# CRIPAC-DIG/GET

Hardware: AMD Instinct MI355X
Metric: claim-evidence pairs/sec fwd+bwd (B=32, h=300) (higher is better)
Workload: dtype f32

## Files before the change

### get_amd/csrc/common.h

```cpp
#pragma once
#include <hip/hip_runtime.h>
#include <stdint.h>
#include <stdio.h>
#include <stdlib.h>
#include <string.h>

namespace gh {

void set_error(const char* fmt, ...);

#define GH_CHECK_HIP(expr)                                                                  \
  do {                                                                                      \
    hipError_t _e = (expr);                                                                 \
    if (_e != hipSuccess) {                                                                 \
      gh::set_error("%s:%d: %s -> %s", __FILE__, __LINE__, #expr, hipGetErrorString(_e));   \
      return 1;                                                                             \
    }                                                                                       \
  } while (0)

#define GH_REQUIRE(cond, ...)                     \
  do {                                            \
    if (!(cond)) {                                \
      gh::set_error(__VA_ARGS__);                 \
      return 2;                                   \
    }                                             \
  } while (0)

#define GH_LAUNCH_CHECK() GH_CHECK_HIP(hipGetLastError())

inline int words_for(int r) { return (r + 63) / 64; }

inline int measure_env(const char* name, int dflt) {
#ifdef GH_MEASURE
  const char* e = getenv(name);
  return e ? atoi(e) : dflt;
#else
  (void)name;
  return dflt;
#endif
}
#ifdef GH_MEASURE
#define GH_DBG_BITS(L) ((L).dbg)
#else
#define GH_DBG_BITS(L) 0
#endif

enum ProfTag : int {
  PROF_GEMM_BIG = 0, PROF_GEMM_BIG_TN, PROF_GEMM_SMALL, PROF_GEMM_SMALL_TN,
  PROF_SPMM, PROF_SCORER_GSL, PROF_GRAPH_BUILD, PROF_ATT_SOFTMAX_FWD, PROF_ATT_SOFTMAX_BWD, PROF_ATT_DPRE,
  PROF_GATE_BWD_PRE, PROF_COLSUM, PROF_ADAM,
  PROF_FEW_ROWS,
  PROF_NTAGS
};
constexpr int PROF_FEW_GROUPS = 256;
unsigned int* clamp_counter();
bool prof_enabled();
void prof_begin(hipStream_t s, int tag);
void prof_end(int tag, double work, hipStream_t s);

int scorer_gsl_impl(const uint64_t* bits, const float* dinv, const float* vals, const int32_t* goff, int pads_collapsed, const float* feat,
                    const float* score_x, int score_parts, long long score_stride, const float* w_p, const float* gate, int n, int r, int h,
                    int k, float* score, uint64_t* keep, float drop_p, uint32_t drop_seed, hipStream_t stream);
int launch_ragged_plan(const int32_t* n_nodes, const int32_t* node_ids, int n, int r, int32_t* goff, int32_t* rowg, int32_t* src,
                       int32_t* cids, float* maskf, const int64_t* slot, int32_t* document, hipStream_t s, bool* scattered);
int launch_graph_build2(const int32_t* ta, const int32_t* la, int na, int ra, int32_t* ida, int32_t* nna, uint64_t* ba, float* da,
                        const int32_t* tb, const int32_t* lb, int nb, int rb, int32_t* idb, int32_t* nnb, uint64_t* bb, float* db,
                        int window, hipStream_t s);
struct ZeroFill { float* p0; long long n0; float* p1; long long n1; };
int launch_spmm(const uint64_t* bits, const float* dinv, const float* vals, const uint64_t* keep, const int32_t* goff,
                int m_real, const float* x, float* y, int n, int r, int h, int transpose, int accumulate, hipStream_t s,
                int bf16 = 0,
                const ZeroFill* zf = nullptr, bool* zf_done = nullptr);
int launch_gate_bwd_pre(const float* g, const float* z, const float* hh, const float* xp, float* dhp, float* dzp,
                        float* dxp, size_t count, hipStream_t s, int bf16 = 0);
int launch_colsum3(const float* a, const float* b, const float* c, float* oa, float* ob, float* oc, int m, int h,
                   hipStream_t s, float* oa2 = nullptr, float* ob2 = nullptr, float* oc2 = nullptr);
int launch_colsum(const float* a, float* oa, int m, int h, hipStream_t s);
struct Workspace { float* p; size_t bytes; float* cs; size_t cs_bytes; };
Workspace workspace_for(hipStream_t s);
int launch_gather_rows(const float* table, const int32_t* ids, float* dst, int m, int d, hipStream_t s,
                       float drop_p = 0.f, unsigned drop_seed = 0, int bf16 = 0);
int launch_tiny_linear_fwd(const float* x, const float* w, const float* bias, float* y, int m, int k, int n, hipStream_t s);
int launch_head_bwd(const float* g_phi, const float* y0, const float* w1, const float* w0, int B, int H, int C, int Xl, int E,
                    float* d_y0, float* dw1, float* db1, float* dx0, int dx0_accumulate, float* dx1, hipStream_t s);
size_t head_bwd_lds(int B, int H, int C, int E, const float* w0);
int launch_tiny_linear_bwd(const float* x, const float* w, const float* g, float* dx, float* dw, float* db, int m, int k, int n,
                           hipStream_t s);
int launch_att_softmax_fwd(float* e, const float* mask, const float* right, const int32_t* goff, int m_real,
                           int b, int l, int dr, int heads, float* weights, float* attended, hipStream_t s,
                           const float* e_parts = nullptr, int n_parts = 0, long long part_stride = 0, const void* right16 = nullptr);
int launch_att_softmax_bwd(const float* right, const float* weights, const float* g_att, const float* g_w,
                           const int32_t* goff, int m_real, int b, int l, int dr, int heads, float* de, float* dright,
                           hipStream_t s, const int32_t* rowg = nullptr, float* dw_tmp = nullptr, int* dw_written = nullptr,
                           const void* right16 = nullptr);
int gemm_mode();
int launch_att_dpre(const float* de, const float* w2, const float* t, const int32_t* goff, int m_real, int b, int l,
                    int ha, int heads, float* dpre, float* du, float* dw2_part, hipStream_t s, const float* dw_in = nullptr,
                    const float* weights = nullptr, float* de_out = nullptr, void* dpre16 = nullptr,
                    long long dw_range_stride = 0, int dw_ranges = 1);

struct GateFuse { const float* z; const float* hh; const float* xp; float* dhp; float* dzp; float* dxp; int bf16; };

int cell_fwd_impl(int bf, float* out32, const uint64_t* bits, const float* dinv, const float* vals, const uint64_t* keep,
                  const int32_t* goff, int m_real, int m_rows, const float* x, const int32_t* ids, int n, int r, int din, int h,
                  const float* w_p, const float* w_z0, const float* w_z1, const float* w_r0, const float* w_r1, const float* w_h0,
                  const float* w_h1, const float* b_z0, const float* b_z1, const float* b_r0, const float* b_r1, const float* b_h0,
                  const float* b_h1, float* xp, float* a, float* z, float* rr, float* rx, float* hh, float* out, float drop_p,
                  uint32_t drop_seed, const float* score_w, float* score_x, float score_drop_p, uint32_t score_drop_seed,
                  void* stream, int pad_out_dead = 0,
                  int* score_parts = nullptr,
                  float* xdrop = nullptr);
int cell_bwd_impl(int bf, const uint64_t* bits, const float* dinv, const float* vals, const uint64_t* keep, const int32_t* goff,
                  int m_real, const float* x, const int32_t* ids, int n, int r, int din, int h, const float* wt_p,
                  const float* wt_z0, const float* wt_z1, const float* wt_r0, const float* wt_r1, const float* wt_h0,
                  const float* wt_h1, const float* xp, const float* a, const float* z, const float* rr, const float* rx,
                  const float* hh, const float* g, float* dhp, float* dzp, float* drp, float* dxp, float* da, float* dx,
                  float* dw_p, float* dw_z0, float* dw_z1, float* dw_r0, float* dw_r1, float* dw_h0, float* dw_h1, float* db_z,
                  float* db_r, float* db_h, float* db_z1, float* db_r1, float* db_h1, float drop_p, uint32_t drop_seed, void* stream,
                  void* wstream, hipEvent_t ev_l1, hipEvent_t ev_agg,
                  int pre_done, const GateFuse* next,
                  const float* xdrop = nullptr);
int att_fwd_impl(const float* left, int nl, const int32_t* rowu, const float* right, const float* mask, const int32_t* goff,
                 const int32_t* rowg, int m_real, int b, int l, int xl, int dr, int ha, int heads, const float* w1, const float* w2,
                 float* u, float* t, float* e, float* weights, float* attended, hipStream_t s, int u_mode = 0,
                 const void* right16 = nullptr, const void* w1_16 = nullptr);
int att_bwd_impl(const float* left, const float* right, const int32_t* goff, int m_real, int b, int l, int xl, int dr, int ha,
                 int heads, const float* w1t, const float* w2, const float* t, const float* weights, const float* g_att,
                 const float* g_w, float* de, float* dpre, float* du, float* dleft, float* dright, float* dw1, float* dw2,
                 const int32_t* claim_offsets, int nl, float* du_c, int dleft_accumulate, hipStream_t s,
                 const int32_t* rowg = nullptr, float* dw_tmp = nullptr, const GateFuse* next = nullptr, int dleft_late = 0,
                 float* dw2_buf = nullptr, const void* right16 = nullptr, const void* w1t_16 = nullptr);
int linear2_fwd(const float* x0, int k0, const float* x1, int k1, const float* w, const float* bias, float* y, int m, int n, hipStream_t s,
                const float* w_out = nullptr, const float* b_out = nullptr, float* y_out = nullptr, int n_out = 0);
int linear2_bwd(const float* x0, int k0, const float* x1, int k1, const float* wt, const float* g, int m, int n, float* dx0,
                int dx0_accumulate, float* dx1, float* dw, float* db, hipStream_t s);

}
```

### get_amd/csrc/gemm.hip.h

```cpp
#pragma once
#include <hip/hip_runtime.h>
#include <stdint.h>
#include <type_traits>

namespace gh {

typedef float f32x4 __attribute__((ext_vector_type(4)));

enum EpiKind : int {
  EPI_STORE = 0,
  EPI_SIGMOID_Z,
  EPI_SIGMOID_R,
  EPI_TANH_H,
  EPI_ATT,
  EPI_BWD_DRX,
  EPI_ATOMIC,
  EPI_GATE_PRE,
};

struct Seg {
  const float* A; const int32_t* gatherA; int lda; int vecA;
  const float* B; const int32_t* gatherB; int ldb; int vecB;
  int K;
};

struct Problem {
  Seg seg[2];
  int nseg;
  int M, N;
  int epi;
  int accumulate;
  float* C; int ldc;
  const float* bias;
  const float* bias2;
  float* out1;
  const float* in0; const float* in1;
  const float* u; const float* w2; float* e; int ldu; int R; int heads;
  int seg0_rows;
  const int32_t* rowg;
  long long split_stride;
  float* colsum; long long colsum_stride;
  int drop_mode; int drop_ld; int drop_col0; unsigned drop_seed; unsigned drop_thresh; float drop_scale;
  int elt; int io; float* c32;
  int e_atomic;
  const float* gin; const float* in2; float* out2;
};

#define GH_MAX_PROBLEMS 12
struct Launch {
  Problem p[GH_MAX_PROBLEMS];
  int nprob;
  int m_tiles;
  int ksplit;
  int kchunk;
  int dbg;
  int n_tiles;
  int per;
};
static_assert(sizeof(Launch) <= 4096, "Launch travels by value in the kernarg segment (4 KB)");
constexpr int DBG_NO_EPILOGUE = 1;
constexpr int DBG_NO_KLOOP = 2;
constexpr int DBG_EPI_TICKS = 1024;

__host__ __device__ __forceinline__ unsigned drop_hash(unsigned seed, unsigned idx) {
  unsigned x = idx * 0x9E3779B1u + seed;
  x ^= x >> 16; x *= 0x85EBCA6Bu; x ^= x >> 13; x *= 0xC2B2AE35u; x ^= x >> 16;
  return x;
}
__device__ __forceinline__ float4 drop4(float4 v, unsigned seed, unsigned idx, unsigned thresh, float scale) {
  v.x = drop_hash(seed, idx + 0) >= thresh ? v.x * scale : 0.f;
  v.y = drop_hash(seed, idx + 1) >= thresh ? v.y * scale : 0.f;
  v.z = drop_hash(seed, idx + 2) >= thresh ? v.z * scale : 0.f;
  v.w = drop_hash(seed, idx + 3) >= thresh ? v.w * scale : 0.f;
  return v;
}

__device__ __forceinline__ float sigmoidf_(float x) { return 1.0f / (1.0f + __expf(-x)); }
__device__ __forceinline__ float tanhf_(float x) {
  float e = __expf(2.0f * x);
  return 1.0f - 2.0f / (e + 1.0f);
}

#define GH_KARG __attribute__((address_space(4)))

template <int WM, int WN, int NI, bool TN>
__global__ void __launch_bounds__(WM * WN * 64, 2)
gemm_kernel(const Launch L_byval) {
  (void)L_byval;
  const GH_KARG Launch& L = *(const GH_KARG Launch*)__builtin_amdgcn_kernarg_segment_ptr();
  constexpr int NTHR = WM * WN * 64;
  constexpr int BM = 32 * WM, BN = 16 * NI * WN, BK = 16;
  constexpr int LDA = BM + 2, LDB = BN + 2;
  constexpr int A4 = BM * 4;
  constexpr int B4 = BK * (BN / 4);
  constexpr int NA = (A4 + NTHR - 1) / NTHR;
  constexpr int NB = (B4 + NTHR - 1) / NTHR;
  __shared__ float smem[2 * BK * LDA + 2 * BK * LDB];
  float* As = smem;
  float* Bs = smem + 2 * BK * LDA;

  const int n_inner = TN ? L.m_tiles * L.nprob : L.nprob;
  const int n_outer = TN ? L.ksplit : L.m_tiles;
  const int bid = blockIdx.x;
  const int xcd = bid & 7, slot = bid >> 3;
  const int outer = xcd + 8 * (slot / n_inner);
  const int inner = slot % n_inner;
  if (outer >= n_outer) return;
  const int prob = TN ? inner % L.nprob : inner;
  const int m_tile = TN ? inner / L.nprob : outer;
  const int ks = TN ? outer : 0;
  const GH_KARG Problem& P = L.p[prob];
  const int M = P.M, N = P.N;
// ... 174 lines not shown
          for (int ni = 0; ni < NI; ++ni) {
            const int col = wcol + ni * 16 + l15;
            if (ni < ni_cnt && col < N) {
              const float t = tanhf_(acc[mi][ni][reg] + urow[col]);
              P.C[(size_t)row * ldc + col] = t;
#pragma unroll
              for (int c = 0; c < 8; ++c)
                if (c < heads) pe[c] += t * P.w2[c * N + col];
            }
          }
        }
#pragma unroll
        for (int c = 0; c < 8; ++c) {
          float v = pe[c];
          v += __shfl_xor(v, 1); v += __shfl_xor(v, 2); v += __shfl_xor(v, 4); v += __shfl_xor(v, 8);
          pe[c] = v;
        }
        if (WN == 1) {
          if (l15 == 0 && row < M && mi < mi_cnt)
            for (int c = 0; c < heads; ++c) P.e[(size_t)row * heads + c] = pe[c];
        } else {
          if (l15 == 0)
            for (int c = 0; c < 8; ++c) red[(wn * BM + lrow) * 8 + c] = pe[c];
        }
      }
    };
    att_rows(std::integral_constant<int, 0>{});
    att_rows(std::integral_constant<int, 1>{});
    if (WN > 1) {
      __syncthreads();
      for (int i = tid; i < BM * 8; i += NTHR) {
        const int lrow = i >> 3, c = i & 7, row = m0 + lrow;
        if (row < M && c < heads) {
          float v = 0.f;
          for (int w = 0; w < WN; ++w) v += red[(w * BM + lrow) * 8 + c];
          P.e[(size_t)row * heads + c] = v;
        }
      }
    }
    return;
  }

  auto epi_rows = [&](auto MI) __attribute__((always_inline)) {
    constexpr int mi = decltype(MI)::value;
#pragma unroll
    for (int ni = 0; ni < NI; ++ni) {
      const int col = wcol + ni * 16 + l15;
      const bool tile_ok = (mi < mi_cnt) && (ni < ni_cnt) && (col < N);
      const float bias = ((tile_ok && P.bias) ? P.bias[col] : 0.f) + ((tile_ok && P.bias2) ? P.bias2[col] : 0.f);
#pragma unroll
      for (int reg = 0; reg < 4; ++reg) {
        const int row = m0 + wrow + mi * 16 + q * 4 + reg;
        if (tile_ok && row < M) {
          const size_t o = (size_t)row * ldc + col;
          const float v = acc[mi][ni][reg] + bias;
          if (epi == EPI_STORE) {
            Cout[o] = P.accumulate ? Cout[o] + v : v;
          } else if (epi == EPI_SIGMOID_Z) {
            Cout[o] = sigmoidf_(v);
          } else if (epi == EPI_SIGMOID_R) {
            const float r = sigmoidf_(v);
            Cout[o] = r;
            P.out1[o] = r * P.in0[o];
          } else if (epi == EPI_TANH_H) {
            const float h = tanhf_(v), z = P.in0[o], xp = P.in1[o];
            Cout[o] = h;
            P.out1[o] = h * z + xp * (1.f - z);
          } else if (epi == EPI_BWD_DRX) {
            const float xp = P.in0[o], r = P.in1[o];
            Cout[o] = v * xp * r * (1.f - r);
            P.out1[o] += v * r;
          } else if (epi == EPI_ATOMIC) {
            atomicAdd(Cout + o, v);
          }
        }
      }
    }
  };
  epi_rows(std::integral_constant<int, 0>{});
  epi_rows(std::integral_constant<int, 1>{});
}

inline int vec_ok(const void* p, int ld, int inner) {
  return ((reinterpret_cast<uintptr_t>(p) & 15) == 0) && (ld % 4 == 0) && (inner % 4 == 0);
}

inline Seg make_seg(const float* A, int lda, const float* B, int ldb, int K, int n_inner,
                    const int32_t* gatherA = nullptr, const int32_t* gatherB = nullptr) {
  Seg s;
  s.A = A; s.lda = lda; s.gatherA = gatherA; s.vecA = vec_ok(A, lda, K);
  s.B = B; s.ldb = ldb; s.gatherB = gatherB; s.vecB = vec_ok(B, ldb, n_inner);
  s.K = K;
  return s;
}
inline Seg make_seg_nt(const float* A, int lda, const float* B, int ldb, int K, const int32_t* gatherA = nullptr, int elt = 0) {
  Seg s;
  const int q = elt ? 8 : 4;
  s.A = A; s.lda = lda; s.gatherA = gatherA; s.vecA = ((reinterpret_cast<uintptr_t>(A) & 15) == 0) && lda % q == 0 && K % q == 0;
  s.B = B; s.ldb = ldb; s.gatherB = nullptr; s.vecB = ((reinterpret_cast<uintptr_t>(B) & 15) == 0) && ldb % q == 0 && K % q == 0;
  s.K = K;
  return s;
}
inline Seg make_seg_tn(const float* A, int lda, int I, const float* B, int ldb, int J, int K,
                       const int32_t* gatherA = nullptr, const int32_t* gatherB = nullptr) {
  Seg s;
  s.A = A; s.lda = lda; s.gatherA = gatherA; s.vecA = vec_ok(A, lda, I);
  s.B = B; s.ldb = ldb; s.gatherB = gatherB; s.vecB = vec_ok(B, ldb, J);
  s.K = K;
  return s;
}

inline Problem make_problem(int M, int N, int epi, float* C, int ldc) {
  Problem p;
  memset(&p, 0, sizeof(p));
  p.M = M; p.N = N; p.epi = epi; p.C = C; p.ldc = ldc; p.nseg = 1;
  return p;
}


hipError_t launch_gemm(Launch& L, bool tn, hipStream_t stream);

}
```

### get_amd/csrc/gemm_nt.hip.h

```cpp
#pragma once
#include "common.h"
#include "gemm.hip.h"

namespace gh {
#ifdef GH_MEASURE
__device__ unsigned long long g_nt_phase[16 * 4];
#endif

__device__ __forceinline__ int nt_swz(int j) { return (0x78 >> (2 * j)) & 3; }
__device__ __forceinline__ unsigned nt_pack_bf16(float a, float b) {
  typedef float f32x2_t __attribute__((ext_vector_type(2)));
  typedef __bf16 bf16x2_t __attribute__((ext_vector_type(2)));
  const f32x2_t v = {a, b};
  return __builtin_bit_cast(unsigned, __builtin_convertvector(v, bf16x2_t));
}

template <int WM, int WN, int NI, int MI = 2, int MODE = 0>
__global__ void __launch_bounds__(WM * WN * 64, (MI == 8 || MI == 4 || MODE == 3 || MODE == 4) ? 2 : (WM == 2 && WN == 2 && NI == 5 && MODE == 0) ? 4 : 3)
gemm_nt_kernel(const Launch L_byval) {
  (void)L_byval;
#if defined(__HIP_DEVICE_COMPILE__)
  const GH_KARG Launch& L = *(const GH_KARG Launch*)__builtin_amdgcn_kernarg_segment_ptr();
  typedef __amdgpu_buffer_rsrc_t rsrc_t;
  constexpr int NW = WM * WN, NTHR = NW * 64;
// ... 384 lines not shown
        mma(aC, bX, 0, CX);
        __builtin_amdgcn_sched_barrier(0);
#pragma unroll
        for (int mi = 0; mi < MI; ++mi) aP[mi] = aC[mi];
        wait_inflight(min(T - 1, t + NST - 1) - (t + 1));
        __builtin_amdgcn_s_barrier();
        asm volatile("" ::: "memory");
        st = st == NST - 1 ? 0 : st + 1;
      }
      mma(aP, bY, NH, CY);
      __syncthreads();
      return;
    }
    dma_tile(0, 0);
    asm volatile("s_waitcnt vmcnt(0)" ::: "memory");
    __syncthreads();
    for (int t = 0; t < T; ++t) {
      const int st = t & 1;
      if (t + 1 < T) dma_tile(t + 1, st ^ 1);
      read_a(st, aC);
      read_b(st, bX, 0, NH);
      __builtin_amdgcn_sched_barrier(0);
      if (t > 0) mma(aP, bY, NH, CY);
      __builtin_amdgcn_sched_barrier(0);
      read_b(st, bY, NH, NI - NH);
      if (drop_mode == 1) drop_a(t, aC);
      __builtin_amdgcn_sched_barrier(0);
      mma(aC, bX, 0, CX);
      __builtin_amdgcn_sched_barrier(0);
#pragma unroll
      for (int mi = 0; mi < MI; ++mi) aP[mi] = aC[mi];
      asm volatile("s_waitcnt vmcnt(0)" ::: "memory");
      __syncthreads();
    }
    mma(aP, bY, NH, CY);
  };
  if constexpr (PP) {
#include "gemm_nt_pp.hip.h"
  } else {
    if (nvX == NH && nvY == NI - NH - 1) run(std::integral_constant<int, NH>{}, std::integral_constant<int, NI - NH - 1>{});
    else run(std::integral_constant<int, NH>{}, std::integral_constant<int, NI - NH>{});
  }

  if (dbg_bits & DBG_NO_EPILOGUE) {
    float sum = 0.f;
#pragma unroll
    for (int mi = 0; mi < MI; ++mi)
#pragma unroll
      for (int ni = 0; ni < NI; ++ni) sum += acc[mi][ni][0] + acc[mi][ni][1] + acc[mi][ni][2] + acc[mi][ni][3];
    if (sum == 12345.678f) P.C[0] = 0.f;
    return;
  }
  const int epi = P.epi;
  const int ldc = P.ldc;
  float* const C = P.C + (split ? (size_t)ks * (size_t)P.split_stride : (size_t)0);
  const float* bias = P.bias;
  float* out1 = P.out1;
  const float* in0 = P.in0;
  const float* in1 = P.in1;
  const int accumulate = P.accumulate;
  const int heads = P.heads;
  const bool scorer = (epi == EPI_TANH_H) && (P.w2 != nullptr);
  const int pad_rows = MODE == 2 ? 0 : P.seg0_rows;
  const bool out_dead = scorer && P.ldu == 1;
  const bool rowred = (epi == EPI_ATT) || scorer;
  float* ep = reinterpret_cast<float*>(smem);
  float* const ep_bias_ptr = ep + (PP ? 64 : 16 * WM) * EP_PITCH + NW * 64 * 4;
  const int N4 = N >> 2;
  constexpr int C4 = EP_PITCH / 4;
  constexpr int ITEMS = 16 * WM * C4;
  constexpr int NIT = (ITEMS + NTHR - 1) / NTHR;
  const float* bias2 = P.bias2;
  float* bsum = ep_bias_ptr;
  for (int c = tid; c < BN; c += NTHR) {
    float bv = 0.f;
    if (c < N) { if (bias) bv = bias[c]; if (bias2) bv += bias2[c]; }
    bsum[c] = bv;
  }
  const int io = (MODE == 2) ? P.io : 0;
  float* const c32 = (MODE == 2) ? P.c32 : nullptr;
  auto ld4 = [&](const float* p, size_t o, bool bf) __attribute__((always_inline)) {
    if constexpr (MODE == 2) {
      if (bf) {
        const uint2 u = *reinterpret_cast<const uint2*>(reinterpret_cast<const unsigned short*>(p) + o);
        return make_float4(__builtin_bit_cast(float, u.x << 16), __builtin_bit_cast(float, u.x & 0xffff0000u),
                           __builtin_bit_cast(float, u.y << 16), __builtin_bit_cast(float, u.y & 0xffff0000u));
      }
    }
    return *reinterpret_cast<const float4*>(p + o);
  };
  auto st4 = [&](float* p, size_t o, const float4 v, bool bf) __attribute__((always_inline)) {
    if constexpr (MODE == 2) {
      if (bf) {
        *reinterpret_cast<uint2*>(reinterpret_cast<unsigned short*>(p) + o) = make_uint2(nt_pack_bf16(v.x, v.y), nt_pack_bf16(v.z, v.w));
        return;
      }
    }
    __builtin_nontemporal_store(f32x4{v.x, v.y, v.z, v.w}, reinterpret_cast<f32x4*>(p + o));
  };
  auto row_reduce = [&](auto MIT) __attribute__((always_inline)) {
    constexpr int mi = decltype(MIT)::value;
    if (rowred) {
      __syncthreads();
      constexpr int KSPL = NW / WM;
      const int nred = scorer ? 1 : heads;
      const int b = wave % WM, kp = wave / WM;
      const float* arow = ep + (b * 16 + l15) * EP_PITCH + 4 * q;
// ... 1 lines not shown
      f32x4 d = f32x4{0.f, 0.f, 0.f, 0.f};
      for (int k0 = kp * 16; k0 < N; k0 += 16 * KSPL) {
        const f32x4 a4 = *reinterpret_cast<const f32x4*>(arow + k0);
        f32x4 w4 = f32x4{0.f, 0.f, 0.f, 0.f};
        if (l15 < nred && k0 + 4 * q < N) w4 = *reinterpret_cast<const f32x4*>(wrow + k0);
#pragma unroll
        for (int s2 = 0; s2 < 4; ++s2) d = __builtin_amdgcn_mfma_f32_16x16x4f32(w4[s2], a4[s2], d, 0, 0, 0);
      }
      float* red = ep + 16 * WM * EP_PITCH;
      *reinterpret_cast<f32x4*>(red + ((kp * WM + b) * 64 + lane) * 4) = d;
      __syncthreads();
      if (kp == 0) {
        f32x4 sum = d;
#pragma unroll
        for (int k2 = 1; k2 < KSPL; ++k2) sum += *reinterpret_cast<const f32x4*>(red + ((k2 * WM + b) * 64 + lane) * 4);
        const int row = m0 + b * 16 * MI + mi * 16 + l15;
        if (row < M) {
#pragma unroll
          for (int r = 0; r < 4; ++r)
            if (4 * q + r < nred) {
              if (P.e_atomic == 1) atomicAdd(&P.e[(size_t)row * nred + 4 * q + r], sum[r]);
              else P.e[(size_t)row * nred + 4 * q + r] = sum[r];
            }
        }
      }
    }
  };
  auto epilogue_pass = [&](auto MIT) __attribute__((always_inline)) {
    constexpr int mi = decltype(MIT)::value;
    if (mi > 0) __syncthreads();
#pragma unroll
    for (int ni = 0; ni < NI; ++ni)
      *reinterpret_cast<f32x4*>(ep + (wm * 16 + l15) * EP_PITCH + wcol + ni * 16 + 4 * q) = acc[mi][ni];
    __syncthreads();
    auto pass = [&](auto EPI) __attribute__((always_inline)) {
      constexpr int E = decltype(EPI)::value;
      constexpr int CH = 4;
#pragma unroll
      for (int it0 = 0; it0 < NIT; it0 += CH) {
        float4 xa[CH], xb[CH], xc[CH], xd[E == EPI_GATE_PRE ? CH : 1];
        auto where = [&](int j, int& row, int& col, float*& sp) __attribute__((always_inline)) {
          const int i = tid + (it0 + j) * NTHR;
          const int rr = i / C4, c4 = i - rr * C4;
          row = m0 + (rr >> 4) * 16 * MI + mi * 16 + (rr & 15);
          col = 4 * c4;
          sp = ep + rr * EP_PITCH + col;
          return (it0 + j < NIT) && (ITEMS % NTHR == 0 || i < ITEMS) && c4 < N4 && row < M;
        };
        if (E != EPI_SIGMOID_Z) {
#pragma unroll
          for (int j = 0; j < CH; ++j) {
            int row, col; float* sp;
            if (where(j, row, col, sp)) {
              const size_t o = (size_t)row * ldc + col;
              if (E == EPI_STORE) { if (accumulate) xa[j] = ld4(C, o, io & 1); }
              else if (E == EPI_SIGMOID_R) xa[j] = ld4(in0, o, io & 4);
              else if (E == EPI_TANH_H) { xa[j] = ld4(in0, o, io & 4); xb[j] = ld4(in1, o, io & 8); }
              else if (E == EPI_BWD_DRX) {
                xa[j] = ld4(in0, o, io & 4);
                xb[j] = ld4(in1, o, io & 8);
                xc[j] = ld4(out1, o, io & 2);
              } else if (E == EPI_GATE_PRE) {
                xa[j] = ld4(in0, o, io & 4);
                xb[j] = ld4(in1, o, io & 8);
                xc[j] = ld4(P.in2, o, io & 16);
                if (P.gin) xd[j] = ld4(P.gin, o, false);
              } else if (E == EPI_ATT)
                xa[j] = *reinterpret_cast<const float4*>(P.u + (size_t)(P.rowg ? P.rowg[row] : row / P.R) * P.ldu + col);
            }
          }
        }
#pragma unroll
        for (int j = 0; j < CH; ++j) {
          int row, col; float* sp;
          if (!where(j, row, col, sp)) continue;
          const float4 v4 = *reinterpret_cast<const float4*>(sp);
          const float4 b4 = *reinterpret_cast<const float4*>(bsum + col);
          float4 w = make_float4(v4.x + b4.x, v4.y + b4.y, v4.z + b4.z, v4.w + b4.w);
          const size_t o = (size_t)row * ldc + col;
          if (E == EPI_STORE) {
            if (drop_mode == 3)
              w = drop4(w, drop_seed, (unsigned)row * (unsigned)drop_ld + (unsigned)(P.drop_col0 + col), drop_thresh, drop_scale);
            if (accumulate) { w.x += xa[j].x; w.y += xa[j].y; w.z += xa[j].z; w.w += xa[j].w; }
            st4(C, o, w, io & 1);
          } else if (E == EPI_SIGMOID_Z) {
            st4(C, o, make_float4(sigmoidf_(w.x), sigmoidf_(w.y), sigmoidf_(w.z), sigmoidf_(w.w)), io & 1);
          } else if (E == EPI_SIGMOID_R) {
            const float4 x = xa[j];
            const float4 r4 = make_float4(sigmoidf_(w.x), sigmoidf_(w.y), sigmoidf_(w.z), sigmoidf_(w.w));
            if (!(pad_rows > 0 && row >= pad_rows)) st4(C, o, r4, io & 1);
            st4(out1, o, make_float4(r4.x * x.x, r4.y * x.y, r4.z * x.z, r4.w * x.w), io & 2);
          } else if (E == EPI_TANH_H) {
            const float4 z = xa[j], x = xb[j];
            const float4 h = make_float4(tanhf_(w.x), tanhf_(w.y), tanhf_(w.z), tanhf_(w.w));
            float4 y = make_float4(h.x * z.x + x.x * (1.f - z.x), h.y * z.y + x.y * (1.f - z.y),
                                   h.z * z.z + x.z * (1.f - z.z), h.w * z.w + x.w * (1.f - z.w));
            const bool pad = pad_rows > 0 && row >= pad_rows;
            if (!pad) st4(C, o, h, io & 1);
            if (!(pad && out_dead)) st4(out1, o, y, io & 2);
            if (c32) *reinterpret_cast<float4*>(c32 + o) = y;
            if (scorer) {
              if (drop_mode == 2)
                y = drop4(y, drop_seed, (unsigned)row * (unsigned)drop_ld + (unsigned)(P.drop_col0 + col), drop_thresh, drop_scale);
              *reinterpret_cast<float4*>(sp) = y;
            }
          } else if (E == EPI_BWD_DRX) {
            const float4 x = xa[j], r4 = xb[j];
            float4 d = xc[j];
            st4(C, o, make_float4(w.x * x.x * r4.x * (1.f - r4.x), w.y * x.y * r4.y * (1.f - r4.y),
                                  w.z * x.z * r4.z * (1.f - r4.z), w.w * x.w * r4.w * (1.f - r4.w)), io & 1);
            d.x += w.x * r4.x; d.y += w.y * r4.y; d.z += w.z * r4.z; d.w += w.w * r4.w;
            st4(out1, o, d, io & 2);
          } else if (E == EPI_GATE_PRE) {
            if (drop_mode == 3)
              w = drop4(w, drop_seed, (unsigned)row * (unsigned)drop_ld + (unsigned)(P.drop_col0 + col), drop_thresh, drop_scale);
            if (P.gin) { const float4 a4 = xd[j]; w.x += a4.x; w.y += a4.y; w.z += a4.z; w.w += a4.w; }
            const float4 Z = xa[j], Hh = xb[j], X = xc[j];
            float4 a, b, c;
#define GH_ONE(f)                                      \
            a.f = w.f * Z.f * (1.f - Hh.f * Hh.f);             \
            b.f = w.f * (Hh.f - X.f) * Z.f * (1.f - Z.f);      \
            c.f = w.f * (1.f - Z.f);
            GH_ONE(x) GH_ONE(y) GH_ONE(z) GH_ONE(w)
#undef GH_ONE
            if constexpr (MODE == 2) {
              st4(C, o, a, io & 1); st4(out1, o, b, io & 2); st4(P.out2, o, c, io & 32);
            } else {
              *reinterpret_cast<float4*>(C + o) = a;
              *reinterpret_cast<float4*>(out1 + o) = b;
              *reinterpret_cast<float4*>(P.out2 + o) = c;
            }
          } else if (E == EPI_ATT) {
            const float4 u4 = xa[j];
            const float4 t4 = make_float4(tanhf_(w.x + u4.x), tanhf_(w.y + u4.y), tanhf_(w.z + u4.z), tanhf_(w.w + u4.w));
            *reinterpret_cast<float4*>(C + o) = t4;
            *reinterpret_cast<float4*>(sp) = t4;
          }
        }
      }
    };
    auto pass8 = [&](auto EPI) __attribute__((always_inline)) {
      constexpr int E = decltype(EPI)::value;
      constexpr int C8 = BN / 8;
      constexpr int ITEMS8 = 16 * WM * C8;
      constexpr int NIT8 = (ITEMS8 + NTHR - 1) / NTHR;
      constexpr int CH = 2;
      struct F8 { float4 a, b; };
      auto ld8 = [&](const float* p, size_t o, bool bf) __attribute__((always_inline)) {
        F8 r;
        if (bf) {
          const uint4 u = *reinterpret_cast<const uint4*>(reinterpret_cast<const unsigned short*>(p) + o);
          r.a = make_float4(__builtin_bit_cast(float, u.x << 16), __builtin_bit_cast(float, u.x & 0xffff0000u),
                            __builtin_bit_cast(float, u.y << 16), __builtin_bit_cast(float, u.y & 0xffff0000u));
          r.b = make_float4(__builtin_bit_cast(float, u.z << 16), __builtin_bit_cast(float, u.z & 0xffff0000u),
                            __builtin_bit_cast(float, u.w << 16), __builtin_bit_cast(float, u.w & 0xffff0000u));
        } else {
          r.a = *reinterpret_cast<const float4*>(p + o);
          r.b = *reinterpret_cast<const float4*>(p + o + 4);
        }
        return r;
      };
      auto st8 = [&](float* p, size_t o, const float4 a, const float4 b, bool bf) __attribute__((always_inline)) {
        if (bf) {
          *reinterpret_cast<uint4*>(reinterpret_cast<unsigned short*>(p) + o) =
              make_uint4(nt_pack_bf16(a.x, a.y), nt_pack_bf16(a.z, a.w), nt_pack_bf16(b.x, b.y), nt_pack_bf16(b.z, b.w));
        } else {
          *reinterpret_cast<float4*>(p + o) = a;
          *reinterpret_cast<float4*>(p + o + 4) = b;
        }
      };
      auto sig4 = [](const float4 v) __attribute__((always_inline)) { return make_float4(sigmoidf_(v.x), sigmoidf_(v.y), sigmoidf_(v.z), sigmoidf_(v.w)); };
      auto tanh4 = [](const float4 v) __attribute__((always_inline)) { return make_float4(tanhf_(v.x), tanhf_(v.y), tanhf_(v.z), tanhf_(v.w)); };
      auto mul4 = [](const float4 a, const float4 b) __attribute__((always_inline)) { return make_float4(a.x * b.x, a.y * b.y, a.z * b.z, a.w * b.w); };
      auto add4 = [](const float4 a, const float4 b) __attribute__((always_inline)) { return make_float4(a.x + b.x, a.y + b.y, a.z + b.z, a.w + b.w); };
      auto mix4 = [](const float4 h, const float4 z, const float4 x) __attribute__((always_inline)) {
        return make_float4(h.x * z.x + x.x * (1.f - z.x), h.y * z.y + x.y * (1.f - z.y), h.z * z.z + x.z * (1.f - z.z), h.w * z.w + x.w * (1.f - z.w));
      };
      auto drx4 = [](const float4 w, const float4 x, const float4 r) __attribute__((always_inline)) {
        return make_float4(w.x * x.x * r.x * (1.f - r.x), w.y * x.y * r.y * (1.f - r.y), w.z * x.z * r.z * (1.f - r.z), w.w * x.w * r.w * (1.f - r.w));
      };
#pragma unroll
      for (int it0 = 0; it0 < NIT8; it0 += CH) {
        F8 xa[CH], xb[CH], xc[CH], xd[E == EPI_GATE_PRE ? CH : 1];
        auto where = [&](int j, int& row, int& col, float*& sp) __attribute__((always_inline)) {
          const int i = tid + (it0 + j) * NTHR;
          const int rr = i / C8, c8 = i - rr * C8;
          row = m0 + (rr >> 4) * 16 * MI + mi * 16 + (rr & 15);
          col = 8 * c8;
          sp = ep + rr * EP_PITCH + col;
          return (it0 + j < NIT8) && (ITEMS8 % NTHR == 0 || i < ITEMS8) && col < N && row < M;
        };
        if (E != EPI_SIGMOID_Z) {
#pragma unroll
          for (int j = 0; j < CH; ++j) {
            int row, col; float* sp;
            if (where(j, row, col, sp)) {
              const size_t o = (size_t)row * ldc + col;
              if (E == EPI_STORE) { if (accumulate) xa[j] = ld8(C, o, io & 1); }
              else if (E == EPI_SIGMOID_R) xa[j] = ld8(in0, o, io & 4);
              else if (E == EPI_TANH_H) { xa[j] = ld8(in0, o, io & 4); xb[j] = ld8(in1, o, io & 8); }
              else if (E == EPI_BWD_DRX) { xa[j] = ld8(in0, o, io & 4); xb[j] = ld8(in1, o, io & 8); xc[j] = ld8(out1, o, io & 2); }
              else if (E == EPI_GATE_PRE) {
                xa[j] = ld8(in0, o, io & 4); xb[j] = ld8(in1, o, io & 8); xc[j] = ld8(P.in2, o, io & 16);
                if (P.gin) xd[j] = ld8(P.gin, o, false);
              }
            }
          }
        }
#pragma unroll
        for (int j = 0; j < CH; ++j) {
          int row, col; float* sp;
          if (!where(j, row, col, sp)) continue;
          float4 wa = add4(*reinterpret_cast<const float4*>(sp), *reinterpret_cast<const float4*>(bsum + col));
          float4 wb = add4(*reinterpret_cast<const float4*>(sp + 4), *reinterpret_cast<const float4*>(bsum + col + 4));
          const size_t o = (size_t)row * ldc + col;
          if (E == EPI_STORE) {
            if (drop_mode == 3) {
              const unsigned idx = (unsigned)row * (unsigned)drop_ld + (unsigned)(P.drop_col0 + col);
              wa = drop4(wa, drop_seed, idx, drop_thresh, drop_scale);
              wb = drop4(wb, drop_seed, idx + 4u, drop_thresh, drop_scale);
            }
            if (accumulate) { wa = add4(wa, xa[j].a); wb = add4(wb, xa[j].b); }
            st8(C, o, wa, wb, io & 1);
          } else if (E == EPI_SIGMOID_Z) {
            st8(C, o, sig4(wa), sig4(wb), io & 1);
          } else if (E == EPI_SIGMOID_R) {
            const float4 ra = sig4(wa), rb = sig4(wb);
            st8(C, o, ra, rb, io & 1);
            st8(out1, o, mul4(ra, xa[j].a), mul4(rb, xa[j].b), io & 2);
          } else if (E == EPI_TANH_H) {
            const float4 ha = tanh4(wa), hb = tanh4(wb);
            const float4 ya = mix4(ha, xa[j].a, xb[j].a), yb = mix4(hb, xa[j].b, xb[j].b);
            st8(C, o, ha, hb, io & 1);
            st8(out1, o, ya, yb, io & 2);
            if (c32) { *reinterpret_cast<float4*>(c32 + o) = ya; *reinterpret_cast<float4*>(c32 + o + 4) = yb; }
            if (scorer) {
              float4 sa = ya, sb = yb;
              if (drop_mode == 2) {
                const unsigned idx = (unsigned)row * (unsigned)drop_ld + (unsigned)(P.drop_col0 + col);
                sa = drop4(sa, drop_seed, idx, drop_thresh, drop_scale);
                sb = drop4(sb, drop_seed, idx + 4u, drop_thresh, drop_scale);
              }
              *reinterpret_cast<float4*>(sp) = sa;
              *reinterpret_cast<float4*>(sp + 4) = sb;
            }
          } else if (E == EPI_BWD_DRX) {
            st8(C, o, drx4(wa, xa[j].a, xb[j].a), drx4(wb, xa[j].b, xb[j].b), io & 1);
            st8(out1, o, add4(xc[j].a, mul4(wa, xb[j].a)), add4(xc[j].b, mul4(wb, xb[j].b)), io & 2);
          } else if (E == EPI_GATE_PRE) {
            if (drop_mode == 3) {
              const unsigned idx = (unsigned)row * (unsigned)drop_ld + (unsigned)(P.drop_col0 + col);
              wa = drop4(wa, drop_seed, idx, drop_thresh, drop_scale);
              wb = drop4(wb, drop_seed, idx + 4u, drop_thresh, drop_scale);
            }
            if (P.gin) { wa = add4(wa, xd[j].a); wb = add4(wb, xd[j].b); }
            auto head = [](const float4 g, const float4 Z, const float4 Hh, const float4 X, float4& a, float4& b, float4& c) __attribute__((always_inline)) {
#define GH_ONE8(f)                                    \
              a.f = g.f * Z.f * (1.f - Hh.f * Hh.f);          \
              b.f = g.f * (Hh.f - X.f) * Z.f * (1.f - Z.f);   \
              c.f = g.f * (1.f - Z.f);
              GH_ONE8(x) GH_ONE8(y) GH_ONE8(z) GH_ONE8(w)
#undef GH_ONE8
            };
            float4 a0, b0, c0, a1, b1, c1;
            head(wa, xa[j].a, xb[j].a, xc[j].a, a0, b0, c0);
            head(wb, xa[j].b, xb[j].b, xc[j].b, a1, b1, c1);
            st8(C, o, a0, a1, io & 1); st8(out1, o, b0, b1, io & 2); st8(P.out2, o, c0, c1, io & 32);
          }
        }
      }
    };
    constexpr bool WIDE8 = (MODE == 2) && (BN % 8 == 0);
    bool done8 = false;
    if constexpr (WIDE8) {
      if (epi != EPI_ATT) {
        if (epi == EPI_STORE) pass8(std::integral_constant<int, EPI_STORE>{});
        else if (epi == EPI_GATE_PRE) pass8(std::integral_constant<int, EPI_GATE_PRE>{});
        else if (epi == EPI_SIGMOID_Z) pass8(std::integral_constant<int, EPI_SIGMOID_Z>{});
        else if (epi == EPI_SIGMOID_R) pass8(std::integral_constant<int, EPI_SIGMOID_R>{});
        else if (epi == EPI_TANH_H) pass8(std::integral_constant<int, EPI_TANH_H>{});
        else if (epi == EPI_BWD_DRX) pass8(std::integral_constant<int, EPI_BWD_DRX>{});
        if (!rowred) return;
        done8 = true;
      }
    }
    if (done8) {  }
    else if (epi == EPI_STORE) pass(std::integral_constant<int, EPI_STORE>{});
    else if (epi == EPI_SIGMOID_Z) pass(std::integral_constant<int, EPI_SIGMOID_Z>{});
    else if (epi == EPI_SIGMOID_R) pass(std::integral_constant<int, EPI_SIGMOID_R>{});
    else if (epi == EPI_TANH_H) pass(std::integral_constant<int, EPI_TANH_H>{});
    else if (epi == EPI_BWD_DRX) pass(std::integral_constant<int, EPI_BWD_DRX>{});
    else if (epi == EPI_GATE_PRE) pass(std::integral_constant<int, EPI_GATE_PRE>{});
    else if (epi == EPI_ATT) pass(std::integral_constant<int, EPI_ATT>{});
    row_reduce(MIT);
  };
  if constexpr ((MODE == 0 || MODE == 1) && MI == 2) {
    bool f32_done = false;
#include "gemm_nt_epi32.hip.h"
    if (f32_done) return;
  }
  if constexpr (PP) {
    bool pp_done = true;
#include "gemm_nt_pp_epi.hip.h"
    if (pp_done) return;
  }
  epilogue_pass(std::integral_constant<int, 0>{});
  epilogue_pass(std::integral_constant<int, 1>{});
  if constexpr (MI >= 4) {
    epilogue_pass(std::integral_constant<int, 2>{});
    epilogue_pass(std::integral_constant<int, 3>{});
  }
  if constexpr (MI == 8) {
    epilogue_pass(std::integral_constant<int, 4>{});
    epilogue_pass(std::integral_constant<int, 5>{});
    epilogue_pass(std::integral_constant<int, 6>{});
    epilogue_pass(std::integral_constant<int, 7>{});
  }
#endif
}

// ... 2 lines not shown
```

### get_amd/csrc/gemm_nt_epi32.hip.h

```cpp
{
  constexpr int NITF = (ITEMS + NTHR - 1) / NTHR;
  constexpr int TOT = MI * NITF;
  constexpr int PD = 2, NSET = PD + 1;
  typedef unsigned e32_u32x4 __attribute__((ext_vector_type(4)));
  int tid_e = tid;
  asm volatile("" : "+v"(tid_e));
  auto f_item = [&](int mi_, int it, int& row, int& col, int& rr) __attribute__((always_inline)) {
    const int i = tid_e + it * NTHR;
    rr = i / C4;
    const int c4 = i - rr * C4;
    col = 4 * c4;
    row = m0 + (rr >> 4) * 16 * MI + mi_ * 16 + (rr & 15);
    return (ITEMS % NTHR == 0 || i < ITEMS) && c4 < N4 && row < M;
  };
  auto as_f4 = [](const e32_u32x4 u) __attribute__((always_inline)) {
    const f32x4 f = __builtin_bit_cast(f32x4, u);
    return make_float4(f[0], f[1], f[2], f[3]);
  };
  auto as_u4 = [](const float4 v) __attribute__((always_inline)) {
    return e32_u32x4{__builtin_bit_cast(unsigned, v.x), __builtin_bit_cast(unsigned, v.y), __builtin_bit_cast(unsigned, v.z), __builtin_bit_cast(unsigned, v.w)};
  };
  auto fast = [&](auto EPI, auto ACCF, auto GINF) __attribute__((always_inline)) {
    constexpr int E = decltype(EPI)::value;
    constexpr bool ACC = decltype(ACCF)::value, GIN = decltype(GINF)::value, ATT = E == EPI_ATT;
    constexpr int NIN = E == EPI_STORE ? (ACC ? 1 : 0) : (E == EPI_SIGMOID_Z || ATT) ? 0 : E == EPI_SIGMOID_R ? 1 : E == EPI_TANH_H ? 2 : 3;
    constexpr int NOUT = (E == EPI_STORE || E == EPI_SIGMOID_Z || ATT) ? 1 : E == EPI_GATE_PRE ? 3 : 2;
    constexpr int NTAUX = (E == EPI_GATE_PRE || ATT) ? 0 : 2;
    const void* i0 = E == EPI_STORE ? (const void*)C : (const void*)in0;
    const void* i2 = E == EPI_BWD_DRX ? (const void*)out1 : (const void*)P.in2;
    const rsrc_t rs_i0 = __builtin_amdgcn_make_buffer_rsrc((void*)(NIN >= 1 ? i0 : (const void*)C), 0, 0x7fffffff, 0x00020000);
    const rsrc_t rs_i1 = __builtin_amdgcn_make_buffer_rsrc((void*)(NIN >= 2 ? (const void*)in1 : (const void*)C), 0, 0x7fffffff, 0x00020000);
    const rsrc_t rs_i2 = __builtin_amdgcn_make_buffer_rsrc((void*)(NIN >= 3 ? i2 : (const void*)C), 0, 0x7fffffff, 0x00020000);
    const rsrc_t rs_g = __builtin_amdgcn_make_buffer_rsrc((void*)(GIN ? (const void*)P.gin : ATT ? (const void*)P.u : (const void*)C), 0, 0x7fffffff, 0x00020000);
    const rsrc_t rs_o0 = __builtin_amdgcn_make_buffer_rsrc((void*)C, 0, 0x7fffffff, 0x00020000);
    const rsrc_t rs_o1 = __builtin_amdgcn_make_buffer_rsrc((void*)(NOUT >= 2 ? (void*)out1 : (void*)C), 0, 0x7fffffff, 0x00020000);
    const rsrc_t rs_o2 = __builtin_amdgcn_make_buffer_rsrc((void*)(NOUT >= 3 ? (void*)P.out2 : (void*)C), 0, 0x7fffffff, 0x00020000);
    e32_u32x4 qa[NSET], qb[NSET], qc[NSET], qg[NSET];
    unsigned uoff[ATT ? TOT : 1];
    if constexpr (ATT) {
#pragma unroll
      for (int idx = 0; idx < TOT; ++idx) {
        int row, col, rr;
        const bool ok = f_item(idx / NITF, idx % NITF, row, col, rr);
        const int rc_ = min(row, M - 1);
        const int ur = P.rowg ? P.rowg[rc_] : rc_ / P.R;
        uoff[idx] = ok ? (unsigned)(ur * P.ldu + col) * 4u : OOB;
      }
    }
    auto load = [&](auto IDX) __attribute__((always_inline)) {
      constexpr int idx = decltype(IDX)::value, mi_ = idx / NITF, it = idx % NITF, s_ = idx % NSET;
      int row, col, rr;
      const bool ok = f_item(mi_, it, row, col, rr);
      const unsigned vo = ok ? (unsigned)(row * ldc + col) * 4u : OOB;
      if constexpr (NIN >= 1) qa[s_] = __builtin_bit_cast(e32_u32x4, __builtin_amdgcn_raw_buffer_load_b128(rs_i0, vo, 0, 0));
      if constexpr (NIN >= 2) qb[s_] = __builtin_bit_cast(e32_u32x4, __builtin_amdgcn_raw_buffer_load_b128(rs_i1, vo, 0, 0));
      if constexpr (NIN >= 3) qc[s_] = __builtin_bit_cast(e32_u32x4, __builtin_amdgcn_raw_buffer_load_b128(rs_i2, vo, 0, 0));
      if constexpr (GIN) qg[s_] = __builtin_bit_cast(e32_u32x4, __builtin_amdgcn_raw_buffer_load_b128(rs_g, vo, 0, 0));
      if constexpr (ATT) qg[s_] = __builtin_bit_cast(e32_u32x4, __builtin_amdgcn_raw_buffer_load_b128(rs_g, uoff[idx], 0, 0));
    };
    auto compute = [&](auto IDX) __attribute__((always_inline)) {
      constexpr int idx = decltype(IDX)::value, mi_ = idx / NITF, it = idx % NITF, s_ = idx % NSET;
      int row, col, rr;
      const bool ok = f_item(mi_, it, row, col, rr);
      const unsigned vo = ok ? (unsigned)(row * ldc + col) * 4u : OOB;
      float* sp = ep + min(rr, 16 * WM - 1) * EP_PITCH + min(col, BN - 4);
      const float4 v4 = *reinterpret_cast<const float4*>(sp);
      const float4 b4 = *reinterpret_cast<const float4*>(bsum + min(col, BN - 4));
      float4 w = make_float4(v4.x + b4.x, v4.y + b4.y, v4.z + b4.z, v4.w + b4.w);
      const bool pad = pad_rows > 0 && row >= pad_rows;
      auto st = [&](const rsrc_t rs, const float4 v, bool live) __attribute__((always_inline)) {
        __builtin_amdgcn_raw_buffer_store_b128(as_u4(v), rs, live ? vo : OOB, 0, NTAUX);
      };
      if (E == EPI_STORE) {
        if (drop_mode == 3)
          w = drop4(w, drop_seed, (unsigned)row * (unsigned)drop_ld + (unsigned)(P.drop_col0 + col), drop_thresh, drop_scale);
        if constexpr (ACC) { const float4 x = as_f4(qa[s_]); w.x += x.x; w.y += x.y; w.z += x.z; w.w += x.w; }
        st(rs_o0, w, true);
      } else if (E == EPI_SIGMOID_Z) {
        st(rs_o0, make_float4(sigmoidf_(w.x), sigmoidf_(w.y), sigmoidf_(w.z), sigmoidf_(w.w)), true);
      } else if (E == EPI_SIGMOID_R) {
        const float4 x = as_f4(qa[s_]);
        const float4 r4 = make_float4(sigmoidf_(w.x), sigmoidf_(w.y), sigmoidf_(w.z), sigmoidf_(w.w));
        st(rs_o0, r4, !pad);
        st(rs_o1, make_float4(r4.x * x.x, r4.y * x.y, r4.z * x.z, r4.w * x.w), true);
      } else if (E == EPI_TANH_H) {
        const float4 z = as_f4(qa[s_]), x = as_f4(qb[s_]);
        const float4 h = make_float4(tanhf_(w.x), tanhf_(w.y), tanhf_(w.z), tanhf_(w.w));
        float4 y = make_float4(h.x * z.x + x.x * (1.f - z.x), h.y * z.y + x.y * (1.f - z.y),
                               h.z * z.z + x.z * (1.f - z.z), h.w * z.w + x.w * (1.f - z.w));
        st(rs_o0, h, !pad);
        st(rs_o1, y, !(pad && out_dead));
        if (scorer) {
          if (drop_mode == 2)
            y = drop4(y, drop_seed, (unsigned)row * (unsigned)drop_ld + (unsigned)(P.drop_col0 + col), drop_thresh, drop_scale);
          if (ok) *reinterpret_cast<float4*>(sp) = y;
        }
      } else if (E == EPI_BWD_DRX) {
        const float4 x = as_f4(qa[s_]), r4 = as_f4(qb[s_]);
        float4 d = as_f4(qc[s_]);
        st(rs_o0, make_float4(w.x * x.x * r4.x * (1.f - r4.x), w.y * x.y * r4.y * (1.f - r4.y),
                              w.z * x.z * r4.z * (1.f - r4.z), w.w * x.w * r4.w * (1.f - r4.w)), true);
        d.x += w.x * r4.x; d.y += w.y * r4.y; d.z += w.z * r4.z; d.w += w.w * r4.w;
        st(rs_o1, d, true);
      } else if (E == EPI_GATE_PRE) {
        if (drop_mode == 3)
          w = drop4(w, drop_seed, (unsigned)row * (unsigned)drop_ld + (unsigned)(P.drop_col0 + col), drop_thresh, drop_scale);
        if constexpr (GIN) { const float4 a4 = as_f4(qg[s_]); w.x += a4.x; w.y += a4.y; w.z += a4.z; w.w += a4.w; }
        const float4 Z = as_f4(qa[s_]), Hh = as_f4(qb[s_]), X = as_f4(qc[s_]);
        float4 a, b, c;
#define GH_E32_ONE(f)                                  \
        a.f = w.f * Z.f * (1.f - Hh.f * Hh.f);             \
        b.f = w.f * (Hh.f - X.f) * Z.f * (1.f - Z.f);      \
        c.f = w.f * (1.f - Z.f);
        GH_E32_ONE(x) GH_E32_ONE(y) GH_E32_ONE(z) GH_E32_ONE(w)
#undef GH_E32_ONE
        st(rs_o0, a, true); st(rs_o1, b, true); st(rs_o2, c, true);
      } else if (E == EPI_ATT) {
        const float4 u4 = as_f4(qg[s_]);
        const float4 t4 = make_float4(tanhf_(w.x + u4.x), tanhf_(w.y + u4.y), tanhf_(w.z + u4.z), tanhf_(w.w + u4.w));
        st(rs_o0, t4, true);
        if (ok) *reinterpret_cast<float4*>(sp) = t4;
      }
    };
    auto stage = [&](auto MIT) __attribute__((always_inline)) {
      constexpr int mi_ = decltype(MIT)::value;
      if (mi_ > 0) __syncthreads();
#pragma unroll
      for (int ni = 0; ni < NI; ++ni)
        *reinterpret_cast<f32x4*>(ep + (wm * 16 + l15) * EP_PITCH + wcol + ni * 16 + 4 * q) = acc[mi_][ni];
      __syncthreads();
    };
    auto step = [&](auto IDX) __attribute__((always_inline)) {
      constexpr int idx = decltype(IDX)::value;
      if constexpr (idx % NITF == 0) stage(std::integral_constant<int, idx / NITF>{});
      if constexpr (idx + PD < TOT) load(std::integral_constant<int, idx + PD>{});
      __builtin_amdgcn_sched_barrier(0);
      compute(IDX);
      __builtin_amdgcn_sched_barrier(0);
      if constexpr (idx % NITF == NITF - 1) { if (rowred) row_reduce(std::integral_constant<int, idx / NITF>{}); }
    };
    load(std::integral_constant<int, 0>{});
    if constexpr (TOT > 1 && PD > 1) load(std::integral_constant<int, 1>{});
    static_assert(TOT <= 24, "the unrolled item sequence below");
#define GH_E32_STEP(k) if constexpr (k < TOT) step(std::integral_constant<int, k>{});
    GH_E32_STEP(0) GH_E32_STEP(1) GH_E32_STEP(2) GH_E32_STEP(3) GH_E32_STEP(4) GH_E32_STEP(5) GH_E32_STEP(6) GH_E32_STEP(7)
    GH_E32_STEP(8) GH_E32_STEP(9) GH_E32_STEP(10) GH_E32_STEP(11) GH_E32_STEP(12) GH_E32_STEP(13) GH_E32_STEP(14) GH_E32_STEP(15)
    GH_E32_STEP(16) GH_E32_STEP(17) GH_E32_STEP(18) GH_E32_STEP(19) GH_E32_STEP(20) GH_E32_STEP(21) GH_E32_STEP(22) GH_E32_STEP(23)
#undef GH_E32_STEP
  };
  constexpr std::integral_constant<bool, false> NO{};
  constexpr std::integral_constant<bool, true> YES{};
  if (io == 0) {
    f32_done = true;
    if (epi == EPI_STORE) { if (accumulate) fast(std::integral_constant<int, EPI_STORE>{}, YES, NO); else fast(std::integral_constant<int, EPI_STORE>{}, NO, NO); }
    else if (epi == EPI_SIGMOID_Z) fast(std::integral_constant<int, EPI_SIGMOID_Z>{}, NO, NO);
    else if (epi == EPI_SIGMOID_R) fast(std::integral_constant<int, EPI_SIGMOID_R>{}, NO, NO);
    else if (epi == EPI_TANH_H) fast(std::integral_constant<int, EPI_TANH_H>{}, NO, NO);
    else if (epi == EPI_BWD_DRX) fast(std::integral_constant<int, EPI_BWD_DRX>{}, NO, NO);
    else if (epi == EPI_GATE_PRE) { if (P.gin) fast(std::integral_constant<int, EPI_GATE_PRE>{}, NO, YES); else fast(std::integral_constant<int, EPI_GATE_PRE>{}, NO, NO); }
    else if (epi == EPI_ATT) fast(std::integral_constant<int, EPI_ATT>{}, NO, NO);
    else f32_done = false;
  }
}
```

### get_amd/csrc/gemm_ops.hip

```cpp
#include "../../include/get_hip.h"
#include "common.h"
#include "gemm.hip.h"
#include "gemm_nt.hip.h"
#include "gemm_tn.hip.h"
#include "gemm_tn_pp.hip.h"
#include <stdlib.h>

namespace gh {

static inline bool al16(const void* p) { return (reinterpret_cast<uintptr_t>(p) & 15) == 0; }

static bool s_lds_bad(const Problem& p) { return p.seg[0].lda % 8 || p.seg[0].ldb % 8; }
static void fast_why(int rule, int prob, const Problem* p = nullptr, int seg = -1) {
  static const bool dbg = measure_env("GH_FASTOK_DEBUG", 0) != 0;
  if (!dbg) return;
  fprintf(stderr, "gemm: generic kernel (fast_ok rule %d, problem %d)\n", rule, prob);
  if (p && seg >= 0) fprintf(stderr, "   seg %d lda %d M %d N %d K %d\n", seg, p->seg[seg].lda, p->M, p->N, p->seg[seg].K);
}
static bool fast_ok(const Launch& L, bool tn) {
  for (int i = 0; i < L.nprob; ++i) {
    const Problem& p = L.p[i];
    const int ns = tn ? 1 : p.nseg;
    for (int j = 0; j < ns; ++j) {
      const Seg& s = p.seg[j];
      if (!s.vecA || !s.vecB || s.gatherB || s.K < 4) { fast_why(1, i); return false; }
      if (tn && s.gatherA) { fast_why(2, i); return false; }
    }
    if (p.elt && tn && (p.M % 8 || p.N % 8 || s_lds_bad(p))) { fast_why(3, i); return false; }
    if (!tn) {
      for (int j = 0; j < p.nseg; ++j) {
        if (4.0 * (double)p.seg[j].ldb * (double)p.N >= 2147483648.0) { fast_why(4, i); return false; }
        if (!p.seg[j].gatherA && 4.0 * (double)p.seg[j].lda * (double)p.M >= 2147483648.0) { fast_why(5, i, &p, j); return false; }
      }
    }
    if (tn) {
      const Seg& s = p.seg[0];
      if (4.0 * (double)s.lda * (double)s.K >= 2147483648.0 || 4.0 * (double)s.ldb * (double)s.K >= 2147483648.0) { fast_why(6, i); return false; }
    }
    if (p.N % 4 || p.N < 4 || p.ldc % 4 || !al16(p.C)) { fast_why(7, i); return false; }
    if (tn && (p.M % 4 || p.M < 4)) { fast_why(8, i); return false; }
    if ((p.bias && !al16(p.bias)) || (p.bias2 && !al16(p.bias2)) || (p.out1 && !al16(p.out1)) || (p.in0 && !al16(p.in0)) || (p.in1 && !al16(p.in1)))
      { fast_why(9, i); return false; }
    if (p.epi == EPI_ATT && (!al16(p.u) || p.ldu % 4 || !al16(p.w2))) { fast_why(10, i); return false; }
    if (p.epi == EPI_TANH_H && p.w2 && !al16(p.w2)) { fast_why(11, i); return false; }
    if (p.epi == EPI_GATE_PRE && (tn || !p.in0 || !p.in1 || !p.in2 || !p.out1 || !p.out2 || !al16(p.in2) || !al16(p.out2) ||
                                  (p.gin && !al16(p.gin)))) { fast_why(12, i); return false; }
  }
  return true;
}
constexpr int TN_PP_ROWS = 16384;
static bool wants_dropout(const Launch& L) {
  for (int i = 0; i < L.nprob; ++i)
    if (L.p[i].drop_mode) return true;
  return false;
}

static long long g_path_counts[3] = {0, 0, 0};
static int g_gemm_mode = 0;
static bool x3p_substitute(Launch& L, hipStream_t s);

int gemm_mode() { return g_gemm_mode; }

template <int WM, int WN, int NI, int MI = 2>
static hipError_t launch_cfg(const Launch& L, bool tn, hipStream_t s) {
  const bool fast = fast_ok(L, tn);
  {
    double fl = 0.0;
    for (int i = 0; i < L.nprob; ++i)
      for (int j = 0; j < L.p[i].nseg; ++j) fl += 2.0 * L.p[i].M * L.p[i].N * (double)L.p[i].seg[j].K;
    g_path_counts[fast ? 0 : 1] += 1;
    if (!fast && fl >= 1e9) g_path_counts[2] += 1;
  }
  const int n_outer = tn ? L.ksplit : L.m_tiles;
  const int n_inner = tn ? L.m_tiles * L.nprob : L.nprob * L.ksplit;
  const bool nt_few = !tn && L.m_tiles < 8 && fast;
  const int grid = nt_few ? n_outer * n_inner : 8 * ((n_outer + 7) / 8) * n_inner;
  if (grid <= 0) return hipSuccess;
  int max_rows = 0;
  for (int i = 0; i < L.nprob; ++i) { const int rws = tn ? L.p[i].seg[0].K : L.p[i].M; if (rws > max_rows) max_rows = rws; }
  const int tag = (max_rows >= 8192 ? PROF_GEMM_BIG : PROF_GEMM_SMALL) + (tn ? 1 : 0);
  double flops = 0.0;
  if (prof_enabled()) {
    for (int i = 0; i < L.nprob; ++i)
      for (int j = 0; j < L.p[i].nseg; ++j) {
        int rows = L.p[i].M;
        if (j == 0 && !tn && L.p[i].nseg > 1 && L.p[i].seg0_rows > 0) {
          const int bm = 16 * MI * WM, cut = ((L.p[i].seg0_rows + bm - 1) / bm) * bm;
          if (cut < rows) rows = cut;
        }
        flops += 2.0 * rows * L.p[i].N * (double)L.p[i].seg[j].K;
      }
    prof_begin(s, tag);
// ... 469 lines not shown
  }

  void flush() {
    if (L.nprob == 0 || err != hipSuccess) { reset(); return; }
    if (tn) {
      const int n_inner = L.m_tiles * L.nprob;
      constexpr int target = 2304;
      int ks = (target + n_inner - 1) / n_inner;
      constexpr int min_rows16 = 4096;
      const int min_rows = L.p[0].elt ? min_rows16 : 256;
      const int ks_max = (k_total / min_rows > 1) ? k_total / min_rows : 1;
      if (ks > ks_max) ks = ks_max;
      if (ks < 1) ks = 1;
      const int align = tn_pp ? 64 : L.p[0].elt ? 32 : 16;
      if (tn_pp) {
        const int tiles = L.nprob * L.m_tiles * L.n_tiles;
        const int ks1 = 256 / tiles > 0 ? 256 / tiles : 1, ks2 = 512 / tiles > 0 ? 512 / tiles : 1;
        const double e1 = tiles * ks1 / 256.0, e2 = tiles * ks2 / 512.0;
        ks = (e1 >= 0.85 || e1 >= e2) ? ks1 : ks2;
        const int kmax = k_total / 1024 > 1 ? k_total / 1024 : 1;
        if (ks > kmax) ks = kmax;
        size_t out_bytes = 0;
        for (int i = 0; i < L.nprob; ++i) out_bytes += ((size_t)L.p[i].M * L.p[i].N + (cs_out[i] ? (size_t)L.p[i].M : 0)) * sizeof(float);
        while (ks > 1 && (size_t)ks * out_bytes > g_ws_bytes) --ks;
      } else
      if (ks >= 12) ks = ((ks + 4) / 8) * 8;
      int chunk = (k_total + ks - 1) / ks;
      chunk = ((chunk + align - 1) / align) * align;
      L.kchunk = chunk;
      L.ksplit = (k_total + chunk - 1) / chunk;
      if (tn_pp) L.per = (L.nprob * L.m_tiles * L.n_tiles * L.ksplit + 7) / 8;
      if (!tn_pp && L.ksplit >= 12 && L.ksplit % 8 != 0) {
        const int k8 = (L.ksplit / 8) * 8;
        chunk = (((k_total + k8 - 1) / k8 + align - 1) / align) * align;
        if ((k_total + chunk - 1) / chunk % 8 == 0) { L.kchunk = chunk; L.ksplit = (k_total + chunk - 1) / chunk; }
      }
      size_t need = 0;
      bool want_cs0 = false;
      for (int i = 0; i < L.nprob; ++i) want_cs0 = want_cs0 || cs_out[i] != nullptr;
      bool ws_ok = g_ws != nullptr && (L.ksplit > 1 || tn_pp || (want_cs0 && L.p[0].elt));
      bool any_cs = false;
      for (int i = 0; i < L.nprob && ws_ok; ++i) {
        if (L.p[i].N % 4) ws_ok = false;
        need += (size_t)L.ksplit * L.p[i].M * L.p[i].N * sizeof(float);
        if (cs_out[i]) { need += (size_t)L.ksplit * L.p[i].M * sizeof(float); any_cs = true; }
      }
      bool want_cs = false;
      for (int i = 0; i < L.nprob; ++i) want_cs = want_cs || cs_out[i] != nullptr;
      if (any_cs && !(ws_ok && need <= g_ws_bytes && fast_ok(L, true) && (g_gemm_mode != 1 || L.p[0].elt))) any_cs = false;
      if (want_cs && !any_cs) {
        for (int i = 0; i < L.nprob; ++i) {
          if (!cs_out[i]) continue;
          const Seg& sg = L.p[i].seg[0];
          if (L.p[i].elt || sg.lda != L.p[i].M) { colsum_missed = true; continue; }
          if (launch_colsum3(sg.A, nullptr, nullptr, cs_out[i], nullptr, nullptr, sg.K, L.p[i].M, s, cs_out2[i], nullptr, nullptr)) colsum_missed = true;
          else colsum_fused = true;
        }
      }
      if (ws_ok && need <= g_ws_bytes) {
        ReduceArgs R;
        R.n = L.nprob;
        float* w = g_ws;
        int max_elems = 0;
        for (int i = 0; i < L.nprob; ++i) {
          Problem& q = L.p[i];
          R.it[i] = ReduceItem{w, q.C, q.M, q.N, q.ldc, L.ksplit, (long long)q.M * q.N};
          q.C = w; q.ldc = q.N; q.epi = EPI_STORE; q.accumulate = 0; q.split_stride = (long long)q.M * q.N;
          w += (size_t)L.ksplit * q.M * q.N;
          if (q.M * (q.N / 4) > max_elems) max_elems = q.M * (q.N / 4);
        }
        ReduceArgs RC;
        RC.n = 0;
        int max_cs = 0;
        for (int i = 0; i < L.nprob && any_cs; ++i) {
          Problem& q = L.p[i];
          if (!cs_out[i]) continue;
          q.colsum = w; q.colsum_stride = q.M;
          RC.it[RC.n++] = ReduceItem{w, cs_out[i], 1, q.M, q.M, L.ksplit, (long long)q.M};
          if (cs_out2[i] && RC.n < GH_MAX_PROBLEMS) RC.it[RC.n++] = ReduceItem{w, cs_out2[i], 1, q.M, q.M, L.ksplit, (long long)q.M};
          w += (size_t)L.ksplit * q.M;
          if (q.M / 4 > max_cs) max_cs = q.M / 4;
        }
        hipError_t e = launch_any();
        if (e != hipSuccess) err = e;
        for (int i = 0; i < RC.n; ++i) R.it[R.n++] = RC.it[i];
        if (max_cs > max_elems) max_elems = max_cs;
        hipLaunchKernelGGL(reduce_partials_kernel, dim3((max_elems + 255) / 256, R.n), dim3(256), 0, s, R);
        if (RC.n > 0) colsum_fused = true;
        e = hipGetLastError();
        if (e != hipSuccess) err = e;
        reset();
        return;
      }
    }
    if (tn && tn_pp) { err = hipErrorInvalidValue; reset(); return; }
    if (!tn && nt_split_plan()) return;
    hipError_t e = launch_any();
    if (e != hipSuccess) err = e;
    reset();
  }

  hipError_t launch_any() {
    if (tn && tn_pp) return launch_tn_pp(L, s);
    if (narrow && !tn && L.ksplit == 1 && !L.p[0].elt) return launch_cfg<2, 2, 5>(L, tn, s);
    if (big && !tn && L.ksplit == 1 && !L.p[0].elt) {
      const double r = (double)L.m_tiles * L.nprob / 768.0;
      const double frac = r - (double)(long long)r;
      if (g_gemm_mode != 1 && r < 3.0 && frac > 0.02 && frac < 0.45) {
        int mt = 0;
        for (int i = 0; i < L.nprob; ++i) { const int t = (L.p[i].M + 31) / 32; if (t > mt) mt = t; }
        L.m_tiles = mt;
        return launch_cfg<1, 4, 5>(L, tn, s);
      }
    }
    if (wide256) {
      bool ok = L.ksplit == 1;
      for (int i = 0; i < L.nprob; ++i) {
        if (L.p[i].drop_mode == 1) ok = false;
        for (int j = 0; j < L.p[i].nseg; ++j) if (L.p[i].seg[j].K % 64) ok = false;
      }
      if (ok) return launch_cfg<2, 4, 4, 8>(L, tn, s);
      int mt = 0;
      for (int i = 0; i < L.nprob; ++i) { const int t = (L.p[i].M + 127) / 128; if (t > mt) mt = t; }
      L.m_tiles = mt;
      return launch_cfg<2, 2, 8, 4>(L, tn, s);
    }
    if (wide) return launch_cfg<2, 2, 8, 4>(L, tn, s);
    return big ? launch_cfg<2, 2, 10>(L, tn, s) : launch_cfg<1, 4, 5>(L, tn, s);
  }

  bool nt_split_plan() {
    const int blocks = L.m_tiles * L.nprob;
    constexpr int max_blocks = 96;
    if (g_ws == nullptr || blocks >= max_blocks || !fast_ok(L, false)) return false;
    int tmax = 0;
    for (int i = 0; i < L.nprob; ++i) {
      const Problem& q = L.p[i];
      if (q.epi == EPI_ATOMIC || q.epi == EPI_GATE_PRE || q.drop_mode != 0 || (q.epi == EPI_TANH_H && q.w2) || q.seg0_rows > 0 || q.elt) return false;
      int t = 0;
      for (int j = 0; j < q.nseg; ++j) t += (q.seg[j].K + 15) / 16;
      if (i > 0 && t != tmax) return false;
      tmax = t;
    }
    int ks = tmax / 4;
    const int tgt = tmax >= 128 ? 512 : 256;
    const int want = (tgt + blocks - 1) / blocks;
    if (ks > want) ks = want;
    if (ks < 2) return false;
    const int ct = (tmax + ks - 1) / ks;
    ks = (tmax + ct - 1) / ct;
    if (ks < 2) return false;
    size_t need = 0;
    for (int i = 0; i < L.nprob; ++i) need += (size_t)ks * L.p[i].M * L.p[i].N * sizeof(float);
    if (need > g_ws_bytes) return false;
    FinishArgs F;
    F.n = L.nprob;
    float* w = g_ws;
    int max_m = 0;
    for (int i = 0; i < L.nprob; ++i) {
      Problem& q = L.p[i];
      F.it[i] = FinishItem{w, (long long)q.M * q.N, ks, q.M, q.N, q.epi, q.accumulate, q.ldc,
                           q.C, q.bias, q.bias2, q.out1, q.in0, q.in1, q.u, q.w2, q.e, q.ldu, q.R, q.heads, q.rowg};
      q.C = w; q.ldc = q.N; q.epi = EPI_STORE; q.accumulate = 0; q.bias = nullptr; q.bias2 = nullptr;
      q.split_stride = (long long)q.M * q.N;
      w += (size_t)ks * q.M * q.N;
      if (q.M > max_m) max_m = q.M;
    }
    L.ksplit = ks;
    L.kchunk = ct * 16;
    hipError_t e = launch_any();
    if (e != hipSuccess) err = e;
    F.split = (ks >= 16 && max_m <= 8192) ? 1 : 0;
    hipLaunchKernelGGL(nt_finish_kernel, dim3(F.split ? max_m : (max_m + 3) / 4, F.n), dim3(256), 0, s, F);
    split_done = true;
    e = hipGetLastError();
    if (e != hipSuccess) err = e;
    reset();
    return true;
  }
};

static Problem gemm_problem(int M, int N, int epi, float* C, int ldc, const float* A, int lda, const float* B, int ldb,
                            int K, const int32_t* gatherA = nullptr, int elt = 0) {
  Problem p = make_problem(M, N, epi, C, ldc);
  p.elt = elt;
  p.seg[0] = make_seg_nt(A, lda, B, ldb, K, gatherA, elt);
  return p;
}
static void add_seg(Problem& p, const float* A, int lda, const float* B, int ldb, int K) {
  p.seg[p.nseg++] = make_seg_nt(A, lda, B, ldb, K, nullptr, p.elt);
}
static void set_dropout(Problem& p, int mode, int ld, float drop_p, unsigned seed) {
  if (drop_p <= 0.f) return;
  p.drop_mode = mode; p.drop_ld = ld; p.drop_col0 = 0; p.drop_seed = seed;
  const double t = (double)drop_p * 4294967296.0;
  p.drop_thresh = t >= 4294967295.0 ? 4294967295u : (unsigned)t;
  p.drop_scale = 1.0f / (1.0f - drop_p);
}
static Problem tn_problem(int I, int J, float* C, int ldc, const float* A, int lda, const float* B, int ldb, int K,
                          const int32_t* gatherB = nullptr, int elt = 0) {
  Problem p = make_problem(I, J, EPI_ATOMIC, C, ldc);
  p.seg[0] = make_seg_tn(A, lda, I, B, ldb, J, K, nullptr, gatherB);
  p.elt = elt;
  if (elt) {
    p.seg[0].vecA = ((reinterpret_cast<uintptr_t>(A) & 15) == 0) && lda % 8 == 0 && I % 8 == 0;
    p.seg[0].vecB = ((reinterpret_cast<uintptr_t>(B) & 15) == 0) && ldb % 8 == 0 && J % 8 == 0;
  }
  return p;
}

}

using namespace gh;

int gh::cell_fwd_impl(int bf, float* out32, const uint64_t* bits, const float* dinv, const float* vals, const uint64_t* keep,
                                const int32_t* goff, int m_real, int m_rows,
// ... 99 lines not shown
    GH_CHECK_HIP(b.err);
  }
  GH_REQUIRE(!partial_zero || g_path_counts[1] == generic_before,
             "ggnn_cell_fwd: internal -- a gate GEMM took the generic kernel although the padding rows of `a` were only zeroed for the fast one");
  return 0;
}

extern "C" int gh_ggnn_cell_fwd(const uint64_t* bits, const float* dinv, const float* vals, const uint64_t* keep,
                                const int32_t* goff, int m_real, int m_rows,
                                const float* x, const int32_t* ids, int n, int r, int din, int h,
                                const float* w_p, const float* w_z0, const float* w_z1, const float* w_r0,
                                const float* w_r1, const float* w_h0, const float* w_h1,
                                const float* b_z0, const float* b_z1, const float* b_r0, const float* b_r1,
                                const float* b_h0, const float* b_h1,
                                float* xp, float* a, float* z, float* rr, float* rx, float* hh, float* out,
                                float drop_p, uint32_t drop_seed,
                                const float* score_w, float* score_x, float score_drop_p, uint32_t score_drop_seed,
                                gh_stream_t stream) {
  return cell_fwd_impl(0, nullptr, bits, dinv, vals, keep, goff, m_real, m_rows, x, ids, n, r, din, h, w_p, w_z0, w_z1, w_r0, w_r1,
                       w_h0, w_h1, b_z0, b_z1, b_r0, b_r1, b_h0, b_h1, xp, a, z, rr, rx, hh, out, drop_p, drop_seed, score_w,
                       score_x, score_drop_p, score_drop_seed, stream, 0, nullptr, nullptr);
}

extern "C" int gh_ggnn_cell_fwd_bf16(const uint64_t* bits, const float* dinv, const float* vals, const uint64_t* keep,
                                     const int32_t* goff, int m_real, int m_rows,
                                     const void* x, const int32_t* ids, int n, int r, int din, int h,
                                     const void* w_p, const void* w_z0, const void* w_z1, const void* w_r0,
                                     const void* w_r1, const void* w_h0, const void* w_h1,
                                     const float* b_z0, const float* b_z1, const float* b_r0, const float* b_r1,
                                     const float* b_h0, const float* b_h1,
                                     void* xp, void* a, void* z, void* rr, void* rx, void* hh, void* out, float* out32,
                                     float drop_p, uint32_t drop_seed,
                                     const float* score_w, float* score_x, float score_drop_p, uint32_t score_drop_seed,
                                     gh_stream_t stream) {
  typedef const float* cf;
  typedef float* mf;
  return cell_fwd_impl(1, out32, bits, dinv, vals, keep, goff, m_real, m_rows, (cf)x, ids, n, r, din, h, (cf)w_p, (cf)w_z0, (cf)w_z1,
                       (cf)w_r0, (cf)w_r1, (cf)w_h0, (cf)w_h1, b_z0, b_z1, b_r0, b_r1, b_h0, b_h1, (mf)xp, (mf)a, (mf)z, (mf)rr,
                       (mf)rx, (mf)hh, (mf)out, drop_p, drop_seed, score_w, score_x, score_drop_p, score_drop_seed, stream, 0, nullptr, nullptr);
}

int gh::cell_bwd_impl(int bf, const uint64_t* bits, const float* dinv, const float* vals, const uint64_t* keep,
                                const int32_t* goff, int m_real,
                                const float* x, const int32_t* ids, int n, int r, int din, int h,
                                const float* wt_p, const float* wt_z0, const float* wt_z1, const float* wt_r0,
                                const float* wt_r1, const float* wt_h0, const float* wt_h1,
                                const float* xp, const float* a, const float* z, const float* rr, const float* rx,
                                const float* hh, const float* g,
                                float* dhp, float* dzp, float* drp, float* dxp, float* da,
                                float* dx, float* dw_p, float* dw_z0, float* dw_z1, float* dw_r0, float* dw_r1,
                                float* dw_h0, float* dw_h1, float* db_z, float* db_r, float* db_h,
                                float* db_z1, float* db_r1, float* db_h1, float drop_p, uint32_t drop_seed,
                                gh_stream_t stream, gh_stream_t wstream, hipEvent_t ev_l1, hipEvent_t ev_agg,
                                int pre_done, const GateFuse* next, const float* xdrop) {
  hipStream_t s = (hipStream_t)stream;
  hipStream_t sw = wstream ? (hipStream_t)wstream : s;
  const bool two = sw != s;
  GH_REQUIRE(!two || (ev_l1 && ev_agg), "ggnn_cell_bwd: a separate weight-gradient stream needs its two events");
  GH_REQUIRE(n > 0 && r > 0 && din > 0 && h > 0, "ggnn_cell_bwd: bad sizes");
  GH_REQUIRE(!bf || (din % 8 == 0 && h % 8 == 0 && din <= h), "ggnn_cell_bwd_bf16: needs din %% 8 == 0, h %% 8 == 0, din <= h (din=%d h=%d)", din, h);
  if (!goff) m_real = n * r;
  GH_REQUIRE(m_real >= 0 && m_real <= n * r, "ggnn_cell_bwd: node-compact rows %d do not fit n*r=%d", m_real, n * r);
  GH_REQUIRE(drop_p <= 0.f || (long long)n * r * (long long)din < (1LL << 32),
             "ggnn_cell_bwd: %d rows x %d columns exceed the dropout mask's 32-bit element index", n * r, din);
  const int M = m_real;
  if (M == 0) return 0;
  if (!pre_done)
    if (int e = launch_gate_bwd_pre(g, z, hh, xp, dhp, dzp, dxp, (size_t)M * h, s, bf)) return e;
  const bool wide = bf && h % 256 == 0;
  {
    Batch b(false, M, s, wide, 3, h);
    Problem p0 = gemm_problem(M, h, EPI_STORE, da, h, dhp, h, wt_h0, h, h, nullptr, bf);
    Problem p1 = gemm_problem(M, h, EPI_BWD_DRX, drp, h, dhp, h, wt_h1, h, h, nullptr, bf);
    p1.out1 = dxp; p1.in0 = xp; p1.in1 = rr;
    p0.io = bf ? 1 : 0; p1.io = bf ? 15 : 0;
    b.add(p0); b.add(p1);
    b.flush();
    GH_CHECK_HIP(b.err);
  }
  const bool cs = bf ? true : (h % 4 == 0);
  bool colsum_done = false;
  if (two) {
    GH_CHECK_HIP(hipEventRecord(ev_l1, s));
    GH_CHECK_HIP(hipStreamWaitEvent(sw, ev_l1, 0));
    Batch b(true, M, sw);
    b.add(tn_problem(h, h, dw_z0, h, dzp, h, a, h, M, nullptr, bf));  if (cs) b.want_colsum(db_z, db_z1);
    b.add(tn_problem(h, h, dw_z1, h, dzp, h, xp, h, M, nullptr, bf));
    b.add(tn_problem(h, h, dw_r0, h, drp, h, a, h, M, nullptr, bf));  if (cs) b.want_colsum(db_r, db_r1);
    b.add(tn_problem(h, h, dw_r1, h, drp, h, xp, h, M, nullptr, bf));
    b.add(tn_problem(h, h, dw_h0, h, dhp, h, a, h, M, nullptr, bf));  if (cs) b.want_colsum(db_h, db_h1);
    b.add(tn_problem(h, h, dw_h1, h, dhp, h, rx, h, M, nullptr, bf));
    b.flush();
    GH_CHECK_HIP(b.err);
    colsum_done = b.colsum_fused && !b.colsum_missed;
    if (!colsum_done) {
      GH_REQUIRE(!bf, "ggnn_cell_bwd_bf16: the bias gradients need the split-K workspace (gh_set_workspace)");
      if (int e = launch_colsum3(dzp, drp, dhp, db_z, db_r, db_h, M, h, sw, db_z1, db_r1, db_h1)) return e;
    }
  }
  {
    Batch b(false, M, s, wide, 4, h);
    Problem p0 = gemm_problem(M, h, EPI_STORE, da, h, dzp, h, wt_z0, h, h, nullptr, bf);
    add_seg(p0, drp, h, wt_r0, h, h);
    p0.accumulate = 1;
    Problem p1 = gemm_problem(M, h, EPI_STORE, dxp, h, dzp, h, wt_z1, h, h, nullptr, bf);
    add_seg(p1, drp, h, wt_r1, h, h);
    p1.accumulate = 1;
    p0.io = p1.io = bf ? 1 : 0;
    b.add(p0); b.add(p1);
    b.flush();
    GH_CHECK_HIP(b.err);
  }
  if (int e = launch_spmm(bits, dinv, vals, keep, goff, m_real, da, dxp, n, r, h, 1, 1, s, bf)) return e;
  if (two) {
    GH_CHECK_HIP(hipEventRecord(ev_agg, s));
    GH_CHECK_HIP(hipStreamWaitEvent(sw, ev_agg, 0));
  }
  if (dx || next) {
    GH_REQUIRE(!next || (din % 4 == 0 && (next->bf16 != 0) == (bf != 0)), "ggnn_cell_bwd: the fused gate head needs float4-shaped rows and both cells in the same storage mode");
    Batch b(false, M, s, wide && din % 256 == 0, 5, din);
    Problem p = gemm_problem(M, din, next ? EPI_GATE_PRE : EPI_STORE, next ? next->dhp : dx, din, dxp, h, wt_p, h, h, nullptr, bf);
    if (next) {
      p.in0 = next->z; p.in1 = next->hh; p.in2 = next->xp; p.out1 = next->dzp; p.out2 = next->dxp;
      p.io = next->bf16 ? (1 | 2 | 4 | 8 | 16 | 32) : 0;
    }
    set_dropout(p, 3, din, drop_p, drop_seed);
    b.add(p);
    b.flush();
    GH_CHECK_HIP(b.err);
  }
  {
    Batch b(true, M, sw);
    if (!two) {
      b.add(tn_problem(h, h, dw_z0, h, dzp, h, a, h, M, nullptr, bf));  if (cs) b.want_colsum(db_z, db_z1);
      b.add(tn_problem(h, h, dw_z1, h, dzp, h, xp, h, M, nullptr, bf));
      b.add(tn_problem(h, h, dw_r0, h, drp, h, a, h, M, nullptr, bf));  if (cs) b.want_colsum(db_r, db_r1);
      b.add(tn_problem(h, h, dw_r1, h, drp, h, xp, h, M, nullptr, bf));
      b.add(tn_problem(h, h, dw_h0, h, dhp, h, a, h, M, nullptr, bf));  if (cs) b.want_colsum(db_h, db_h1);
      b.add(tn_problem(h, h, dw_h1, h, dhp, h, rx, h, M, nullptr, bf));
    }
    if (bf && xdrop && drop_p > 0.f && din <= h) {
      b.add(tn_problem(h, din, dw_p, din, dxp, h, xdrop, din, M, nullptr, bf));
    } else if ((ids || drop_p > 0.f || bf) && din <= h) {
      if (int e = launch_gather_rows(x, ids, da, M, din, sw, drop_p, drop_seed, bf)) return e;
      b.add(tn_problem(h, din, dw_p, din, dxp, h, da, din, M, nullptr, bf));
    } else {
      GH_REQUIRE(drop_p == 0.f, "ggnn_cell_bwd: fused dropout needs din (%d) <= h (%d)", din, h);
      b.add(tn_problem(h, din, dw_p, din, dxp, h, x, din, M, ids));
    }
    b.flush();
    GH_CHECK_HIP(b.err);
    if (two || (b.colsum_fused && !b.colsum_missed)) return 0;
  }
  GH_REQUIRE(!bf, "ggnn_cell_bwd_bf16: the bias gradients need the split-K workspace (gh_set_workspace)");
  return launch_colsum3(dzp, drp, dhp, db_z, db_r, db_h, M, h, s, db_z1, db_r1, db_h1);
}

extern "C" int gh_ggnn_cell_bwd(const uint64_t* bits, const float* dinv, const float* vals, const uint64_t* keep,
                                const int32_t* goff, int m_real,
                                const float* x, const int32_t* ids, int n, int r, int din, int h,
                                const float* wt_p, const float* wt_z0, const float* wt_z1, const float* wt_r0,
                                const float* wt_r1, const float* wt_h0, const float* wt_h1,
                                const float* xp, const float* a, const float* z, const float* rr, const float* rx,
                                const float* hh, const float* g,
                                float* dhp, float* dzp, float* drp, float* dxp, float* da,
                                float* dx, float* dw_p, float* dw_z0, float* dw_z1, float* dw_r0, float* dw_r1,
                                float* dw_h0, float* dw_h1, float* db_z, float* db_r, float* db_h,
                                float* db_z1, float* db_r1, float* db_h1, float drop_p, uint32_t drop_seed,
                                gh_stream_t stream) {
  return cell_bwd_impl(0, bits, dinv, vals, keep, goff, m_real, x, ids, n, r, din, h, wt_p, wt_z0, wt_z1, wt_r0, wt_r1, wt_h0, wt_h1,
                       xp, a, z, rr, rx, hh, g, dhp, dzp, drp, dxp, da, dx, dw_p, dw_z0, dw_z1, dw_r0, dw_r1, dw_h0, dw_h1,
                       db_z, db_r, db_h, db_z1, db_r1, db_h1, drop_p, drop_seed, stream, nullptr, nullptr, nullptr, 0, nullptr, nullptr);
}

extern "C" int gh_ggnn_cell_bwd_bf16(const uint64_t* bits, const float* dinv, const float* vals, const uint64_t* keep,
                                     const int32_t* goff, int m_real,
                                     const void* x, const int32_t* ids, int n, int r, int din, int h,
                                     const void* wt_p, const void* wt_z0, const void* wt_z1, const void* wt_r0,
                                     const void* wt_r1, const void* wt_h0, const void* wt_h1,
                                     const void* xp, const void* a, const void* z, const void* rr, const void* rx,
                                     const void* hh, const float* g,
                                     void* dhp, void* dzp, void* drp, void* dxp, void* da,
                                     float* dx, float* dw_p, float* dw_z0, float* dw_z1, float* dw_r0, float* dw_r1,
                                     float* dw_h0, float* dw_h1, float* db_z, float* db_r, float* db_h,
                                     float* db_z1, float* db_r1, float* db_h1, float drop_p, uint32_t drop_seed,
                                     gh_stream_t stream) {
  typedef const float* cf;
  typedef float* mf;
  return cell_bwd_impl(1, bits, dinv, vals, keep, goff, m_real, (cf)x, ids, n, r, din, h, (cf)wt_p, (cf)wt_z0, (cf)wt_z1, (cf)wt_r0,
                       (cf)wt_r1, (cf)wt_h0, (cf)wt_h1, (cf)xp, (cf)a, (cf)z, (cf)rr, (cf)rx, (cf)hh, g, (mf)dhp, (mf)dzp, (mf)drp,
                       (mf)dxp, (mf)da, dx, dw_p, dw_z0, dw_z1, dw_r0, dw_r1, dw_h0, dw_h1, db_z, db_r, db_h, db_z1, db_r1,
                       db_h1, drop_p, drop_seed, stream, nullptr, nullptr, nullptr, 0, nullptr, nullptr);
}

int gh::att_fwd_impl(const float* left, int nl, const int32_t* rowu, const float* right, const float* mask, const int32_t* goff,
                 const int32_t* rowg, int m_real, int b, int l, int xl, int dr, int ha, int heads, const float* w1, const float* w2,
                 float* u, float* t, float* e, float* weights, float* attended, hipStream_t s, int u_mode,
                 const void* right16, const void* w1_16) {
  GH_REQUIRE(heads >= 1 && heads <= 8, "concat_att: heads=%d not in [1,8]", heads);
  GH_REQUIRE(b > 0 && l > 0 && dr > 0 && ha > 0, "concat_att_fwd: bad sizes");
  GH_REQUIRE(u_mode >= 0 && u_mode <= 2, "concat_att_fwd: u_mode %d not in {0,1,2}", u_mode);
  GH_REQUIRE((goff == nullptr) == (rowg == nullptr), "concat_att_fwd: goff and rowg come together");
  if (!goff) m_real = b * l;
  GH_REQUIRE(m_real >= 0 && m_real <= b * l, "concat_att_fwd: node-compact rows %d do not fit b*l=%d", m_real, b * l);
  if (!rowu && u_mode != 1) nl = b;
  const int M = m_real;
  const bool one_block = ha <= Batch(false, M, s).bn;
  GH_REQUIRE(one_block || (ha % 4 == 0 && al16(t) && al16(u) && al16(w2)),
// ... 60 lines not shown
                                 gh_stream_t stream) {
  return att_fwd_impl(left, b, nullptr, right, mask, goff, rowg, m_real, b, l, xl, dr, ha, heads, w1, w2, u, t, e, weights, attended,
                      (hipStream_t)stream);
}

int gh::att_bwd_impl(const float* left, const float* right, const int32_t* goff, int m_real, int b, int l,
                 int xl, int dr, int ha, int heads, const float* w1t, const float* w2, const float* t, const float* weights,
                 const float* g_att, const float* g_w, float* de, float* dpre, float* du,
                 float* dleft, float* dright, float* dw1, float* dw2,
                 const int32_t* claim_offsets, int nl, float* du_c, int dleft_accumulate, hipStream_t s,
                 const int32_t* rowg, float* dw_tmp, const GateFuse* next, int dleft_late, float* dw2_buf,
                 const void* right16, const void* w1t_16) {
  GH_REQUIRE(heads >= 1 && heads <= 8, "concat_att: heads=%d not in [1,8]", heads);
  if (!goff) m_real = b * l;
  GH_REQUIRE(m_real >= 0 && m_real <= b * l, "concat_att_bwd: node-compact rows %d do not fit b*l=%d", m_real, b * l);
  GH_REQUIRE((claim_offsets == nullptr) == (du_c == nullptr), "concat_att_bwd: claim_offsets and du_c come together");
  const int M = m_real;
  if (!left) xl = 0;
  if (!claim_offsets) nl = b;
  const float* dul = claim_offsets ? du_c : du;
  const int ldw = xl + dr;
  const bool weights_only = (dright == nullptr);
  GH_REQUIRE(!weights_only || dw1, "concat_att_bwd: dright == NULL asks for the dw1-only phase, which needs dw1");
  const bool use16 = right16 && w1t_16 && g_gemm_mode == 1 && m_real >= 8192 && dr % 8 == 0 && ha % 8 == 0 && xl % 8 == 0;
  void* const dpre16 = use16 ? (void*)dpre : nullptr;
  float* dw2_part = nullptr;
  if (!weights_only) {
  int dw_written = 0;
  if (int e = launch_att_softmax_bwd(right, weights, g_att, g_w, goff, m_real, b, l, dr, heads, de, dright, s, rowg, dw_tmp, &dw_written,
                                     use16 ? right16 : nullptr)) return e;
  const size_t dw2_bytes = (size_t)b * heads * ha * sizeof(float);
  const Workspace wsp = workspace_for(s);
  const bool late = dleft_late && dw2_buf && ha % 4 == 0;
  dw2_part = late ? dw2_buf : ((wsp.p && dw2_bytes <= wsp.bytes && ha % 4 == 0) ? wsp.p : nullptr);
  if (int e = launch_att_dpre(de, w2, t, goff, m_real, b, l, ha, heads, dpre, du, dw2_part, s, dw_written ? dw_tmp : nullptr,
                              dw_written ? weights : nullptr, dw_written ? de : nullptr, dpre16,
                              (long long)m_real * heads, dw_written > 1 ? dw_written : 1)) return e;
  if (dw2_part && !late) {
    ReduceArgs R;
    R.n = 1;
    R.it[0] = ReduceItem{dw2_part, dw2, heads, ha, ha, b, (long long)heads * ha};
    hipLaunchKernelGGL(reduce_partials_wave_kernel, dim3((heads * (ha / 4) + 3) / 4, 1), dim3(256), 0, s, R);
    GH_LAUNCH_CHECK();
  }
  if (claim_offsets && xl > 0 && !dleft_late)
    if (int e = gh_seg_sum(du, claim_offsets, du_c, nl, ha, (gh_stream_t)s)) return e;
  const float* w1t_r16 = use16 ? (const float*)((const unsigned short*)w1t_16 + (size_t)xl * ha) : nullptr;
  GH_REQUIRE(!next || !next->bf16 || use16, "concat_att_bwd: a bf16 gate head needs the bf16 twins of right and w1t");
  if (M > 0 && next) {
    Batch bt(false, M, s, use16 && dr % 256 == 0, 6, dr);
    Problem p = use16 ? gemm_problem(M, dr, EPI_GATE_PRE, next->dhp, dr, (const float*)dpre16, ha, w1t_r16, ha, ha, nullptr, 1)
                      : gemm_problem(M, dr, EPI_GATE_PRE, next->dhp, dr, dpre, ha, w1t + (size_t)xl * ha, ha, ha);
    p.gin = dright; p.in0 = next->z; p.in1 = next->hh; p.in2 = next->xp; p.out1 = next->dzp; p.out2 = next->dxp;
    p.io = next->bf16 ? (1 | 2 | 4 | 8 | 16 | 32) : 0;
    bt.add(p);
    bt.flush();
    GH_CHECK_HIP(bt.err);
  } else if (M > 0) {
    Batch bt(false, M, s, use16 && dr % 256 == 0);
    Problem p = use16 ? gemm_problem(M, dr, EPI_STORE, dright, dr, (const float*)dpre16, ha, w1t_r16, ha, ha, nullptr, 1)
                      : gemm_problem(M, dr, EPI_STORE, dright, dr, dpre, ha, w1t + (size_t)xl * ha, ha, ha);
    p.accumulate = 1;
    bt.add(p);
    bt.flush();
    GH_CHECK_HIP(bt.err);
  }
  if (xl > 0 && dleft && !dleft_late) {
    Batch bt(false, nl, s);
    Problem p = gemm_problem(nl, xl, EPI_STORE, dleft, xl, dul, ha, w1t, ha, ha);
    p.accumulate = dleft_accumulate ? 1 : 0;
    bt.add(p);
    bt.flush();
    GH_CHECK_HIP(bt.err);
  }
  if (!dw2_part && M > 0) {
    Batch bt(true, M, s);
    bt.add(tn_problem(heads, ha, dw2, ha, de, heads, t, ha, M));
    bt.flush();
    GH_CHECK_HIP(bt.err);
  }
  }
  if (weights_only && dleft_late) {
    if (dw2_buf && ha % 4 == 0) {
      ReduceArgs R;
      R.n = 1;
      R.it[0] = ReduceItem{dw2_buf, dw2, heads, ha, ha, b, (long long)heads * ha};
      hipLaunchKernelGGL(reduce_partials_wave_kernel, dim3((heads * (ha / 4) + 3) / 4, 1), dim3(256), 0, s, R);
      GH_LAUNCH_CHECK();
    }
    if (claim_offsets && xl > 0)
      if (int e = gh_seg_sum(du, claim_offsets, du_c, nl, ha, (gh_stream_t)s)) return e;
  }
  if (weights_only && dleft_late && xl > 0 && dleft) {
    Batch bt(false, nl, s);
    Problem p = gemm_problem(nl, xl, EPI_STORE, dleft, xl, dul, ha, w1t, ha, ha);
    p.accumulate = dleft_accumulate ? 1 : 0;
    bt.add(p);
    bt.flush();
    GH_CHECK_HIP(bt.err);
  }
  if (!dw1) return 0;
  if (M > 0) {
    Batch bt(true, M, s);
    if (use16) bt.add(tn_problem(ha, dr, dw1 + xl, ldw, (const float*)dpre16, ha, (const float*)right16, dr, M, nullptr, 1));
    else bt.add(tn_problem(ha, dr, dw1 + xl, ldw, dpre, ha, right, dr, M));
    bt.flush();
// ... 175 lines not shown
```

### get_amd/csrc/misc_ops.hip

```cpp
#include "../../include/get_hip.h"
#include "common.h"
#include <mutex>
#include <unordered_map>
#include "gemm.hip.h"
#include <stdarg.h>
#include <vector>

namespace gh {

static thread_local char g_err[512] = "";

void set_error(const char* fmt, ...) {
  va_list ap;
  va_start(ap, fmt);
  vsnprintf(g_err, sizeof(g_err), fmt, ap);
  va_end(ap);
}

struct ProfRec { hipEvent_t a, b; int tag; double work; };
static bool g_prof_on = false;
static unsigned g_prof_mask = 0xFFFFFFFFu;
static std::vector<ProfRec> g_prof_recs;
static std::vector<hipEvent_t> g_prof_pool;
static hipEvent_t g_prof_cur = nullptr;
// ... 144 lines not shown
gate_bwd_pre_bf16_kernel(const float4* __restrict__ g, const uint2* __restrict__ z, const uint2* __restrict__ hh,
                         const uint2* __restrict__ xp, uint2* __restrict__ dhp, uint2* __restrict__ dzp,
                         uint2* __restrict__ dxp, size_t n4) {
  for (size_t i = (size_t)blockIdx.x * blockDim.x + threadIdx.x; i < n4; i += (size_t)gridDim.x * blockDim.x) {
    const float4 G = g[i], Z = mbf4_to_f4(z[i]), Hh = mbf4_to_f4(hh[i]), X = mbf4_to_f4(xp[i]);
    float4 a, b, c;
#define GH_ONE(f)                                      \
    a.f = G.f * Z.f * (1.f - Hh.f * Hh.f);             \
    b.f = G.f * (Hh.f - X.f) * Z.f * (1.f - Z.f);      \
    c.f = G.f * (1.f - Z.f);
    GH_ONE(x) GH_ONE(y) GH_ONE(z) GH_ONE(w)
#undef GH_ONE
    dhp[i] = make_uint2(mpack_bf2(a.x, a.y), mpack_bf2(a.z, a.w));
    dzp[i] = make_uint2(mpack_bf2(b.x, b.y), mpack_bf2(b.z, b.w));
    dxp[i] = make_uint2(mpack_bf2(c.x, c.y), mpack_bf2(c.z, c.w));
  }
}

int launch_gate_bwd_pre(const float* g, const float* z, const float* hh, const float* xp, float* dhp, float* dzp,
                        float* dxp, size_t count, hipStream_t s, int bf16) {
  if (count == 0) return 0;
  if (bf16) {
    GH_REQUIRE(count % 4 == 0, "gate_bwd_pre: the bf16 variant needs a multiple of 4 elements");
    const size_t n4 = count / 4;
    const int grid = (int)((n4 + 255) / 256 < 4096 ? (n4 + 255) / 256 : 4096);
    prof_begin(s, PROF_GATE_BWD_PRE);
    hipLaunchKernelGGL(gate_bwd_pre_bf16_kernel, dim3(grid), dim3(256), 0, s, (const float4*)g, (const uint2*)z, (const uint2*)hh,
                       (const uint2*)xp, (uint2*)dhp, (uint2*)dzp, (uint2*)dxp, n4);
    prof_end(PROF_GATE_BWD_PRE, (4.0 + 6.0 * 2.0) * (double)count, s);
    GH_LAUNCH_CHECK();
    return 0;
  }
  const uintptr_t al = (uintptr_t)g | (uintptr_t)z | (uintptr_t)hh | (uintptr_t)xp | (uintptr_t)dhp | (uintptr_t)dzp | (uintptr_t)dxp;
  if (count % 4 == 0 && (al & 15) == 0) {
    const size_t n4 = count / 4;
    const int grid = (int)((n4 + 255) / 256 < 4096 ? (n4 + 255) / 256 : 4096);
    const int ptag = count < ((size_t)1 << 21) ? PROF_FEW_ROWS : PROF_GATE_BWD_PRE;
    prof_begin(s, ptag);
    hipLaunchKernelGGL(gate_bwd_pre_kernel, dim3(grid), dim3(256), 0, s, (const float4*)g, (const float4*)z,
                       (const float4*)hh, (const float4*)xp, (float4*)dhp, (float4*)dzp, (float4*)dxp, n4);
    prof_end(ptag, 7.0 * 4.0 * (double)count, s);
  } else {
    const int grid = (int)((count + 255) / 256 < 4096 ? (count + 255) / 256 : 4096);
    hipLaunchKernelGGL(gate_bwd_pre_scalar_kernel, dim3(grid), dim3(256), 0, s, g, z, hh, xp, dhp, dzp, dxp, count);
  }
  GH_LAUNCH_CHECK();
  return 0;
}

constexpr int CS_ROWS = 256;
__global__ void __launch_bounds__(256)
colsum_kernel(const float* __restrict__ a, const float* __restrict__ b, const float* __restrict__ c,
              float* __restrict__ oa, float* __restrict__ ob, float* __restrict__ oc, float* __restrict__ oa2,
              float* __restrict__ ob2, float* __restrict__ oc2, int m, int h) {
  const int r0 = blockIdx.x * CS_ROWS, r1 = min(m, r0 + CS_ROWS);
  for (int col = threadIdx.x; col < h; col += 256) {
    float sa = 0.f, sb = 0.f, sc = 0.f;
    for (int r = r0; r < r1; ++r) {
      sa += a[(size_t)r * h + col];
      if (b) sb += b[(size_t)r * h + col];
      if (c) sc += c[(size_t)r * h + col];
    }
    atomicAdd(oa + col, sa);
    if (b) atomicAdd(ob + col, sb);
    if (c) atomicAdd(oc + col, sc);
    if (oa2) atomicAdd(oa2 + col, sa);
    if (b && ob2) atomicAdd(ob2 + col, sb);
    if (c && oc2) atomicAdd(oc2 + col, sc);
  }
}
constexpr int CS2_ROWS = 128;
__global__ void colsum_partial_kernel(const float* __restrict__ a, const float* __restrict__ b, const float* __restrict__ c,
                                      float* __restrict__ ws, int m, int h, int RL, int rows_per_block) {
  extern __shared__ __attribute__((aligned(16))) unsigned char dsm[];
  float4* red = reinterpret_cast<float4*>(dsm);
  const int n4 = h / 4;
  const int c4 = threadIdx.x % n4, rl = threadIdx.x / n4;
  const int r0 = blockIdx.x * rows_per_block, r1 = min(m, r0 + rows_per_block);
  float4 sa = make_float4(0.f, 0.f, 0.f, 0.f), sb = sa, sc = sa;
  if (rl < RL) {
#pragma unroll 4
    for (int r = r0 + rl; r < r1; r += RL) {
      const size_t o = (size_t)r * n4 + c4;
      const float4 va = reinterpret_cast<const float4*>(a)[o];
      sa.x += va.x; sa.y += va.y; sa.z += va.z; sa.w += va.w;
      if (b) { const float4 v = reinterpret_cast<const float4*>(b)[o]; sb.x += v.x; sb.y += v.y; sb.z += v.z; sb.w += v.w; }
      if (c) { const float4 v = reinterpret_cast<const float4*>(c)[o]; sc.x += v.x; sc.y += v.y; sc.z += v.z; sc.w += v.w; }
    }
    red[(0 * RL + rl) * n4 + c4] = sa;
    red[(1 * RL + rl) * n4 + c4] = sb;
    red[(2 * RL + rl) * n4 + c4] = sc;
  }
  __syncthreads();
  for (int i = threadIdx.x; i < 3 * n4; i += blockDim.x) {
    const int arr = i / n4, cc = i % n4;
    float4 t = make_float4(0.f, 0.f, 0.f, 0.f);
    for (int k = 0; k < RL; ++k) {
      const float4 v = red[(arr * RL + k) * n4 + cc];
      t.x += v.x; t.y += v.y; t.z += v.z; t.w += v.w;
    }
    reinterpret_cast<float4*>(ws)[((size_t)blockIdx.x * 3 + arr) * n4 + cc] = t;
  }
}
__global__ void __launch_bounds__(256)
colsum_final_kernel(const float* __restrict__ ws, int nblk, int h, float* __restrict__ oa, float* __restrict__ ob,
                    float* __restrict__ oc, float* __restrict__ oa2, float* __restrict__ ob2, float* __restrict__ oc2) {
  __shared__ float red[4][64];
  const int i = blockIdx.x * 64 + (threadIdx.x & 63), kl = threadIdx.x >> 6;
  float acc = 0.f;
  if (i < 3 * h) {
    const int arr = i / h, col = i % h;
#pragma unroll 4
    for (int k = kl; k < nblk; k += 4) acc += ws[((size_t)k * 3 + arr) * h + col];
  }
  red[kl][threadIdx.x & 63] = acc;
  __syncthreads();
  if (kl == 0 && i < 3 * h) {
    const int arr = i / h, col = i % h;
    float* out = arr == 0 ? oa : (arr == 1 ? ob : oc);
    float* out2 = arr == 0 ? oa2 : (arr == 1 ? ob2 : oc2);
    const float v = red[0][threadIdx.x] + red[1][threadIdx.x] + red[2][threadIdx.x] + red[3][threadIdx.x];
    if (out) out[col] += v;
    if (out2) out2[col] += v;
  }
}


int launch_colsum3(const float* a, const float* b, const float* c, float* oa, float* ob, float* oc, int m, int h,
                   hipStream_t s, float* oa2, float* ob2, float* oc2) {
  if (m <= 0) return 0;
  const uintptr_t al = (uintptr_t)a | (uintptr_t)b | (uintptr_t)c;
  const int rpb = m <= 8192 ? 16 : CS2_ROWS;
  const int nblk = (m + rpb - 1) / rpb;
  const size_t need = (size_t)nblk * 3 * h * sizeof(float);
  const double bytes = 4.0 * (double)m * h * (1 + (b != nullptr) + (c != nullptr));
  const Workspace wsp = workspace_for(s);
  float* const g_cs_ws = wsp.cs;
  if (g_cs_ws && need <= wsp.cs_bytes && h % 4 == 0 && h / 4 <= 256 && (al & 15) == 0) {
    const int n4 = h / 4;
    const int RL = (256 / n4) > 0 ? (256 / n4) : 1;
    const int threads = ((n4 * RL + 63) / 64) * 64;
    prof_begin(s, PROF_COLSUM);
    hipLaunchKernelGGL(colsum_partial_kernel, dim3(nblk), dim3(threads), (size_t)3 * RL * h * sizeof(float), s, a, b, c,
                       g_cs_ws, m, h, RL, rpb);
    hipLaunchKernelGGL(colsum_final_kernel, dim3((3 * h + 63) / 64), dim3(256), 0, s, g_cs_ws, nblk, h, oa, ob, oc, oa2, ob2, oc2);
    prof_end(PROF_COLSUM, bytes, s);
    GH_LAUNCH_CHECK();
    return 0;
  }
  prof_begin(s, PROF_COLSUM);
  hipLaunchKernelGGL(colsum_kernel, dim3((m + CS_ROWS - 1) / CS_ROWS), dim3(256), 0, s, a, b, c, oa, ob, oc, oa2, ob2, oc2, m, h);
  prof_end(PROF_COLSUM, bytes, s);
  GH_LAUNCH_CHECK();
  return 0;
}
int launch_colsum(const float* a, float* oa, int m, int h, hipStream_t s) {
  return launch_colsum3(a, nullptr, nullptr, oa, nullptr, nullptr, m, h, s, nullptr, nullptr, nullptr);
}

__global__ void __launch_bounds__(256)
gather_rows_kernel(const float* __restrict__ table, const int32_t* __restrict__ ids, float* __restrict__ dst, int m,
                   int d, unsigned drop_thresh, float drop_scale, unsigned drop_seed) {
  const int per = (d + 3) / 4;
  if (d % 4 == 0 && ((reinterpret_cast<uintptr_t>(table) | reinterpret_cast<uintptr_t>(dst)) & 15) == 0) {
    const size_t total = (size_t)m * per, stride = (size_t)gridDim.x * blockDim.x;
    for (size_t it0 = (size_t)blockIdx.x * blockDim.x + threadIdx.x; it0 < total; it0 += 4 * stride) {
      int r[4], c[4], src[4];
      float4 v[4];
#pragma unroll
      for (int k = 0; k < 4; ++k) {
        const size_t it = it0 + k * stride < total ? it0 + k * stride : it0;
        r[k] = (int)(it / per); c[k] = 4 * (int)(it % per);
      }
#pragma unroll
      for (int k = 0; k < 4; ++k) src[k] = ids ? ids[r[k]] : r[k];
#pragma unroll
      for (int k = 0; k < 4; ++k) v[k] = *reinterpret_cast<const float4*>(table + (size_t)src[k] * d + c[k]);
#pragma unroll
      for (int k = 0; k < 4; ++k) {
        if (it0 + k * stride >= total) break;
        float4 w = v[k];
        if (drop_thresh) w = drop4(w, drop_seed, (unsigned)r[k] * (unsigned)d + (unsigned)c[k], drop_thresh, drop_scale);
        *reinterpret_cast<float4*>(dst + (size_t)r[k] * d + c[k]) = w;
      }
    }
    return;
  }
  for (size_t it = (size_t)blockIdx.x * blockDim.x + threadIdx.x; it < (size_t)m * per; it += (size_t)gridDim.x * blockDim.x) {
    const int r = (int)(it / per), c = 4 * (int)(it % per);
    const float* s = table + (size_t)(ids ? ids[r] : r) * d + c;
    float* o = dst + (size_t)r * d + c;
    if (d % 4 == 0) {
      float4 v = *reinterpret_cast<const float4*>(s);
      if (drop_thresh) v = drop4(v, drop_seed, (unsigned)r * (unsigned)d + (unsigned)c, drop_thresh, drop_scale);
      *reinterpret_cast<float4*>(o) = v;
    } else {
      for (int k = 0; k < 4 && c + k < d; ++k) {
        float v = s[k];
        if (drop_thresh) v = drop_hash(drop_seed, (unsigned)r * (unsigned)d + (unsigned)(c + k)) >= drop_thresh ? v * drop_scale : 0.f;
        o[k] = v;
      }
    }
  }
}
// ... 1285 lines not shown
```

### get_amd/csrc/model_ops.hip

```cpp
#include "../../include/get_hip.h"
#include "common.h"
#include <mutex>
#include <unordered_map>

namespace gh {

struct Dims {
  int B, B1, L, R, n, D, H, hw, he, C, cs, as, Xl, Xa, Dre, E, W;
  bool compact;
  int Mr, Mt, M1, Mq;
  bool bf;
  bool att16;
  bool fuse_scorer;
};
struct CellBuf { int64_t xp, a, z, rr, rx, hh, out, out32, xdrop; };
struct FwdBuf {
  int64_t offsets, pair2claim, has, lens_eff, rowc, maskf_p;
  CellBuf q, c1, c2;
  int64_t q_repr, score_x, score, keep;
  int64_t uw, tw, ew, ww, avg, new_left;
  int64_t right_e, mask_e, ue, te, ee, we, att_e, y0, phi;
  int64_t total;
  int64_t obs_total;
};
struct BwdBuf {
  int64_t d_y0, d_new_left, d_att_e, de_e, dpre_e, du_e, dright_e, d_avg;
  int64_t de_w, dw_w, dpre_w, du_w, du_c, d_q, g2, d_qhid, qs[5], sc2[5], sc1[5], dx2, dw2p_e, dw2p_w, dw_e;
  int64_t total;
};
struct Bump {
  int64_t off = 0;
  int64_t take(int64_t nfloats) { const int64_t o = off; off += (nfloats + 63) & ~(int64_t)63; return o; }
};

static int make_dims(const gh_get_model* Mo, const gh_get_batch* Ba, Dims& d) {
  GH_REQUIRE(Mo && Ba, "get: NULL model / batch descriptor");
  d.B = Ba->b; d.B1 = Ba->b1; d.L = Ba->l; d.R = Ba->r; d.n = Ba->n_max;
  d.D = Mo->d; d.H = Mo->h; d.hw = Mo->word_heads; d.he = Mo->evd_heads; d.C = Mo->n_classes;
  d.cs = Mo->claim_src_dim; d.as = Mo->article_src_dim;
  GH_REQUIRE(d.B > 0 && d.B1 > 0 && d.L > 0 && d.R > 0 && d.n > 0, "get: bad batch sizes b=%d b1=%d l=%d r=%d n_max=%d", d.B, d.B1, d.L, d.R, d.n);
  GH_REQUIRE(d.R <= 256 && d.L <= 256, "get: padded graph sizes above 256 nodes are not supported (l=%d r=%d)", d.L, d.R);
  GH_REQUIRE(d.D % 4 == 0 && d.H % 4 == 0 && d.D >= 4 && d.D <= d.H && d.H <= 1024,
             "get: the composite path needs float4-shaped widths with d <= h <= 1024 (d=%d h=%d); use the per-module entry points", d.D, d.H);
  GH_REQUIRE(Mo->storage == 0 || Mo->storage == 1, "get: model->storage %d not in {0 (fp32), 1 (bf16 storage in the evidence cells)}", Mo->storage);
  GH_REQUIRE(d.hw >= 1 && d.hw <= 8 && d.he >= 1 && d.he <= 8, "get: heads %d / %d not in [1,8]", d.hw, d.he);
  GH_REQUIRE(Ba->k_keep >= 0 && Ba->k_keep <= d.R, "get: k_keep=%d not in [0, r=%d]", Ba->k_keep, d.R);
  GH_REQUIRE(d.C >= 1 && d.cs >= 0 && d.as >= 0 && d.cs % 4 == 0 && d.as % 4 == 0, "get: bad class / source widths (%d, %d, %d)", d.C, d.cs, d.as);
  d.Xl = d.H + d.cs; d.Xa = d.H * d.hw; d.Dre = d.Xa + d.as; d.E = d.Xl + d.Dre * d.he; d.W = words_for(d.R);
  d.compact = Ba->m_real >= 0;
  d.Mt = d.B1 * d.R;
  if (d.compact) {
    GH_REQUIRE(Ba->goff && Ba->rowg && Ba->cids && Ba->maskf, "get: the node-compact layout needs goff, rowg, cids and maskf");
    GH_REQUIRE(Ba->m_real > 0 && Ba->m_real <= d.Mt, "get: m_real=%d does not fit b1*r=%d", Ba->m_real, d.Mt);
    d.Mr = Ba->m_real;
    d.M1 = Ba->collapsed ? (d.Mr + 1 < d.Mt ? d.Mr + 1 : d.Mt) : d.Mt;
    GH_REQUIRE(!(Ba->collapsed && Ba->drop_gnn > 0.f), "get: collapsed padding rows are an evaluation-mode layout (no dropout)");
  } else {
    d.Mr = d.Mt; d.M1 = d.Mt;
  }
  d.Mq = d.B * d.L;
  d.fuse_scorer = d.H <= 320;
  d.bf = Mo->storage == 1 && d.D % 8 == 0 && d.H % 8 == 0 && d.Mr >= 8192;
  if (d.bf) {
    const gh_cell_bf16* cs[2] = {&Mo->cell1_16, &Mo->cell2_16};
    for (const gh_cell_bf16* c : cs)
      GH_REQUIRE(c->w_p && c->w_z0 && c->w_z1 && c->w_r0 && c->w_r1 && c->w_h0 && c->w_h1,
                 "get: storage = 1 needs the bf16 twins of both evidence cells' weights (gh_weights_refresh)");
    GH_REQUIRE(Mo->embedding16, "get: storage = 1 needs the bf16 copy of the word table (embedding16)");
  }
  d.att16 = d.bf && gemm_mode() == 1 && Mo->att_word_w1_16 && Mo->att_word_w1t_16 && d.Mr >= 8192 && d.H % 8 == 0;
  return 0;
}

static void cell_buf(Bump& b, CellBuf& c, int64_t rows, int H, bool bf = false, bool need32 = true, int64_t drop_din = 0) {
  c.xdrop = (bf && drop_din > 0) ? b.take(rows * drop_din / 2) : -1;
  const int64_t e = bf ? rows * H / 2 : rows * H;
  c.xp = b.take(e); c.a = b.take(e); c.z = b.take(e); c.rr = b.take(e);
  c.rx = b.take(e); c.hh = b.take(e); c.out = b.take(e);
  c.out32 = bf ? (need32 ? b.take(rows * H) : -1) : c.out;
}

static int layout(const gh_get_model* Mo, const gh_get_batch* Ba, Dims& d, FwdBuf& f, BwdBuf& w) {
  if (int e = make_dims(Mo, Ba, d)) return e;
  Bump b;
  f.offsets = b.take(d.B + 1); f.pair2claim = b.take(d.B1); f.has = b.take(d.B); f.lens_eff = b.take(d.B);
  f.rowc = b.take(d.Mr);
  f.maskf_p = d.compact ? -1 : b.take(d.Mt);
  {
    Bump o;
    f.phi = o.take((int64_t)d.B * d.C);
    f.ww = o.take((int64_t)d.Mr * d.hw);
    f.we = o.take((int64_t)d.B * d.n * d.he);
    f.score = o.take((int64_t)d.B1 * d.R);
    f.keep = o.take((int64_t)d.B1 * d.W * 2);
    f.obs_total = o.off;
  }
  cell_buf(b, f.q, d.Mq, d.H);
  f.q_repr = b.take((int64_t)d.B * d.H);
  const bool pre_drop = d.bf && Ba->drop_gnn > 0.f;
  cell_buf(b, f.c1, d.M1, d.H, d.bf, !d.bf, pre_drop ? d.D : 0);
  f.score_x = b.take((int64_t)d.M1 * ((d.fuse_scorer || !d.bf) ? 1 : 8));
  cell_buf(b, f.c2, d.Mr, d.H, d.bf, !d.att16, pre_drop ? d.H : 0);
  f.uw = b.take((int64_t)d.B * d.H); f.tw = b.take((int64_t)d.Mr * d.H); f.ew = b.take((int64_t)d.Mr * d.hw);
  f.avg = b.take((int64_t)d.B1 * d.Xa);
  f.new_left = d.cs > 0 ? b.take((int64_t)d.B * d.Xl) : f.q_repr;
  f.right_e = b.take((int64_t)d.B * d.n * d.Dre); f.mask_e = b.take((int64_t)d.B * d.n);
  f.ue = b.take((int64_t)d.B * d.H); f.te = b.take((int64_t)d.B * d.n * d.H); f.ee = b.take((int64_t)d.B * d.n * d.he);
  f.att_e = b.take((int64_t)d.B * d.Dre * d.he);
  f.y0 = b.take((int64_t)d.B * d.H);
  f.total = b.off;
  Bump c;
  w.d_y0 = c.take((int64_t)d.B * d.H); w.d_new_left = c.take((int64_t)d.B * d.Xl); w.d_att_e = c.take((int64_t)d.B * d.Dre * d.he);
  w.de_e = c.take((int64_t)d.B * d.n * d.he); w.dpre_e = c.take((int64_t)d.B * d.n * d.H); w.du_e = c.take((int64_t)d.B * d.H);
  w.dright_e = c.take((int64_t)d.B * d.n * d.Dre);
  w.d_avg = c.take((int64_t)d.B1 * d.Xa);
  w.de_w = c.take((int64_t)d.Mr * d.hw); w.dw_w = c.take((int64_t)((d.H + 511) / 512) * d.Mr * d.hw);
  w.dw_e = c.take((int64_t)((d.Dre + 511) / 512) * d.B * d.n * d.he); w.dpre_w = c.take((int64_t)d.Mr * d.H); w.du_w = c.take((int64_t)d.B1 * d.H);
  w.du_c = c.take((int64_t)d.B * d.H);
  w.d_q = d.cs > 0 ? c.take((int64_t)d.B * d.H) : w.d_new_left;
  w.g2 = c.take((int64_t)d.Mr * d.H);
  w.d_qhid = c.take((int64_t)d.Mq * d.H);
  for (int i = 0; i < 5; ++i) w.qs[i] = c.take((int64_t)d.Mq * d.H);
  const int64_t se = d.bf ? (int64_t)d.Mr * d.H / 2 : (int64_t)d.Mr * d.H;
  for (int i = 0; i < 5; ++i) w.sc2[i] = c.take(se);
  for (int i = 0; i < 5; ++i) w.sc1[i] = c.take(se);
  w.dx2 = d.bf ? c.take((int64_t)d.Mr * d.H) : w.g2;
  w.dw2p_e = c.take((int64_t)d.B * d.he * d.H); w.dw2p_w = c.take((int64_t)d.B1 * d.hw * d.H);
  w.total = c.off;
  return 0;
}

struct DevEvents { hipEvent_t ev[12]; };
static std::mutex g_ev_mu;
static std::unordered_map<int, DevEvents> g_events;
static int get_events(DevEvents& out) {
  int dev = 0;
  GH_CHECK_HIP(hipGetDevice(&dev));
  std::lock_guard<std::mutex> lk(g_ev_mu);
  auto it = g_events.find(dev);
  if (it == g_events.end()) {
    DevEvents e;
    for (int i = 0; i < 12; ++i) GH_CHECK_HIP(hipEventCreateWithFlags(&e.ev[i], hipEventDisableTiming));
    it = g_events.emplace(dev, e).first;
  }
  out = it->second;
  return 0;
}
static int stream_after(hipStream_t to, hipStream_t from, hipEvent_t ev) {
  if (to == from) return 0;
  GH_CHECK_HIP(hipEventRecord(ev, from));
  GH_CHECK_HIP(hipStreamWaitEvent(to, ev, 0));
  return 0;
}

__global__ void __launch_bounds__(256)
rows_prep_kernel(const int32_t* __restrict__ pair2claim, const int32_t* __restrict__ rowg, int R, int Mr,
                 int32_t* __restrict__ rowc, const int32_t* __restrict__ d_ids, float* __restrict__ maskf_p,
                 const void* __restrict__ q_lens, int kind, const float* __restrict__ has, float* __restrict__ lens_eff, int B) {
  const int i = blockIdx.x * blockDim.x + threadIdx.x;
  if (i < Mr) {
    const int pair = rowg ? rowg[i] : i / R;
    rowc[i] = pair2claim[pair];
    if (maskf_p) maskf_p[i] = d_ids[i] >= 1 ? 1.f : 0.f;
  }
  if (i < B) {
    float len;
    if (kind == 0) len = reinterpret_cast<const float*>(q_lens)[i];
    else if (kind == 1) len = (float)reinterpret_cast<const int32_t*>(q_lens)[i];
    else len = (float)reinterpret_cast<const int64_t*>(q_lens)[i];
    lens_eff[i] = has[i] > 0.f ? len : INFINITY;
  }
}

template <typename TL>
__global__ void __launch_bounds__(256)
seg_rows_kernel(const int64_t* __restrict__ counts, int B, int b1, const int32_t* __restrict__ rowg, int R, int Mr,
                int32_t* __restrict__ offsets, int32_t* __restrict__ pair2claim, float* __restrict__ has, int32_t* __restrict__ rowc,
                const int32_t* __restrict__ d_ids, float* __restrict__ maskf_p, const TL* __restrict__ q_lens, float* __restrict__ lens_eff) {
// ... 48 lines not shown
  const int b = blockIdx.x;
  const float hb = has[b];
  const long long sb = (long long)src[b];
  if ((sb < 0 || sb >= rows) && threadIdx.x == 0) atomicAdd(clamped + 1, 1u);
  const float* tp = table + (size_t)(sb < 0 ? 0 : (sb >= rows ? rows - 1 : sb)) * cs;
  float* o = new_left + (size_t)b * (cs + H);
  for (int i = threadIdx.x; i < cs; i += blockDim.x) o[i] = tp[i] * hb;
  for (int i = threadIdx.x; i < H; i += blockDim.x) o[cs + i] = q_repr[(size_t)b * H + i];
}
template <typename TS>
__global__ void __launch_bounds__(256)
left_assemble_bwd_kernel(const float* __restrict__ d_new_left, const TS* __restrict__ src, const float* __restrict__ has,
                         float* __restrict__ d_q, float* __restrict__ d_table, int B, int cs, int H, int rows) {
  for (int i = threadIdx.x; i < B * H; i += blockDim.x) {
    const int b = i / H, c = i - b * H;
    d_q[i] = d_new_left[(size_t)b * (cs + H) + cs + c];
  }
  if (!d_table) return;
  for (int c = threadIdx.x; c < cs; c += blockDim.x)
    for (int b = 0; b < B; ++b) {
      const long long sb = (long long)src[b];
      d_table[(size_t)(sb < 0 ? 0 : (sb >= rows ? rows - 1 : sb)) * cs + c] += d_new_left[(size_t)b * (cs + H) + c] * has[b];
    }
}

__global__ void __launch_bounds__(256)
cross_entropy_kernel(const float* __restrict__ phi, const int64_t* __restrict__ labels, int B, int C, float* __restrict__ loss,
                     float* __restrict__ dphi, unsigned int* __restrict__ clamped) {
  __shared__ float part[256];
  float acc = 0.f;
  const float invb = 1.f / (float)B;
  for (int b = threadIdx.x; b < B; b += blockDim.x) {
    const float* p = phi + (size_t)b * C;
    float mx = p[0];
    for (int c = 1; c < C; ++c) mx = fmaxf(mx, p[c]);
    float se = 0.f;
    for (int c = 0; c < C; ++c) se += expf(p[c] - mx);
    const float lse = mx + logf(se);
    const long long yl = labels[b];
    const int y = yl < 0 ? 0 : (yl >= C ? C - 1 : (int)yl);
    if (yl < 0 || yl >= C) atomicAdd(clamped, 1u);
    acc += lse - p[y];
    for (int c = 0; c < C; ++c) dphi[(size_t)b * C + c] = (expf(p[c] - lse) - (c == y ? 1.f : 0.f)) * invb;
  }
  part[threadIdx.x] = acc;
  __syncthreads();
  for (int o = 128; o > 0; o >>= 1) {
    if ((int)threadIdx.x < o) part[threadIdx.x] += part[threadIdx.x + o];
    __syncthreads();
  }
  if (threadIdx.x == 0) loss[0] = part[0] * invb;
}

__global__ void __launch_bounds__(256)
document_scatter_kernel(const int32_t* __restrict__ d_ids, const int64_t* __restrict__ slot, int32_t* __restrict__ document, int R) {
  const int g = blockIdx.x;
  const size_t dst = (size_t)slot[g] * R;
  for (int j = threadIdx.x; j < R; j += blockDim.x) document[dst + j] = d_ids[(size_t)g * R + j];
}

}

using namespace gh;

extern "C" int gh_get_plan_buffers(const gh_get_model* Mo, const gh_get_batch* Ba, gh_get_plan* P) {
  GH_REQUIRE(P, "get_plan_buffers: NULL plan");
  Dims d; FwdBuf f; BwdBuf w;
  if (int e = layout(Mo, Ba, d, f, w)) return e;
  P->fwd_floats = f.total; P->bwd_floats = w.total; P->obs_floats = f.obs_total;
  P->phi = f.phi; P->word_w = f.ww; P->evd_w = f.we; P->score = f.score; P->keep = f.keep;
  return 0;
}

extern "C" int gh_get_struct_sizes(int64_t* out) {
  GH_REQUIRE(out, "get_struct_sizes: NULL");
  out[0] = sizeof(gh_get_model); out[1] = sizeof(gh_get_batch); out[2] = sizeof(gh_get_plan); out[3] = sizeof(gh_cell_params);
  out[4] = sizeof(gh_cell_bf16);
  return 0;
}

#define GH_TRY(expr) do { if (int _rc = (expr)) return _rc; } while (0)

static inline const int32_t* I32(const float* A, int64_t off) { return reinterpret_cast<const int32_t*>(A + off); }
static inline int32_t* I32(float* A, int64_t off) { return reinterpret_cast<int32_t*>(A + off); }

static int cell_fwd(const gh_cell_params& c, const gh_cell_bf16* c16, const CellBuf& cb, float* A, const uint64_t* bits, const float* dinv,
                    const float* vals, const uint64_t* keep, const int32_t* goff, int m_real, int m_rows, const float* x, const int32_t* ids,
                    int n, int r, int din, int h, float drop_p, uint32_t seed, const float* score_w, float* score_x, float sdrop,
                    uint32_t sseed, hipStream_t s, int pad_out_dead = 0, int* score_parts = nullptr) {
  typedef const float* cf;
  if (c16)
    return cell_fwd_impl(1, cb.out32 >= 0 ? A + cb.out32 : nullptr, bits, dinv, vals, keep, goff, m_real, m_rows, x, ids, n, r, din, h, (cf)c16->w_p, (cf)c16->w_z0,
                         (cf)c16->w_z1, (cf)c16->w_r0, (cf)c16->w_r1, (cf)c16->w_h0, (cf)c16->w_h1, c.b_z0, c.b_z1, c.b_r0, c.b_r1, c.b_h0,
                         c.b_h1, A + cb.xp, A + cb.a, A + cb.z, A + cb.rr, A + cb.rx, A + cb.hh, A + cb.out, drop_p, seed, score_w, score_x,
                         sdrop, sseed, (void*)s, 0, score_parts, cb.xdrop >= 0 ? A + cb.xdrop : nullptr);
  return cell_fwd_impl(0, nullptr, bits, dinv, vals, keep, goff, m_real, m_rows, x, ids, n, r, din, h, c.w_p, c.w_z0, c.w_z1, c.w_r0,
                       c.w_r1, c.w_h0, c.w_h1, c.b_z0, c.b_z1, c.b_r0, c.b_r1, c.b_h0, c.b_h1, A + cb.xp, A + cb.a, A + cb.z,
                       A + cb.rr, A + cb.rx, A + cb.hh, A + cb.out, drop_p, seed, score_w, score_x, sdrop, sseed, (void*)s, pad_out_dead);
}
static int cell_bwd(const gh_cell_params& c, const gh_cell_bf16* c16, const CellBuf& cb, const float* A, const uint64_t* bits, const float* dinv,
                    const float* vals, const uint64_t* keep, const int32_t* goff, int m_real, const float* x, const int32_t* ids, int n,
                    int r, int din, int h, const float* g, float* W, const int64_t* sc, float* dx, float drop_p, uint32_t seed,
                    hipStream_t s, int pre_done = 0, const GateFuse* next = nullptr) {
  GH_REQUIRE(c.dw_p && c.db_z0 && c.db_z1, "get_backward: a cell's gradient outputs are missing");
  if (c16) {
    typedef const float* cf;
    GH_REQUIRE(c16->wt_p && c16->wt_z0 && c16->wt_z1 && c16->wt_r0 && c16->wt_r1 && c16->wt_h0 && c16->wt_h1,
               "get_backward: storage = 1 needs the bf16 twins of the cells' transposed weights (gh_weights_refresh)");
    return cell_bwd_impl(1, bits, dinv, vals, keep, goff, m_real, x, ids, n, r, din, h, (cf)c16->wt_p, (cf)c16->wt_z0, (cf)c16->wt_z1,
                         (cf)c16->wt_r0, (cf)c16->wt_r1, (cf)c16->wt_h0, (cf)c16->wt_h1, A + cb.xp, A + cb.a, A + cb.z, A + cb.rr,
                         A + cb.rx, A + cb.hh, g, W + sc[0], W + sc[1], W + sc[2], W + sc[3], W + sc[4], dx, c.dw_p, c.dw_z0, c.dw_z1,
                         c.dw_r0, c.dw_r1, c.dw_h0, c.dw_h1, c.db_z0, c.db_r0, c.db_h0, c.db_z1, c.db_r1, c.db_h1, drop_p, seed, (void*)s,
                         nullptr, nullptr, nullptr, pre_done, next, cb.xdrop >= 0 ? A + cb.xdrop : nullptr);
  }
  GH_REQUIRE(c.wt_p, "get_backward: a cell's transposes are missing");
  return cell_bwd_impl(0, bits, dinv, vals, keep, goff, m_real, x, ids, n, r, din, h, c.wt_p, c.wt_z0, c.wt_z1, c.wt_r0, c.wt_r1,
                       c.wt_h0, c.wt_h1, A + cb.xp, A + cb.a, A + cb.z, A + cb.rr, A + cb.rx, A + cb.hh, g, W + sc[0], W + sc[1],
                       W + sc[2], W + sc[3], W + sc[4], dx, c.dw_p, c.dw_z0, c.dw_z1, c.dw_r0, c.dw_r1, c.dw_h0, c.dw_h1, c.db_z0,
                       c.db_r0, c.db_h0, c.db_z1, c.db_r1, c.db_h1, drop_p, seed, (void*)s, nullptr, nullptr, nullptr, pre_done, next);
}

extern "C" int gh_get_forward(const gh_get_model* Mo, const gh_get_batch* Ba, float* A, float* O, gh_stream_t stream, gh_stream_t side_stream) {
  Dims d; FwdBuf f; BwdBuf w;
  GH_TRY(layout(Mo, Ba, d, f, w));
  GH_REQUIRE(A && (reinterpret_cast<uintptr_t>(A) & 255) == 0, "get_forward: the arena must be 256-byte aligned");
  GH_REQUIRE(O && (reinterpret_cast<uintptr_t>(O) & 255) == 0, "get_forward: the observables buffer must be 256-byte aligned");
  GH_REQUIRE(Ba->q_ids && Ba->q_lens && Ba->q_bits && (Ba->q_dinv || Ba->q_vals) && Ba->d_ids && Ba->d_bits && (Ba->d_dinv || Ba->d_vals) &&
             Ba->counts && Ba->document, "get_forward: a batch tensor is missing (ids, lens, packed graphs, counts, document)");
  GH_REQUIRE(Ba->q_lens_kind >= 0 && Ba->q_lens_kind <= 2, "get_forward: q_lens_kind %d not in {0,1,2}", Ba->q_lens_kind);
  GH_REQUIRE(d.as == 0 || Ba->doc_sources, "get_forward: article-source ids are missing");
  GH_REQUIRE(d.cs == 0 || Ba->query_sources, "get_forward: claim-source ids are missing");
  GH_REQUIRE(Mo->embedding && Mo->scorer_w && Mo->scorer_gate && Mo->out0_w && Mo->out1_w, "get_forward: missing model tensors");
  GH_REQUIRE((d.cs == 0) == (Mo->claim_src_table == nullptr) && (d.as == 0) == (Mo->article_src_table == nullptr),
             "get_forward: source tables and their widths must come together");
  GH_REQUIRE(d.cs == 0 || Mo->claim_src_rows > 0, "get_forward: claim_src_rows must give the claim-source table's row count");
  GH_REQUIRE(d.as == 0 || Mo->article_src_rows > 0, "get_forward: article_src_rows must give the article-source table's row count");
  GH_REQUIRE(Ba->drop_claim >= 0.f && Ba->drop_claim < 1.f && Ba->drop_gnn >= 0.f && Ba->drop_gnn < 1.f, "get_forward: dropout p not in [0,1)");
  hipStream_t s = (hipStream_t)stream, ss = side_stream ? (hipStream_t)side_stream : s;
  DevEvents ev;
  GH_TRY(get_events(ev));
  const int H = d.H;
  if (d.B <= 1024) {
    const int nthr = d.Mr > d.B1 ? d.Mr : d.B1;
    const dim3 grid((nthr + 255) / 256);
    const int32_t* rg = d.compact ? Ba->rowg : nullptr;
    float* mp = d.compact ? nullptr : A + f.maskf_p;
    if (Ba->q_lens_kind == 0)
      hipLaunchKernelGGL(seg_rows_kernel<float>, grid, dim3(256), 0, s, Ba->counts, d.B, d.B1, rg, d.R, d.Mr, I32(A, f.offsets), I32(A, f.pair2claim),
                         A + f.has, I32(A, f.rowc), Ba->d_ids, mp, (const float*)Ba->q_lens, A + f.lens_eff);
    else if (Ba->q_lens_kind == 1)
      hipLaunchKernelGGL(seg_rows_kernel<int32_t>, grid, dim3(256), 0, s, Ba->counts, d.B, d.B1, rg, d.R, d.Mr, I32(A, f.offsets), I32(A, f.pair2claim),
                         A + f.has, I32(A, f.rowc), Ba->d_ids, mp, (const int32_t*)Ba->q_lens, A + f.lens_eff);
    else
      hipLaunchKernelGGL(seg_rows_kernel<int64_t>, grid, dim3(256), 0, s, Ba->counts, d.B, d.B1, rg, d.R, d.Mr, I32(A, f.offsets), I32(A, f.pair2claim),
                         A + f.has, I32(A, f.rowc), Ba->d_ids, mp, (const int64_t*)Ba->q_lens, A + f.lens_eff);
    GH_LAUNCH_CHECK();
  } else {
  GH_TRY(gh_seg_offsets(Ba->counts, d.B, I32(A, f.offsets), I32(A, f.pair2claim), d.B1, A + f.has, (void*)s));
  {
    const int nthr = d.Mr > d.B ? d.Mr : d.B;
    hipLaunchKernelGGL(rows_prep_kernel, dim3((nthr + 255) / 256), dim3(256), 0, s, I32(A, f.pair2claim), d.compact ? Ba->rowg : nullptr, d.R,
                       d.Mr, I32(A, f.rowc), Ba->d_ids, d.compact ? nullptr : A + f.maskf_p, Ba->q_lens, Ba->q_lens_kind, A + f.has,
                       A + f.lens_eff, d.B);
    GH_LAUNCH_CHECK();
  }
  }
  GH_TRY(stream_after(ss, s, ev.ev[0]));
  GH_TRY(cell_fwd(Mo->claim, nullptr, f.q, A, Ba->q_bits, Ba->q_dinv, Ba->q_vals, nullptr, nullptr, 0, 0, Mo->embedding, Ba->q_ids, d.B, d.L,
                  d.D, H, Ba->drop_claim, Ba->seed_claim, nullptr, nullptr, 0.f, 0, ss));
  GH_TRY(gh_masked_mean_fwd(A + f.q.out, Ba->q_ids, A + f.lens_eff, A + f.q_repr, d.B, d.L, H, (void*)ss));
  if (d.cs > 0) {
    unsigned int* cl = clamp_counter();
// ... 21 lines not shown
                    Ba->drop_gnn, Ba->seed_cell1, Mo->scorer_w, A + f.score_x, Ba->drop_gnn, Ba->seed_scorer, s, 1));
    GH_TRY(gh_scorer_gsl(Ba->d_bits, Ba->d_dinv, Ba->d_vals, goff, (d.compact && Ba->collapsed) ? 1 : 0, nullptr, A + f.score_x, Mo->scorer_w,
                         Mo->scorer_gate, d.B1, d.R, H, Ba->k_keep, O + f.score, keep, 0.f, 0, (void*)s));
  } else if (d.bf) {
    GH_REQUIRE((H + 127) / 128 <= 8, "get_forward: hidden width %d needs more than the 8 scorer-partial slots", H);
    int parts = 1;
    GH_TRY(cell_fwd(Mo->cell1, c16_1, f.c1, A, Ba->d_bits, Ba->d_dinv, Ba->d_vals, nullptr, goff, d.Mr, d.M1, table1, ids1, d.B1, d.R, d.D, H,
                    Ba->drop_gnn, Ba->seed_cell1, Mo->scorer_w, A + f.score_x, Ba->drop_gnn, Ba->seed_scorer, s, 0, &parts));
    GH_REQUIRE(parts >= 1 && parts <= 8, "get_forward: internal -- %d scorer partials", parts);
    GH_TRY(scorer_gsl_impl(Ba->d_bits, Ba->d_dinv, Ba->d_vals, goff, (d.compact && Ba->collapsed) ? 1 : 0, nullptr, A + f.score_x, parts, d.M1,
                           Mo->scorer_w, Mo->scorer_gate, d.B1, d.R, H, Ba->k_keep, O + f.score, keep, 0.f, 0, s));
  } else {
    GH_TRY(cell_fwd(Mo->cell1, c16_1, f.c1, A, Ba->d_bits, Ba->d_dinv, Ba->d_vals, nullptr, goff, d.Mr, d.M1, table1, ids1, d.B1, d.R, d.D, H,
                    Ba->drop_gnn, Ba->seed_cell1, nullptr, nullptr, 0.f, 0, s, 0));
    GH_TRY(gh_scorer_gsl(Ba->d_bits, Ba->d_dinv, Ba->d_vals, goff, (d.compact && Ba->collapsed) ? 1 : 0, A + f.c1.out32, nullptr, Mo->scorer_w,
                         Mo->scorer_gate, d.B1, d.R, H, Ba->k_keep, O + f.score, keep, Ba->drop_gnn, Ba->seed_scorer, (void*)s));
  }
  GH_TRY(cell_fwd(Mo->cell2, c16_2, f.c2, A, Ba->d_bits, Ba->d_dinv, Ba->d_vals, keep, goff, d.Mr, d.Mr, A + f.c1.out, nullptr, d.B1, d.R, H, H,
                  Ba->drop_gnn, Ba->seed_cell2, nullptr, nullptr, 0.f, 0, s));
  GH_TRY(stream_after(s, ss, ev.ev[1]));
  GH_TRY(att_fwd_impl(A + f.q_repr, d.B, I32(A, f.rowc), f.c2.out32 >= 0 ? A + f.c2.out32 : nullptr, d.compact ? Ba->maskf : A + f.maskf_p, goff,
                      d.compact ? Ba->rowg : nullptr, d.Mr, d.B1, d.R, H, H, H, d.hw, Mo->att_word.w1, Mo->att_word.w2, A + f.uw, A + f.tw,
                      A + f.ew, O + f.ww, A + f.avg, s, 2, d.bf ? (const void*)(A + f.c2.out) : nullptr, d.bf ? Mo->att_word_w1_16 : nullptr));
  GH_TRY(gh_evd_assemble_fwd(A + f.avg, I32(A, f.offsets), Mo->article_src_table, Mo->article_src_rows, d.as > 0 ? Ba->doc_sources : nullptr, Ba->doc_sources_i64,
                             Ba->document, Ba->document_i64, d.B, d.n, d.Xa, d.as, d.R, A + f.right_e, A + f.mask_e, (void*)s));
  GH_TRY(att_fwd_impl(A + f.new_left, d.B, nullptr, A + f.right_e, A + f.mask_e, nullptr, nullptr, 0, d.B, d.n, d.Xl, d.Dre, H, d.he,
                      Mo->att_evd.w1, Mo->att_evd.w2, A + f.ue, A + f.te, A + f.ee, O + f.we, A + f.att_e, s, 2));
  if (d.C <= 8) {
    GH_TRY(linear2_fwd(A + f.new_left, d.Xl, A + f.att_e, d.Dre * d.he, Mo->out0_w, Mo->out0_b, A + f.y0, d.B, H, s, Mo->out1_w, Mo->out1_b,
                       O + f.phi, d.C));
  } else {
    GH_TRY(linear2_fwd(A + f.new_left, d.Xl, A + f.att_e, d.Dre * d.he, Mo->out0_w, Mo->out0_b, A + f.y0, d.B, H, s));
    GH_TRY(gh_linear_fwd(A + f.y0, Mo->out1_w, Mo->out1_b, O + f.phi, d.B, H, d.C, (void*)s));
  }
  return 0;
}

extern "C" int gh_get_backward(const gh_get_model* Mo, const gh_get_batch* Ba, const float* A, const float* O, float* Wb, const float* g_phi,
                               const float* g_word_w, const float* g_evd_w, int phase, gh_stream_t stream, gh_stream_t side_stream) {
  Dims d; FwdBuf f; BwdBuf w;
  GH_TRY(layout(Mo, Ba, d, f, w));
  GH_REQUIRE(phase >= 0 && phase <= 2, "get_backward: phase %d not in {0,1,2}", phase);
  GH_REQUIRE(A && O && Wb && g_phi, "get_backward: NULL arena / observables / gradient");
  GH_REQUIRE(Mo->out0_wt && Mo->out1_wt && Mo->att_word.w1t && Mo->att_evd.w1t && Mo->d_out0_w && Mo->d_out0_b && Mo->d_out1_w &&
             Mo->d_out1_b && Mo->att_word.dw1 && Mo->att_word.dw2 && Mo->att_evd.dw1 && Mo->att_evd.dw2,
             "get_backward: transposes / gradient outputs of the attention layers or the head are missing");
  hipStream_t s = (hipStream_t)stream, ss = side_stream ? (hipStream_t)side_stream : s;
  DevEvents ev;
  GH_TRY(get_events(ev));
  const int H = d.H;
  const int32_t* goff = d.compact ? Ba->goff : nullptr;
  const int32_t* ids1 = d.compact ? Ba->cids : Ba->d_ids;
  const uint64_t* keep = reinterpret_cast<const uint64_t*>(O + f.keep);
  const GateFuse gf2 = {A + f.c2.z, A + f.c2.hh, A + f.c2.xp, Wb + w.sc2[0], Wb + w.sc2[1], Wb + w.sc2[3], d.bf ? 1 : 0};
  const GateFuse gf1 = {A + f.c1.z, A + f.c1.hh, A + f.c1.xp, Wb + w.sc1[0], Wb + w.sc1[1], Wb + w.sc1[3], d.bf ? 1 : 0};
  const bool fuse_gate = !d.bf || (Mo->att_word_w1t_16 != nullptr);
  const void* att_r16 = d.bf ? (const void*)(A + f.c2.out) : nullptr;
  const void* att_w1t16 = d.bf ? Mo->att_word_w1t_16 : nullptr;
  const gh_cell_bf16* c16_1 = d.bf ? &Mo->cell1_16 : nullptr;
  const gh_cell_bf16* c16_2 = d.bf ? &Mo->cell2_16 : nullptr;
  const float* table1 = d.bf ? (const float*)Mo->embedding16 : Mo->embedding;
  if (phase != 2) {
    if (d.C <= 8 && H % 4 == 0 && Mo->out0_w && Mo->out1_w && head_bwd_lds(d.B, H, d.C, d.E, Mo->out0_w) > 0) {
      GH_TRY(launch_head_bwd(g_phi, A + f.y0, Mo->out1_w, Mo->out0_w, d.B, H, d.C, d.Xl, d.E, Wb + w.d_y0, Mo->d_out1_w, Mo->d_out1_b,
                             Wb + w.d_new_left, 0, Wb + w.d_att_e, s));
    } else {
      GH_TRY(gh_linear_bwd(A + f.y0, Mo->out1_wt, Mo->out1_w, g_phi, d.B, H, d.C, Wb + w.d_y0, Mo->d_out1_w, Mo->d_out1_b, (void*)s));
      GH_TRY(linear2_bwd(A + f.new_left, d.Xl, A + f.att_e, d.Dre * d.he, Mo->out0_wt, Wb + w.d_y0, d.B, H, Wb + w.d_new_left, 0,
                         Wb + w.d_att_e, nullptr, nullptr, s));
    }
    GH_TRY(stream_after(ss, s, ev.ev[2]));
    GH_TRY(linear2_bwd(A + f.new_left, d.Xl, A + f.att_e, d.Dre * d.he, Mo->out0_wt, Wb + w.d_y0, d.B, H, nullptr, 0, nullptr,
                       Mo->d_out0_w, Mo->d_out0_b, ss));
    GH_TRY(att_bwd_impl(A + f.new_left, A + f.right_e, nullptr, 0, d.B, d.n, d.Xl, d.Dre, H, d.he, Mo->att_evd.w1t, Mo->att_evd.w2, A + f.te,
                        O + f.we, Wb + w.d_att_e, g_evd_w, Wb + w.de_e, Wb + w.dpre_e, Wb + w.du_e, Wb + w.d_new_left, Wb + w.dright_e,
                        nullptr, Mo->att_evd.dw2, nullptr, d.B, nullptr, 1, s, nullptr, (d.Dre + 511) / 512 <= 16 ? Wb + w.dw_e : nullptr, nullptr, 1,
                        Wb + w.dw2p_e));
    GH_TRY(stream_after(ss, s, ev.ev[3]));
    GH_TRY(att_bwd_impl(A + f.new_left, A + f.right_e, nullptr, 0, d.B, d.n, d.Xl, d.Dre, H, d.he, Mo->att_evd.w1t, Mo->att_evd.w2, A + f.te,
                        O + f.we, Wb + w.d_att_e, g_evd_w, Wb + w.de_e, Wb + w.dpre_e, Wb + w.du_e, Wb + w.d_new_left, nullptr, Mo->att_evd.dw1,
                        Mo->att_evd.dw2, nullptr, d.B, nullptr, 1, ss, nullptr, nullptr, nullptr, 1, Wb + w.dw2p_e));
    if (d.cs > 0) {
      if (Ba->query_sources_i64)
        hipLaunchKernelGGL(left_assemble_bwd_kernel<int64_t>, dim3(1), dim3(256), 0, ss, Wb + w.d_new_left, (const int64_t*)Ba->query_sources,
                           A + f.has, Wb + w.d_q, Mo->d_claim_src_table, d.B, d.cs, H, Mo->claim_src_rows);
      else
        hipLaunchKernelGGL(left_assemble_bwd_kernel<int32_t>, dim3(1), dim3(256), 0, ss, Wb + w.d_new_left, (const int32_t*)Ba->query_sources,
                           A + f.has, Wb + w.d_q, Mo->d_claim_src_table, d.B, d.cs, H, Mo->claim_src_rows);
      GH_LAUNCH_CHECK();
    }
    GH_TRY(gh_evd_assemble_bwd(Wb + w.dright_e, I32(A, f.offsets), d.as > 0 ? Ba->doc_sources : nullptr, Ba->doc_sources_i64, Mo->article_src_rows, d.B, d.n, d.Xa,
                               d.as, Wb + w.d_avg, d.as > 0 ? Mo->d_article_src_table : nullptr, (void*)s));
    GH_TRY(att_bwd_impl(A + f.q_repr, f.c2.out32 >= 0 ? A + f.c2.out32 : nullptr, goff, d.Mr, d.B1, d.R, H, H, H, d.hw, Mo->att_word.w1t, Mo->att_word.w2, A + f.tw,
                        O + f.ww, Wb + w.d_avg, g_word_w, Wb + w.de_w, Wb + w.dpre_w, Wb + w.du_w, Wb + w.d_q, Wb + w.g2, nullptr,
                        Mo->att_word.dw2, I32(A, f.offsets), d.B, Wb + w.du_c, 1, s, d.compact ? Ba->rowg : nullptr, Wb + w.dw_w,
                        fuse_gate ? &gf2 : nullptr, 1, Wb + w.dw2p_w, att_r16, att_w1t16));
    GH_TRY(stream_after(ss, s, ev.ev[4]));
    GH_TRY(att_bwd_impl(A + f.q_repr, f.c2.out32 >= 0 ? A + f.c2.out32 : nullptr, goff, d.Mr, d.B1, d.R, H, H, H, d.hw, Mo->att_word.w1t, Mo->att_word.w2, A + f.tw,
                        O + f.ww, Wb + w.d_avg, g_word_w, Wb + w.de_w, Wb + w.dpre_w, Wb + w.du_w, Wb + w.d_q, nullptr, Mo->att_word.dw1,
                        Mo->att_word.dw2, I32(A, f.offsets), d.B, Wb + w.du_c, 1, ss, nullptr, nullptr, nullptr, 1, Wb + w.dw2p_w, att_r16,
                        att_w1t16));
    GH_TRY(gh_masked_mean_bwd(Wb + w.d_q, Ba->q_ids, A + f.lens_eff, Wb + w.d_qhid, d.B, d.L, H, (void*)ss));
    GH_TRY(cell_bwd(Mo->claim, nullptr, f.q, A, Ba->q_bits, Ba->q_dinv, Ba->q_vals, nullptr, nullptr, 0, Mo->embedding, Ba->q_ids, d.B, d.L, d.D, H,
                    Wb + w.d_qhid, Wb, w.qs, nullptr, Ba->drop_claim, Ba->seed_claim, ss));
    if (fuse_gate)
      GH_TRY(cell_bwd(Mo->cell2, c16_2, f.c2, A, Ba->d_bits, Ba->d_dinv, Ba->d_vals, keep, goff, d.Mr, A + f.c1.out, nullptr, d.B1, d.R, H, H,
                      Wb + w.g2, Wb, w.sc2, nullptr, Ba->drop_gnn, Ba->seed_cell2, s, 1, &gf1));
    else
      GH_TRY(cell_bwd(Mo->cell2, c16_2, f.c2, A, Ba->d_bits, Ba->d_dinv, Ba->d_vals, keep, goff, d.Mr, A + f.c1.out, nullptr, d.B1, d.R, H, H,
                      Wb + w.g2, Wb, w.sc2, Wb + w.dx2, Ba->drop_gnn, Ba->seed_cell2, s, 0, nullptr));
  }
  if (phase != 1) {
    if (fuse_gate)
      GH_TRY(cell_bwd(Mo->cell1, c16_1, f.c1, A, Ba->d_bits, Ba->d_dinv, Ba->d_vals, nullptr, goff, d.Mr, table1, ids1, d.B1, d.R, d.D, H,
                      nullptr, Wb, w.sc1, nullptr, Ba->drop_gnn, Ba->seed_cell1, s, 1, nullptr));
    else
      GH_TRY(cell_bwd(Mo->cell1, c16_1, f.c1, A, Ba->d_bits, Ba->d_dinv, Ba->d_vals, nullptr, goff, d.Mr, table1, ids1, d.B1, d.R, d.D, H,
                      Wb + w.dx2, Wb, w.sc1, nullptr, Ba->drop_gnn, Ba->seed_cell1, s, 0, nullptr));
    GH_TRY(stream_after(s, ss, ev.ev[5]));
  }
  return 0;
}

extern "C" int gh_cross_entropy(const float* phi, const int64_t* labels, int b, int c, float* loss, float* dphi, gh_stream_t stream) {
  GH_REQUIRE(b > 0 && c > 0 && phi && labels && loss && dphi, "cross_entropy: bad arguments");
  unsigned int* cl = clamp_counter();
  GH_REQUIRE(cl, "cross_entropy: cannot allocate the clamp counter");
  hipLaunchKernelGGL(cross_entropy_kernel, dim3(1), dim3(256), 0, (hipStream_t)stream, phi, labels, b, c, loss, dphi, cl);
  GH_LAUNCH_CHECK();
  return 0;
}

extern "C" int gh_get_prepare(const int32_t* claim_tokens, const int32_t* claim_len, int b, int l,
                              const int32_t* evd_tokens, const int32_t* evd_len, int b1, int r, int window,
                              int32_t* q_ids, int32_t* q_n, uint64_t* q_bits, float* q_dinv,
                              int32_t* d_ids, int32_t* d_n, uint64_t* d_bits, float* d_dinv,
                              int m_real, int32_t* goff, int32_t* rowg, int32_t* src, int32_t* cids, float* maskf,
                              const int64_t* slot, int32_t* document, gh_stream_t stream) {
  if (b > 0 && b1 > 0) {
    GH_TRY(launch_graph_build2(claim_tokens, claim_len, b, l, q_ids, q_n, q_bits, q_dinv, evd_tokens, evd_len, b1, r, d_ids, d_n, d_bits,
                               d_dinv, window, (hipStream_t)stream));
  } else {
    GH_TRY(gh_graph_build(claim_tokens, claim_len, b, l, window, q_ids, q_n, q_bits, q_dinv, stream));
    GH_TRY(gh_graph_build(evd_tokens, evd_len, b1, r, window, d_ids, d_n, d_bits, d_dinv, stream));
  }
  bool scattered = false;
  if (m_real >= 0 && b1 > 0) {
    GH_TRY(launch_ragged_plan(d_n, d_ids, b1, r, goff, rowg, src, cids, maskf, slot, document, (hipStream_t)stream, &scattered));
  }
  if (slot && document && b1 > 0 && !scattered) {
    hipLaunchKernelGGL(document_scatter_kernel, dim3(b1), dim3(256), 0, (hipStream_t)stream, d_ids, slot, document, r);
    GH_LAUNCH_CHECK();
  }
  return 0;
}
```

Before: 163,200.

## Pack GRU backward gate gradients into one strided buffer and fuse r/h weight GEMM

The backward scratch for the three gate gradients (dz, dr, dh) is placed in one row-interleaved buffer with a 3H leading dimension. The transposed r0 and h0 weights are concatenated per step into one [H,2H] matrix, so the two input-gradient GEMMs can run as a single wider GEMM. To support this, a separate leading dimension for the auxiliary epilogue tensors is threaded through all GEMM epilogue paths, the gate-fuse struct and column sums. The cost is an extra concat kernel per backward pass, strided rather than contiguous epilogue accesses, and the colsum fast path no longer applies when ld != h.

```diff
diff --git a/get_amd/csrc/common.h b/get_amd/csrc/common.h
--- a/get_amd/csrc/common.h
+++ b/get_amd/csrc/common.h
@@ -74,7 +74,8 @@
 int launch_gate_bwd_pre(const float* g, const float* z, const float* hh, const float* xp, float* dhp, float* dzp,
                         float* dxp, size_t count, hipStream_t s, int bf16 = 0);
 int launch_colsum3(const float* a, const float* b, const float* c, float* oa, float* ob, float* oc, int m, int h,
-                   hipStream_t s, float* oa2 = nullptr, float* ob2 = nullptr, float* oc2 = nullptr);
+                   hipStream_t s, float* oa2 = nullptr, float* ob2 = nullptr, float* oc2 = nullptr,
+                   int ld = 0);
 int launch_colsum(const float* a, float* oa, int m, int h, hipStream_t s);
 struct Workspace { float* p; size_t bytes; float* cs; size_t cs_bytes; };
 Workspace workspace_for(hipStream_t s);
@@ -99,7 +100,7 @@
                     const float* weights = nullptr, float* de_out = nullptr, void* dpre16 = nullptr,
                     long long dw_range_stride = 0, int dw_ranges = 1);
 
-struct GateFuse { const float* z; const float* hh; const float* xp; float* dhp; float* dzp; float* dxp; int bf16; };
+struct GateFuse { const float* z; const float* hh; const float* xp; float* dhp; float* dzp; float* dxp; int bf16; int ldg; };
 
 int cell_fwd_impl(int bf, float* out32, const uint64_t* bits, const float* dinv, const float* vals, const uint64_t* keep,
                   const int32_t* goff, int m_real, int m_rows, const float* x, const int32_t* ids, int n, int r, int din, int h,
@@ -119,7 +120,8 @@
                   float* db_r, float* db_h, float* db_z1, float* db_r1, float* db_h1, float drop_p, uint32_t drop_seed, void* stream,
                   void* wstream, hipEvent_t ev_l1, hipEvent_t ev_agg,
                   int pre_done, const GateFuse* next,
-                  const float* xdrop = nullptr);
+                  const float* xdrop = nullptr,
+                  const float* wt_rh0 = nullptr);
 int att_fwd_impl(const float* left, int nl, const int32_t* rowu, const float* right, const float* mask, const int32_t* goff,
                  const int32_t* rowg, int m_real, int b, int l, int xl, int dr, int ha, int heads, const float* w1, const float* w2,
                  float* u, float* t, float* e, float* weights, float* attended, hipStream_t s, int u_mode = 0,
diff --git a/get_amd/csrc/gemm.hip.h b/get_amd/csrc/gemm.hip.h
--- a/get_amd/csrc/gemm.hip.h
+++ b/get_amd/csrc/gemm.hip.h
@@ -30,6 +30,7 @@
   int M, N;
   int epi;
   int accumulate;
+  int ldx;
   float* C; int ldc;
   const float* bias;
   const float* bias2;
@@ -58,6 +59,7 @@
   int per;
 };
 static_assert(sizeof(Launch) <= 4096, "Launch travels by value in the kernarg segment (4 KB)");
+static_assert(sizeof(Problem) == 336, "Problem layout (GH_MAX_PROBLEMS of them fill the kernarg segment)");
 constexpr int DBG_NO_EPILOGUE = 1;
 constexpr int DBG_NO_KLOOP = 2;
 constexpr int DBG_EPI_TICKS = 1024;
@@ -338,7 +340,7 @@
       for (int reg = 0; reg < 4; ++reg) {
         const int row = m0 + wrow + mi * 16 + q * 4 + reg;
         if (tile_ok && row < M) {
-          const size_t o = (size_t)row * ldc + col;
+          const size_t o = (size_t)row * ldc + col, ox = (size_t)row * P.ldx + col;
           const float v = acc[mi][ni][reg] + bias;
           if (epi == EPI_STORE) {
             Cout[o] = P.accumulate ? Cout[o] + v : v;
@@ -347,15 +349,15 @@
           } else if (epi == EPI_SIGMOID_R) {
             const float r = sigmoidf_(v);
             Cout[o] = r;
-            P.out1[o] = r * P.in0[o];
+            P.out1[ox] = r * P.in0[ox];
           } else if (epi == EPI_TANH_H) {
-            const float h = tanhf_(v), z = P.in0[o], xp = P.in1[o];
+            const float h = tanhf_(v), z = P.in0[ox], xp = P.in1[ox];
             Cout[o] = h;
-            P.out1[o] = h * z + xp * (1.f - z);
+            P.out1[ox] = h * z + xp * (1.f - z);
           } else if (epi == EPI_BWD_DRX) {
-            const float xp = P.in0[o], r = P.in1[o];
+            const float xp = P.in0[ox], r = P.in1[ox];
             Cout[o] = v * xp * r * (1.f - r);
-            P.out1[o] += v * r;
+            P.out1[ox] += v * r;
           } else if (epi == EPI_ATOMIC) {
             atomicAdd(Cout + o, v);
           }
@@ -399,7 +401,7 @@
 inline Problem make_problem(int M, int N, int epi, float* C, int ldc) {
   Problem p;
   memset(&p, 0, sizeof(p));
-  p.M = M; p.N = N; p.epi = epi; p.C = C; p.ldc = ldc; p.nseg = 1;
+  p.M = M; p.N = N; p.epi = epi; p.C = C; p.ldc = ldc; p.ldx = ldc; p.nseg = 1;
   return p;
 }
 
diff --git a/get_amd/csrc/gemm_nt.hip.h b/get_amd/csrc/gemm_nt.hip.h
--- a/get_amd/csrc/gemm_nt.hip.h
+++ b/get_amd/csrc/gemm_nt.hip.h
@@ -460,7 +460,7 @@
     return;
   }
   const int epi = P.epi;
-  const int ldc = P.ldc;
+  const int ldc = P.ldc, ldx = P.ldx;
   float* const C = P.C + (split ? (size_t)ks * (size_t)P.split_stride : (size_t)0);
   const float* bias = P.bias;
   float* out1 = P.out1;
@@ -568,19 +568,19 @@
           for (int j = 0; j < CH; ++j) {
             int row, col; float* sp;
             if (where(j, row, col, sp)) {
-              const size_t o = (size_t)row * ldc + col;
+              const size_t o = (size_t)row * ldc + col, ox = (size_t)row * ldx + col;
               if (E == EPI_STORE) { if (accumulate) xa[j] = ld4(C, o, io & 1); }
-              else if (E == EPI_SIGMOID_R) xa[j] = ld4(in0, o, io & 4);
-              else if (E == EPI_TANH_H) { xa[j] = ld4(in0, o, io & 4); xb[j] = ld4(in1, o, io & 8); }
+              else if (E == EPI_SIGMOID_R) xa[j] = ld4(in0, ox, io & 4);
+              else if (E == EPI_TANH_H) { xa[j] = ld4(in0, ox, io & 4); xb[j] = ld4(in1, ox, io & 8); }
               else if (E == EPI_BWD_DRX) {
-                xa[j] = ld4(in0, o, io & 4);
-                xb[j] = ld4(in1, o, io & 8);
-                xc[j] = ld4(out1, o, io & 2);
+                xa[j] = ld4(in0, ox, io & 4);
+                xb[j] = ld4(in1, ox, io & 8);
+                xc[j] = ld4(out1, ox, io & 2);
               } else if (E == EPI_GATE_PRE) {
-                xa[j] = ld4(in0, o, io & 4);
-                xb[j] = ld4(in1, o, io & 8);
-                xc[j] = ld4(P.in2, o, io & 16);
-                if (P.gin) xd[j] = ld4(P.gin, o, false);
+                xa[j] = ld4(in0, ox, io & 4);
+                xb[j] = ld4(in1, ox, io & 8);
+                xc[j] = ld4(P.in2, ox, io & 16);
+                if (P.gin) xd[j] = ld4(P.gin, ox, false);
               } else if (E == EPI_ATT)
                 xa[j] = *reinterpret_cast<const float4*>(P.u + (size_t)(P.rowg ? P.rowg[row] : row / P.R) * P.ldu + col);
             }
@@ -593,7 +593,7 @@
           const float4 v4 = *reinterpret_cast<const float4*>(sp);
           const float4 b4 = *reinterpret_cast<const float4*>(bsum + col);
           float4 w = make_float4(v4.x + b4.x, v4.y + b4.y, v4.z + b4.z, v4.w + b4.w);
-          const size_t o = (size_t)row * ldc + col;
+          const size_t o = (size_t)row * ldc + col, ox = (size_t)row * ldx + col;
           if (E == EPI_STORE) {
             if (drop_mode == 3)
               w = drop4(w, drop_seed, (unsigned)row * (unsigned)drop_ld + (unsigned)(P.drop_col0 + col), drop_thresh, drop_scale);
@@ -605,7 +605,7 @@
             const float4 x = xa[j];
             const float4 r4 = make_float4(sigmoidf_(w.x), sigmoidf_(w.y), sigmoidf_(w.z), sigmoidf_(w.w));
             if (!(pad_rows > 0 && row >= pad_rows)) st4(C, o, r4, io & 1);
-            st4(out1, o, make_float4(r4.x * x.x, r4.y * x.y, r4.z * x.z, r4.w * x.w), io & 2);
+            st4(out1, ox, make_float4(r4.x * x.x, r4.y * x.y, r4.z * x.z, r4.w * x.w), io & 2);
           } else if (E == EPI_TANH_H) {
             const float4 z = xa[j], x = xb[j];
             const float4 h = make_float4(tanhf_(w.x), tanhf_(w.y), tanhf_(w.z), tanhf_(w.w));
@@ -613,8 +613,8 @@
                                    h.z * z.z + x.z * (1.f - z.z), h.w * z.w + x.w * (1.f - z.w));
             const bool pad = pad_rows > 0 && row >= pad_rows;
             if (!pad) st4(C, o, h, io & 1);
-            if (!(pad && out_dead)) st4(out1, o, y, io & 2);
-            if (c32) *reinterpret_cast<float4*>(c32 + o) = y;
+            if (!(pad && out_dead)) st4(out1, ox, y, io & 2);
+            if (c32) *reinterpret_cast<float4*>(c32 + ox) = y;
             if (scorer) {
               if (drop_mode == 2)
                 y = drop4(y, drop_seed, (unsigned)row * (unsigned)drop_ld + (unsigned)(P.drop_col0 + col), drop_thresh, drop_scale);
@@ -626,7 +626,7 @@
             st4(C, o, make_float4(w.x * x.x * r4.x * (1.f - r4.x), w.y * x.y * r4.y * (1.f - r4.y),
                                   w.z * x.z * r4.z * (1.f - r4.z), w.w * x.w * r4.w * (1.f - r4.w)), io & 1);
             d.x += w.x * r4.x; d.y += w.y * r4.y; d.z += w.z * r4.z; d.w += w.w * r4.w;
-            st4(out1, o, d, io & 2);
+            st4(out1, ox, d, io & 2);
           } else if (E == EPI_GATE_PRE) {
             if (drop_mode == 3)
               w = drop4(w, drop_seed, (unsigned)row * (unsigned)drop_ld + (unsigned)(P.drop_col0 + col), drop_thresh, drop_scale);
@@ -640,11 +640,11 @@
             GH_ONE(x) GH_ONE(y) GH_ONE(z) GH_ONE(w)
 #undef GH_ONE
             if constexpr (MODE == 2) {
-              st4(C, o, a, io & 1); st4(out1, o, b, io & 2); st4(P.out2, o, c, io & 32);
+              st4(C, o, a, io & 1); st4(out1, o, b, io & 2); st4(P.out2, ox, c, io & 32);
             } else {
               *reinterpret_cast<float4*>(C + o) = a;
               *reinterpret_cast<float4*>(out1 + o) = b;
-              *reinterpret_cast<float4*>(P.out2 + o) = c;
+              *reinterpret_cast<float4*>(P.out2 + ox) = c;
             }
           } else if (E == EPI_ATT) {
             const float4 u4 = xa[j];
@@ -711,14 +711,14 @@
           for (int j = 0; j < CH; ++j) {
             int row, col; float* sp;
             if (where(j, row, col, sp)) {
-              const size_t o = (size_t)row * ldc + col;
+              const size_t o = (size_t)row * ldc + col, ox = (size_t)row * ldx + col;
               if (E == EPI_STORE) { if (accumulate) xa[j] = ld8(C, o, io & 1); }
-              else if (E == EPI_SIGMOID_R) xa[j] = ld8(in0, o, io & 4);
-              else if (E == EPI_TANH_H) { xa[j] = ld8(in0, o, io & 4); xb[j] = ld8(in1, o, io & 8); }
-              else if (E == EPI_BWD_DRX) { xa[j] = ld8(in0, o, io & 4); xb[j] = ld8(in1, o, io & 8); xc[j] = ld8(out1, o, io & 2); }
+              else if (E == EPI_SIGMOID_R) xa[j] = ld8(in0, ox, io & 4);
+              else if (E == EPI_TANH_H) { xa[j] = ld8(in0, ox, io & 4); xb[j] = ld8(in1, ox, io & 8); }
+              else if (E == EPI_BWD_DRX) { xa[j] = ld8(in0, ox, io & 4); xb[j] = ld8(in1, ox, io & 8); xc[j] = ld8(out1, ox, io & 2); }
               else if (E == EPI_GATE_PRE) {
-                xa[j] = ld8(in0, o, io & 4); xb[j] = ld8(in1, o, io & 8); xc[j] = ld8(P.in2, o, io & 16);
-                if (P.gin) xd[j] = ld8(P.gin, o, false);
+                xa[j] = ld8(in0, ox, io & 4); xb[j] = ld8(in1, ox, io & 8); xc[j] = ld8(P.in2, ox, io & 16);
+                if (P.gin) xd[j] = ld8(P.gin, ox, false);
               }
             }
           }
@@ -729,7 +729,7 @@
           if (!where(j, row, col, sp)) continue;
           float4 wa = add4(*reinterpret_cast<const float4*>(sp), *reinterpret_cast<const float4*>(bsum + col));
           float4 wb = add4(*reinterpret_cast<const float4*>(sp + 4), *reinterpret_cast<const float4*>(bsum + col + 4));
-          const size_t o = (size_t)row * ldc + col;
+          const size_t o = (size_t)row * ldc + col, ox = (size_t)row * ldx + col;
           if (E == EPI_STORE) {
             if (drop_mode == 3) {
               const unsigned idx = (unsigned)row * (unsigned)drop_ld + (unsigned)(P.drop_col0 + col);
@@ -743,13 +743,13 @@
           } else if (E == EPI_SIGMOID_R) {
             const float4 ra = sig4(wa), rb = sig4(wb);
             st8(C, o, ra, rb, io & 1);
-            st8(out1, o, mul4(ra, xa[j].a), mul4(rb, xa[j].b), io & 2);
+            st8(out1, ox, mul4(ra, xa[j].a), mul4(rb, xa[j].b), io & 2);
           } else if (E == EPI_TANH_H) {
             const float4 ha = tanh4(wa), hb = tanh4(wb);
             const float4 ya = mix4(ha, xa[j].a, xb[j].a), yb = mix4(hb, xa[j].b, xb[j].b);
             st8(C, o, ha, hb, io & 1);
-            st8(out1, o, ya, yb, io & 2);
-            if (c32) { *reinterpret_cast<float4*>(c32 + o) = ya; *reinterpret_cast<float4*>(c32 + o + 4) = yb; }
+            st8(out1, ox, ya, yb, io & 2);
+            if (c32) { *reinterpret_cast<float4*>(c32 + ox) = ya; *reinterpret_cast<float4*>(c32 + ox + 4) = yb; }
             if (scorer) {
               float4 sa = ya, sb = yb;
               if (drop_mode == 2) {
@@ -762,7 +762,7 @@
             }
           } else if (E == EPI_BWD_DRX) {
             st8(C, o, drx4(wa, xa[j].a, xb[j].a), drx4(wb, xa[j].b, xb[j].b), io & 1);
-            st8(out1, o, add4(xc[j].a, mul4(wa, xb[j].a)), add4(xc[j].b, mul4(wb, xb[j].b)), io & 2);
+            st8(out1, ox, add4(xc[j].a, mul4(wa, xb[j].a)), add4(xc[j].b, mul4(wb, xb[j].b)), io & 2);
           } else if (E == EPI_GATE_PRE) {
             if (drop_mode == 3) {
               const unsigned idx = (unsigned)row * (unsigned)drop_ld + (unsigned)(P.drop_col0 + col);
@@ -781,7 +781,7 @@
             float4 a0, b0, c0, a1, b1, c1;
             head(wa, xa[j].a, xb[j].a, xc[j].a, a0, b0, c0);
             head(wb, xa[j].b, xb[j].b, xc[j].b, a1, b1, c1);
-            st8(C, o, a0, a1, io & 1); st8(out1, o, b0, b1, io & 2); st8(P.out2, o, c0, c1, io & 32);
+            st8(C, o, a0, a1, io & 1); st8(out1, o, b0, b1, io & 2); st8(P.out2, ox, c0, c1, io & 32);
           }
         }
       }
diff --git a/get_amd/csrc/gemm_nt_epi32.hip.h b/get_amd/csrc/gemm_nt_epi32.hip.h
--- a/get_amd/csrc/gemm_nt_epi32.hip.h
+++ b/get_amd/csrc/gemm_nt_epi32.hip.h
@@ -27,6 +27,7 @@
     constexpr int NOUT = (E == EPI_STORE || E == EPI_SIGMOID_Z || ATT) ? 1 : E == EPI_GATE_PRE ? 3 : 2;
     constexpr int NTAUX = (E == EPI_GATE_PRE || ATT) ? 0 : 2;
     const void* i0 = E == EPI_STORE ? (const void*)C : (const void*)in0;
+    constexpr bool I0C = E == EPI_STORE;
     const void* i2 = E == EPI_BWD_DRX ? (const void*)out1 : (const void*)P.in2;
     const rsrc_t rs_i0 = __builtin_amdgcn_make_buffer_rsrc((void*)(NIN >= 1 ? i0 : (const void*)C), 0, 0x7fffffff, 0x00020000);
     const rsrc_t rs_i1 = __builtin_amdgcn_make_buffer_rsrc((void*)(NIN >= 2 ? (const void*)in1 : (const void*)C), 0, 0x7fffffff, 0x00020000);
@@ -52,10 +53,11 @@
       int row, col, rr;
       const bool ok = f_item(mi_, it, row, col, rr);
       const unsigned vo = ok ? (unsigned)(row * ldc + col) * 4u : OOB;
-      if constexpr (NIN >= 1) qa[s_] = __builtin_bit_cast(e32_u32x4, __builtin_amdgcn_raw_buffer_load_b128(rs_i0, vo, 0, 0));
-      if constexpr (NIN >= 2) qb[s_] = __builtin_bit_cast(e32_u32x4, __builtin_amdgcn_raw_buffer_load_b128(rs_i1, vo, 0, 0));
-      if constexpr (NIN >= 3) qc[s_] = __builtin_bit_cast(e32_u32x4, __builtin_amdgcn_raw_buffer_load_b128(rs_i2, vo, 0, 0));
-      if constexpr (GIN) qg[s_] = __builtin_bit_cast(e32_u32x4, __builtin_amdgcn_raw_buffer_load_b128(rs_g, vo, 0, 0));
+      const unsigned vx = ok ? (unsigned)(row * ldx + col) * 4u : OOB;
+      if constexpr (NIN >= 1) qa[s_] = __builtin_bit_cast(e32_u32x4, __builtin_amdgcn_raw_buffer_load_b128(rs_i0, I0C ? vo : vx, 0, 0));
+      if constexpr (NIN >= 2) qb[s_] = __builtin_bit_cast(e32_u32x4, __builtin_amdgcn_raw_buffer_load_b128(rs_i1, vx, 0, 0));
+      if constexpr (NIN >= 3) qc[s_] = __builtin_bit_cast(e32_u32x4, __builtin_amdgcn_raw_buffer_load_b128(rs_i2, vx, 0, 0));
+      if constexpr (GIN) qg[s_] = __builtin_bit_cast(e32_u32x4, __builtin_amdgcn_raw_buffer_load_b128(rs_g, vx, 0, 0));
       if constexpr (ATT) qg[s_] = __builtin_bit_cast(e32_u32x4, __builtin_amdgcn_raw_buffer_load_b128(rs_g, uoff[idx], 0, 0));
     };
     auto compute = [&](auto IDX) __attribute__((always_inline)) {
@@ -63,6 +65,7 @@
       int row, col, rr;
       const bool ok = f_item(mi_, it, row, col, rr);
       const unsigned vo = ok ? (unsigned)(row * ldc + col) * 4u : OOB;
+      const unsigned vx = ok ? (unsigned)(row * ldx + col) * 4u : OOB;
       float* sp = ep + min(rr, 16 * WM - 1) * EP_PITCH + min(col, BN - 4);
       const float4 v4 = *reinterpret_cast<const float4*>(sp);
       const float4 b4 = *reinterpret_cast<const float4*>(bsum + min(col, BN - 4));
@@ -70,6 +73,9 @@
       const bool pad = pad_rows > 0 && row >= pad_rows;
       auto st = [&](const rsrc_t rs, const float4 v, bool live) __attribute__((always_inline)) {
         __builtin_amdgcn_raw_buffer_store_b128(as_u4(v), rs, live ? vo : OOB, 0, NTAUX);
+      };
+      auto stx = [&](const rsrc_t rs, const float4 v, bool live) __attribute__((always_inline)) {
+        __builtin_amdgcn_raw_buffer_store_b128(as_u4(v), rs, live ? vx : OOB, 0, NTAUX);
       };
       if (E == EPI_STORE) {
         if (drop_mode == 3)
@@ -82,14 +88,14 @@
         const float4 x = as_f4(qa[s_]);
         const float4 r4 = make_float4(sigmoidf_(w.x), sigmoidf_(w.y), sigmoidf_(w.z), sigmoidf_(w.w));
         st(rs_o0, r4, !pad);
-        st(rs_o1, make_float4(r4.x * x.x, r4.y * x.y, r4.z * x.z, r4.w * x.w), true);
+        stx(rs_o1, make_float4(r4.x * x.x, r4.y * x.y, r4.z * x.z, r4.w * x.w), true);
       } else if (E == EPI_TANH_H) {
         const float4 z = as_f4(qa[s_]), x = as_f4(qb[s_]);
         const float4 h = make_float4(tanhf_(w.x), tanhf_(w.y), tanhf_(w.z), tanhf_(w.w));
         float4 y = make_float4(h.x * z.x + x.x * (1.f - z.x), h.y * z.y + x.y * (1.f - z.y),
                                h.z * z.z + x.z * (1.f - z.z), h.w * z.w + x.w * (1.f - z.w));
         st(rs_o0, h, !pad);
-        st(rs_o1, y, !(pad && out_dead));
+        stx(rs_o1, y, !(pad && out_dead));
         if (scorer) {
           if (drop_mode == 2)
             y = drop4(y, drop_seed, (unsigned)row * (unsigned)drop_ld + (unsigned)(P.drop_col0 + col), drop_thresh, drop_scale);
@@ -101,7 +107,7 @@
         st(rs_o0, make_float4(w.x * x.x * r4.x * (1.f - r4.x), w.y * x.y * r4.y * (1.f - r4.y),
                               w.z * x.z * r4.z * (1.f - r4.z), w.w * x.w * r4.w * (1.f - r4.w)), true);
         d.x += w.x * r4.x; d.y += w.y * r4.y; d.z += w.z * r4.z; d.w += w.w * r4.w;
-        st(rs_o1, d, true);
+        stx(rs_o1, d, true);
       } else if (E == EPI_GATE_PRE) {
         if (drop_mode == 3)
           w = drop4(w, drop_seed, (unsigned)row * (unsigned)drop_ld + (unsigned)(P.drop_col0 + col), drop_thresh, drop_scale);
@@ -114,7 +120,7 @@
         c.f = w.f * (1.f - Z.f);
         GH_E32_ONE(x) GH_E32_ONE(y) GH_E32_ONE(z) GH_E32_ONE(w)
 #undef GH_E32_ONE
-        st(rs_o0, a, true); st(rs_o1, b, true); st(rs_o2, c, true);
+        st(rs_o0, a, true); st(rs_o1, b, true); stx(rs_o2, c, true);
       } else if (E == EPI_ATT) {
         const float4 u4 = as_f4(qg[s_]);
         const float4 t4 = make_float4(tanhf_(w.x + u4.x), tanhf_(w.y + u4.y), tanhf_(w.z + u4.z), tanhf_(w.w + u4.w));
diff --git a/get_amd/csrc/gemm_ops.hip b/get_amd/csrc/gemm_ops.hip
--- a/get_amd/csrc/gemm_ops.hip
+++ b/get_amd/csrc/gemm_ops.hip
@@ -37,7 +37,8 @@
       const Seg& s = p.seg[0];
       if (4.0 * (double)s.lda * (double)s.K >= 2147483648.0 || 4.0 * (double)s.ldb * (double)s.K >= 2147483648.0) { fast_why(6, i); return false; }
     }
-    if (p.N % 4 || p.N < 4 || p.ldc % 4 || !al16(p.C)) { fast_why(7, i); return false; }
+    if (p.N % 4 || p.N < 4 || p.ldc % 4 || p.ldx % 4 || !al16(p.C)) { fast_why(7, i); return false; }
+    if (!tn && p.ldx != p.ldc && 4.0 * (double)(p.ldx > p.ldc ? p.ldx : p.ldc) * (double)p.M >= 2147483648.0) { fast_why(7, i); return false; }
     if (tn && (p.M % 4 || p.M < 4)) { fast_why(8, i); return false; }
     if ((p.bias && !al16(p.bias)) || (p.bias2 && !al16(p.bias2)) || (p.out1 && !al16(p.out1)) || (p.in0 && !al16(p.in0)) || (p.in1 && !al16(p.in1)))
       { fast_why(9, i); return false; }
@@ -613,8 +614,8 @@
         for (int i = 0; i < L.nprob; ++i) {
           if (!cs_out[i]) continue;
           const Seg& sg = L.p[i].seg[0];
-          if (L.p[i].elt || sg.lda != L.p[i].M) { colsum_missed = true; continue; }
-          if (launch_colsum3(sg.A, nullptr, nullptr, cs_out[i], nullptr, nullptr, sg.K, L.p[i].M, s, cs_out2[i], nullptr, nullptr)) colsum_missed = true;
+          if (L.p[i].elt) { colsum_missed = true; continue; }
+          if (launch_colsum3(sg.A, nullptr, nullptr, cs_out[i], nullptr, nullptr, sg.K, L.p[i].M, s, cs_out2[i], nullptr, nullptr, sg.lda)) colsum_missed = true;
           else colsum_fused = true;
         }
       }
@@ -626,7 +627,7 @@
         for (int i = 0; i < L.nprob; ++i) {
           Problem& q = L.p[i];
           R.it[i] = ReduceItem{w, q.C, q.M, q.N, q.ldc, L.ksplit, (long long)q.M * q.N};
-          q.C = w; q.ldc = q.N; q.epi = EPI_STORE; q.accumulate = 0; q.split_stride = (long long)q.M * q.N;
+          q.C = w; q.ldc = q.ldx = q.N; q.epi = EPI_STORE; q.accumulate = 0; q.split_stride = (long long)q.M * q.N;
           w += (size_t)L.ksplit * q.M * q.N;
           if (q.M * (q.N / 4) > max_elems) max_elems = q.M * (q.N / 4);
         }
@@ -677,7 +678,7 @@
     if (wide256) {
       bool ok = L.ksplit == 1;
       for (int i = 0; i < L.nprob; ++i) {
-        if (L.p[i].drop_mode == 1) ok = false;
+        if (L.p[i].drop_mode == 1 || L.p[i].ldx != L.p[i].ldc) ok = false;
         for (int j = 0; j < L.p[i].nseg; ++j) if (L.p[i].seg[j].K % 64) ok = false;
       }
       if (ok) return launch_cfg<2, 4, 4, 8>(L, tn, s);
@@ -698,6 +699,7 @@
     for (int i = 0; i < L.nprob; ++i) {
       const Problem& q = L.p[i];
       if (q.epi == EPI_ATOMIC || q.epi == EPI_GATE_PRE || q.drop_mode != 0 || (q.epi == EPI_TANH_H && q.w2) || q.seg0_rows > 0 || q.elt) return false;
+      if (q.ldx != q.ldc) return false;
       int t = 0;
       for (int j = 0; j < q.nseg; ++j) t += (q.seg[j].K + 15) / 16;
       if (i > 0 && t != tmax) return false;
@@ -722,7 +724,7 @@
       Problem& q = L.p[i];
       F.it[i] = FinishItem{w, (long long)q.M * q.N, ks, q.M, q.N, q.epi, q.accumulate, q.ldc,
                            q.C, q.bias, q.bias2, q.out1, q.in0, q.in1, q.u, q.w2, q.e, q.ldu, q.R, q.heads, q.rowg};
-      q.C = w; q.ldc = q.N; q.epi = EPI_STORE; q.accumulate = 0; q.bias = nullptr; q.bias2 = nullptr;
+      q.C = w; q.ldc = q.ldx = q.N; q.epi = EPI_STORE; q.accumulate = 0; q.bias = nullptr; q.bias2 = nullptr;
       q.split_stride = (long long)q.M * q.N;
       w += (size_t)ks * q.M * q.N;
       if (q.M > max_m) max_m = q.M;
@@ -928,7 +930,7 @@
                                 float* dw_h0, float* dw_h1, float* db_z, float* db_r, float* db_h,
                                 float* db_z1, float* db_r1, float* db_h1, float drop_p, uint32_t drop_seed,
                                 gh_stream_t stream, gh_stream_t wstream, hipEvent_t ev_l1, hipEvent_t ev_agg,
-                                int pre_done, const GateFuse* next, const float* xdrop) {
+                                int pre_done, const GateFuse* next, const float* xdrop, const float* wt_rh0) {
   hipStream_t s = (hipStream_t)stream;
   hipStream_t sw = wstream ? (hipStream_t)wstream : s;
   const bool two = sw != s;
@@ -941,16 +943,25 @@
              "ggnn_cell_bwd: %d rows x %d columns exceed the dropout mask's 32-bit element index", n * r, din);
   const int M = m_real;
   if (M == 0) return 0;
+  const bool packed = wt_rh0 != nullptr;
+  GH_REQUIRE(!packed || (!bf && pre_done && drp == dzp + h && dhp == dzp + 2 * h && h % 4 == 0),
+             "ggnn_cell_bwd: packed gate gradients need fp32 storage, a fused gate head and dzp / drp / dhp as the slices of one [rows][3h] array");
+  const int ldg = packed ? 3 * h : h;
   if (!pre_done)
     if (int e = launch_gate_bwd_pre(g, z, hh, xp, dhp, dzp, dxp, (size_t)M * h, s, bf)) return e;
   const bool wide = bf && h % 256 == 0;
   {
     Batch b(false, M, s, wide, 3, h);
-    Problem p0 = gemm_problem(M, h, EPI_STORE, da, h, dhp, h, wt_h0, h, h, nullptr, bf);
-    Problem p1 = gemm_problem(M, h, EPI_BWD_DRX, drp, h, dhp, h, wt_h1, h, h, nullptr, bf);
+    Problem p1 = gemm_problem(M, h, EPI_BWD_DRX, drp, ldg, dhp, ldg, wt_h1, h, h, nullptr, bf);
+    p1.ldx = h;
     p1.out1 = dxp; p1.in0 = xp; p1.in1 = rr;
-    p0.io = bf ? 1 : 0; p1.io = bf ? 15 : 0;
-    b.add(p0); b.add(p1);
+    p1.io = bf ? 15 : 0;
+    if (!packed) {
+      Problem p0 = gemm_problem(M, h, EPI_STORE, da, h, dhp, h, wt_h0, h, h, nullptr, bf);
+      p0.io = bf ? 1 : 0;
+      b.add(p0);
+    }
+    b.add(p1);
     b.flush();
     GH_CHECK_HIP(b.err);
   }
@@ -960,27 +971,31 @@
     GH_CHECK_HIP(hipEventRecord(ev_l1, s));
     GH_CHECK_HIP(hipStreamWaitEvent(sw, ev_l1, 0));
     Batch b(true, M, sw);
-    b.add(tn_problem(h, h, dw_z0, h, dzp, h, a, h, M, nullptr, bf));  if (cs) b.want_colsum(db_z, db_z1);
-    b.add(tn_problem(h, h, dw_z1, h, dzp, h, xp, h, M, nullptr, bf));
-    b.add(tn_problem(h, h, dw_r0, h, drp, h, a, h, M, nullptr, bf));  if (cs) b.want_colsum(db_r, db_r1);
-    b.add(tn_problem(h, h, dw_r1, h, drp, h, xp, h, M, nullptr, bf));
-    b.add(tn_problem(h, h, dw_h0, h, dhp, h, a, h, M, nullptr, bf));  if (cs) b.want_colsum(db_h, db_h1);
-    b.add(tn_problem(h, h, dw_h1, h, dhp, h, rx, h, M, nullptr, bf));
+    b.add(tn_problem(h, h, dw_z0, h, dzp, ldg, a, h, M, nullptr, bf));  if (cs) b.want_colsum(db_z, db_z1);
+    b.add(tn_problem(h, h, dw_z1, h, dzp, ldg, xp, h, M, nullptr, bf));
+    b.add(tn_problem(h, h, dw_r0, h, drp, ldg, a, h, M, nullptr, bf));  if (cs) b.want_colsum(db_r, db_r1);
+    b.add(tn_problem(h, h, dw_r1, h, drp, ldg, xp, h, M, nullptr, bf));
+    b.add(tn_problem(h, h, dw_h0, h, dhp, ldg, a, h, M, nullptr, bf));  if (cs) b.want_colsum(db_h, db_h1);
+    b.add(tn_problem(h, h, dw_h1, h, dhp, ldg, rx, h, M, nullptr, bf));
     b.flush();
     GH_CHECK_HIP(b.err);
     colsum_done = b.colsum_fused && !b.colsum_missed;
     if (!colsum_done) {
       GH_REQUIRE(!bf, "ggnn_cell_bwd_bf16: the bias gradients need the split-K workspace (gh_set_workspace)");
-      if (int e = launch_colsum3(dzp, drp, dhp, db_z, db_r, db_h, M, h, sw, db_z1, db_r1, db_h1)) return e;
+      if (int e = launch_colsum3(dzp, drp, dhp, db_z, db_r, db_h, M, h, sw, db_z1, db_r1, db_h1, ldg)) return e;
     }
   }
   {
     Batch b(false, M, s, wide, 4, h);
-    Problem p0 = gemm_problem(M, h, EPI_STORE, da, h, dzp, h, wt_z0, h, h, nullptr, bf);
-    add_seg(p0, drp, h, wt_r0, h, h);
-    p0.accumulate = 1;
-    Problem p1 = gemm_problem(M, h, EPI_STORE, dxp, h, dzp, h, wt_z1, h, h, nullptr, bf);
-    add_seg(p1, drp, h, wt_r1, h, h);
+    Problem p0 = gemm_problem(M, h, EPI_STORE, da, h, dzp, ldg, wt_z0, h, h, nullptr, bf);
+    if (packed) {
+      add_seg(p0, drp, ldg, wt_rh0, 2 * h, 2 * h);
+    } else {
+      add_seg(p0, drp, h, wt_r0, h, h);
+      p0.accumulate = 1;
+    }
+    Problem p1 = gemm_problem(M, h, EPI_STORE, dxp, h, dzp, ldg, wt_z1, h, h, nullptr, bf);
+    add_seg(p1, drp, ldg, wt_r1, h, h);
     p1.accumulate = 1;
     p0.io = p1.io = bf ? 1 : 0;
     b.add(p0); b.add(p1);
@@ -998,6 +1013,7 @@
     Problem p = gemm_problem(M, din, next ? EPI_GATE_PRE : EPI_STORE, next ? next->dhp : dx, din, dxp, h, wt_p, h, h, nullptr, bf);
     if (next) {
       p.in0 = next->z; p.in1 = next->hh; p.in2 = next->xp; p.out1 = next->dzp; p.out2 = next->dxp;
+      p.ldc = next->ldg;
       p.io = next->bf16 ? (1 | 2 | 4 | 8 | 16 | 32) : 0;
     }
     set_dropout(p, 3, din, drop_p, drop_seed);
@@ -1008,12 +1024,12 @@
   {
     Batch b(true, M, sw);
     if (!two) {
-      b.add(tn_problem(h, h, dw_z0, h, dzp, h, a, h, M, nullptr, bf));  if (cs) b.want_colsum(db_z, db_z1);
-      b.add(tn_problem(h, h, dw_z1, h, dzp, h, xp, h, M, nullptr, bf));
-      b.add(tn_problem(h, h, dw_r0, h, drp, h, a, h, M, nullptr, bf));  if (cs) b.want_colsum(db_r, db_r1);
-      b.add(tn_problem(h, h, dw_r1, h, drp, h, xp, h, M, nullptr, bf));
-      b.add(tn_problem(h, h, dw_h0, h, dhp, h, a, h, M, nullptr, bf));  if (cs) b.want_colsum(db_h, db_h1);
-      b.add(tn_problem(h, h, dw_h1, h, dhp, h, rx, h, M, nullptr, bf));
+      b.add(tn_problem(h, h, dw_z0, h, dzp, ldg, a, h, M, nullptr, bf));  if (cs) b.want_colsum(db_z, db_z1);
+      b.add(tn_problem(h, h, dw_z1, h, dzp, ldg, xp, h, M, nullptr, bf));
+      b.add(tn_problem(h, h, dw_r0, h, drp, ldg, a, h, M, nullptr, bf));  if (cs) b.want_colsum(db_r, db_r1);
+      b.add(tn_problem(h, h, dw_r1, h, drp, ldg, xp, h, M, nullptr, bf));
+      b.add(tn_problem(h, h, dw_h0, h, dhp, ldg, a, h, M, nullptr, bf));  if (cs) b.want_colsum(db_h, db_h1);
+      b.add(tn_problem(h, h, dw_h1, h, dhp, ldg, rx, h, M, nullptr, bf));
     }
     if (bf && xdrop && drop_p > 0.f && din <= h) {
       b.add(tn_problem(h, din, dw_p, din, dxp, h, xdrop, din, M, nullptr, bf));
@@ -1029,7 +1045,7 @@
     if (two || (b.colsum_fused && !b.colsum_missed)) return 0;
   }
   GH_REQUIRE(!bf, "ggnn_cell_bwd_bf16: the bias gradients need the split-K workspace (gh_set_workspace)");
-  return launch_colsum3(dzp, drp, dhp, db_z, db_r, db_h, M, h, s, db_z1, db_r1, db_h1);
+  return launch_colsum3(dzp, drp, dhp, db_z, db_r, db_h, M, h, s, db_z1, db_r1, db_h1, ldg);
 }
 
 extern "C" int gh_ggnn_cell_bwd(const uint64_t* bits, const float* dinv, const float* vals, const uint64_t* keep,
@@ -1196,6 +1212,7 @@
     Problem p = use16 ? gemm_problem(M, dr, EPI_GATE_PRE, next->dhp, dr, (const float*)dpre16, ha, w1t_r16, ha, ha, nullptr, 1)
                       : gemm_problem(M, dr, EPI_GATE_PRE, next->dhp, dr, dpre, ha, w1t + (size_t)xl * ha, ha, ha);
     p.gin = dright; p.in0 = next->z; p.in1 = next->hh; p.in2 = next->xp; p.out1 = next->dzp; p.out2 = next->dxp;
+    p.ldc = next->ldg;
     p.io = next->bf16 ? (1 | 2 | 4 | 8 | 16 | 32) : 0;
     bt.add(p);
     bt.flush();
diff --git a/get_amd/csrc/misc_ops.hip b/get_amd/csrc/misc_ops.hip
--- a/get_amd/csrc/misc_ops.hip
+++ b/get_amd/csrc/misc_ops.hip
@@ -220,14 +220,14 @@
 __global__ void __launch_bounds__(256)
 colsum_kernel(const float* __restrict__ a, const float* __restrict__ b, const float* __restrict__ c,
               float* __restrict__ oa, float* __restrict__ ob, float* __restrict__ oc, float* __restrict__ oa2,
-              float* __restrict__ ob2, float* __restrict__ oc2, int m, int h) {
+              float* __restrict__ ob2, float* __restrict__ oc2, int m, int h, int ld) {
   const int r0 = blockIdx.x * CS_ROWS, r1 = min(m, r0 + CS_ROWS);
   for (int col = threadIdx.x; col < h; col += 256) {
     float sa = 0.f, sb = 0.f, sc = 0.f;
     for (int r = r0; r < r1; ++r) {
-      sa += a[(size_t)r * h + col];
-      if (b) sb += b[(size_t)r * h + col];
-      if (c) sc += c[(size_t)r * h + col];
+      sa += a[(size_t)r * ld + col];
+      if (b) sb += b[(size_t)r * ld + col];
+      if (c) sc += c[(size_t)r * ld + col];
     }
     atomicAdd(oa + col, sa);
     if (b) atomicAdd(ob + col, sb);
@@ -295,8 +295,9 @@
 
 
 int launch_colsum3(const float* a, const float* b, const float* c, float* oa, float* ob, float* oc, int m, int h,
-                   hipStream_t s, float* oa2, float* ob2, float* oc2) {
+                   hipStream_t s, float* oa2, float* ob2, float* oc2, int ld) {
   if (m <= 0) return 0;
+  if (ld <= 0) ld = h;
   const uintptr_t al = (uintptr_t)a | (uintptr_t)b | (uintptr_t)c;
   const int rpb = m <= 8192 ? 16 : CS2_ROWS;
   const int nblk = (m + rpb - 1) / rpb;
@@ -304,7 +305,7 @@
   const double bytes = 4.0 * (double)m * h * (1 + (b != nullptr) + (c != nullptr));
   const Workspace wsp = workspace_for(s);
   float* const g_cs_ws = wsp.cs;
-  if (g_cs_ws && need <= wsp.cs_bytes && h % 4 == 0 && h / 4 <= 256 && (al & 15) == 0) {
+  if (g_cs_ws && need <= wsp.cs_bytes && h % 4 == 0 && h / 4 <= 256 && (al & 15) == 0 && ld == h) {
     const int n4 = h / 4;
     const int RL = (256 / n4) > 0 ? (256 / n4) : 1;
     const int threads = ((n4 * RL + 63) / 64) * 64;
@@ -317,7 +318,7 @@
     return 0;
   }
   prof_begin(s, PROF_COLSUM);
-  hipLaunchKernelGGL(colsum_kernel, dim3((m + CS_ROWS - 1) / CS_ROWS), dim3(256), 0, s, a, b, c, oa, ob, oc, oa2, ob2, oc2, m, h);
+  hipLaunchKernelGGL(colsum_kernel, dim3((m + CS_ROWS - 1) / CS_ROWS), dim3(256), 0, s, a, b, c, oa, ob, oc, oa2, ob2, oc2, m, h, ld);
   prof_end(PROF_COLSUM, bytes, s);
   GH_LAUNCH_CHECK();
   return 0;
diff --git a/get_amd/csrc/model_ops.hip b/get_amd/csrc/model_ops.hip
--- a/get_amd/csrc/model_ops.hip
+++ b/get_amd/csrc/model_ops.hip
@@ -26,6 +26,7 @@
 struct BwdBuf {
   int64_t d_y0, d_new_left, d_att_e, de_e, dpre_e, du_e, dright_e, d_avg;
   int64_t de_w, dw_w, dpre_w, du_w, du_c, d_q, g2, d_qhid, qs[5], sc2[5], sc1[5], dx2, dw2p_e, dw2p_w, dw_e;
+  int64_t wrh2, wrh1;
   int64_t total;
 };
 struct Bump {
@@ -122,8 +123,18 @@
   w.d_qhid = c.take((int64_t)d.Mq * d.H);
   for (int i = 0; i < 5; ++i) w.qs[i] = c.take((int64_t)d.Mq * d.H);
   const int64_t se = d.bf ? (int64_t)d.Mr * d.H / 2 : (int64_t)d.Mr * d.H;
-  for (int i = 0; i < 5; ++i) w.sc2[i] = c.take(se);
-  for (int i = 0; i < 5; ++i) w.sc1[i] = c.take(se);
+  const bool packed = !d.bf && d.H % 4 == 0 && gemm_mode() == 0;
+  for (int64_t* sc : {w.sc2, w.sc1}) {
+    if (!packed) {
+      for (int i = 0; i < 5; ++i) sc[i] = c.take(se);
+    } else {
+      const int64_t g = c.take(3 * se);
+      sc[0] = g + 2 * d.H; sc[1] = g; sc[2] = g + d.H;
+      for (int i = 3; i < 5; ++i) sc[i] = c.take(se);
+    }
+  }
+  w.wrh2 = packed ? c.take((int64_t)2 * d.H * d.H) : -1;
+  w.wrh1 = packed ? c.take((int64_t)2 * d.H * d.H) : -1;
   w.dx2 = d.bf ? c.take((int64_t)d.Mr * d.H) : w.g2;
   w.dw2p_e = c.take((int64_t)d.B * d.he * d.H); w.dw2p_w = c.take((int64_t)d.B1 * d.hw * d.H);
   w.total = c.off;
@@ -278,6 +289,16 @@
   if (threadIdx.x == 0) loss[0] = part[0] * invb;
 }
 
+struct CatCols { const float* a[2]; const float* b[2]; float* dst[2]; };
+__global__ void __launch_bounds__(256)
+cat_cols_kernel(const CatCols C, int h) {
+  const int it = blockIdx.y, row = blockIdx.x;
+  const float* a = C.a[it] + (size_t)row * h;
+  const float* b = C.b[it] + (size_t)row * h;
+  float* o = C.dst[it] + (size_t)row * 2 * h;
+  for (int i = threadIdx.x; i < h; i += blockDim.x) { o[i] = a[i]; o[h + i] = b[i]; }
+}
+
 __global__ void __launch_bounds__(256)
 document_scatter_kernel(const int32_t* __restrict__ d_ids, const int64_t* __restrict__ slot, int32_t* __restrict__ document, int R) {
   const int g = blockIdx.x;
@@ -327,7 +348,7 @@
 static int cell_bwd(const gh_cell_params& c, const gh_cell_bf16* c16, const CellBuf& cb, const float* A, const uint64_t* bits, const float* dinv,
                     const float* vals, const uint64_t* keep, const int32_t* goff, int m_real, const float* x, const int32_t* ids, int n,
                     int r, int din, int h, const float* g, float* W, const int64_t* sc, float* dx, float drop_p, uint32_t seed,
-                    hipStream_t s, int pre_done = 0, const GateFuse* next = nullptr) {
+                    hipStream_t s, int pre_done = 0, const GateFuse* next = nullptr, const float* wt_rh0 = nullptr) {
   GH_REQUIRE(c.dw_p && c.db_z0 && c.db_z1, "get_backward: a cell's gradient outputs are missing");
   if (c16) {
     typedef const float* cf;
@@ -343,7 +364,8 @@
   return cell_bwd_impl(0, bits, dinv, vals, keep, goff, m_real, x, ids, n, r, din, h, c.wt_p, c.wt_z0, c.wt_z1, c.wt_r0, c.wt_r1,
                        c.wt_h0, c.wt_h1, A + cb.xp, A + cb.a, A + cb.z, A + cb.rr, A + cb.rx, A + cb.hh, g, W + sc[0], W + sc[1],
                        W + sc[2], W + sc[3], W + sc[4], dx, c.dw_p, c.dw_z0, c.dw_z1, c.dw_r0, c.dw_r1, c.dw_h0, c.dw_h1, c.db_z0,
-                       c.db_r0, c.db_h0, c.db_z1, c.db_r1, c.db_h1, drop_p, seed, (void*)s, nullptr, nullptr, nullptr, pre_done, next);
+                       c.db_r0, c.db_h0, c.db_z1, c.db_r1, c.db_h1, drop_p, seed, (void*)s, nullptr, nullptr, nullptr, pre_done, next,
+                       nullptr, wt_rh0);
 }
 
 extern "C" int gh_get_forward(const gh_get_model* Mo, const gh_get_batch* Ba, float* A, float* O, gh_stream_t stream, gh_stream_t side_stream) {
@@ -471,8 +493,21 @@
   const int32_t* goff = d.compact ? Ba->goff : nullptr;
   const int32_t* ids1 = d.compact ? Ba->cids : Ba->d_ids;
   const uint64_t* keep = reinterpret_cast<const uint64_t*>(O + f.keep);
-  const GateFuse gf2 = {A + f.c2.z, A + f.c2.hh, A + f.c2.xp, Wb + w.sc2[0], Wb + w.sc2[1], Wb + w.sc2[3], d.bf ? 1 : 0};
-  const GateFuse gf1 = {A + f.c1.z, A + f.c1.hh, A + f.c1.xp, Wb + w.sc1[0], Wb + w.sc1[1], Wb + w.sc1[3], d.bf ? 1 : 0};
+  const bool packed = w.wrh2 >= 0;
+  const int ldg = packed ? 3 * H : H;
+  const GateFuse gf2 = {A + f.c2.z, A + f.c2.hh, A + f.c2.xp, Wb + w.sc2[0], Wb + w.sc2[1], Wb + w.sc2[3], d.bf ? 1 : 0, ldg};
+  const GateFuse gf1 = {A + f.c1.z, A + f.c1.hh, A + f.c1.xp, Wb + w.sc1[0], Wb + w.sc1[1], Wb + w.sc1[3], d.bf ? 1 : 0, ldg};
+  if (packed) {
+    GH_REQUIRE(Mo->cell2.wt_r0 && Mo->cell2.wt_h0 && Mo->cell1.wt_r0 && Mo->cell1.wt_h0, "get_backward: a cell's transposes are missing");
+    CatCols cc;
+    int n = 0;
+    if (phase != 2) { cc.a[n] = Mo->cell2.wt_r0; cc.b[n] = Mo->cell2.wt_h0; cc.dst[n++] = Wb + w.wrh2; }
+    if (phase != 1) { cc.a[n] = Mo->cell1.wt_r0; cc.b[n] = Mo->cell1.wt_h0; cc.dst[n++] = Wb + w.wrh1; }
+    hipLaunchKernelGGL(cat_cols_kernel, dim3(H, n), dim3(256), 0, s, cc, H);
+    GH_LAUNCH_CHECK();
+  }
+  const float* wrh2 = packed ? Wb + w.wrh2 : nullptr;
+  const float* wrh1 = packed ? Wb + w.wrh1 : nullptr;
   const bool fuse_gate = !d.bf || (Mo->att_word_w1t_16 != nullptr);
   const void* att_r16 = d.bf ? (const void*)(A + f.c2.out) : nullptr;
   const void* att_w1t16 = d.bf ? Mo->att_word_w1t_16 : nullptr;
@@ -524,7 +559,7 @@
                     Wb + w.d_qhid, Wb, w.qs, nullptr, Ba->drop_claim, Ba->seed_claim, ss));
     if (fuse_gate)
       GH_TRY(cell_bwd(Mo->cell2, c16_2, f.c2, A, Ba->d_bits, Ba->d_dinv, Ba->d_vals, keep, goff, d.Mr, A + f.c1.out, nullptr, d.B1, d.R, H, H,
-                      Wb + w.g2, Wb, w.sc2, nullptr, Ba->drop_gnn, Ba->seed_cell2, s, 1, &gf1));
+                      Wb + w.g2, Wb, w.sc2, nullptr, Ba->drop_gnn, Ba->seed_cell2, s, 1, &gf1, wrh2));
     else
       GH_TRY(cell_bwd(Mo->cell2, c16_2, f.c2, A, Ba->d_bits, Ba->d_dinv, Ba->d_vals, keep, goff, d.Mr, A + f.c1.out, nullptr, d.B1, d.R, H, H,
                       Wb + w.g2, Wb, w.sc2, Wb + w.dx2, Ba->drop_gnn, Ba->seed_cell2, s, 0, nullptr));
@@ -532,7 +567,7 @@
   if (phase != 1) {
     if (fuse_gate)
       GH_TRY(cell_bwd(Mo->cell1, c16_1, f.c1, A, Ba->d_bits, Ba->d_dinv, Ba->d_vals, nullptr, goff, d.Mr, table1, ids1, d.B1, d.R, d.D, H,
-                      nullptr, Wb, w.sc1, nullptr, Ba->drop_gnn, Ba->seed_cell1, s, 1, nullptr));
+                      nullptr, Wb, w.sc1, nullptr, Ba->drop_gnn, Ba->seed_cell1, s, 1, nullptr, wrh1));
     else
       GH_TRY(cell_bwd(Mo->cell1, c16_1, f.c1, A, Ba->d_bits, Ba->d_dinv, Ba->d_vals, nullptr, goff, d.Mr, table1, ids1, d.B1, d.R, d.D, H,
                       Wb + w.dx2, Wb, w.sc1, nullptr, Ba->drop_gnn, Ba->seed_cell1, s, 0, nullptr));
```

Result: slower. 159,500, median of 2 (-2.3%).
